# victorca25/traiNNer

Measured on AMD Instinct MI355X. Metric: HR images/sec (G+D step), ESRGAN x4 128->512, higher is better.
Workload: dtype f32 (bf16x3)

## Files before the change

include/trainner_hip.h:

```cpp
#ifndef TRAINNER_HIP_H
#define TRAINNER_HIP_H

#include <stdint.h>

#ifdef __cplusplus
extern "C" {
#endif

#define TNR_OK 0
#define TNR_EINVAL (-1)
#define TNR_ELAUNCH (-2)

enum { TNR_ACT_NONE = 0, TNR_ACT_LRELU = 1, TNR_ACT_RELU = 2 };

enum {
    TNR_CONV_3x3 = 0,
    TNR_CONV_3x3_UP2 = 1,
    TNR_CONV_4x4_S2 = 2,
    TNR_DGRAD_4x4_S2 = 3,
    TNR_CONV_1x1 = 4,
    TNR_CONV_3x3_C4 = 5,
    TNR_CONV_7x7_C4 = 6
};

enum {
    TNR_PACK_FWD = 0,
    TNR_PACK_DGRAD_3x3 = 1,
    TNR_PACK_FWD_S2D = 2,
    TNR_PACK_DGRAD_S2 = 3,
    TNR_PACK_COL_FWD = 4,
    TNR_PACK_COL_DGRAD3 = 5,
    TNR_PACK_C4_FWD = 6,
    TNR_PACK_C4_DGRAD3 = 7,
    TNR_PACK_UP2_DGRAD_S2 = 8,
    TNR_PACK_UP2_FWD_S2D = 9
};

#define TNR_MMA_F32 0
#define TNR_MMA_BF16 1
#define TNR_MMA_BF16X3 2

typedef struct tnr_view {
    float *ptr;
    int32_t ctot;
    int32_t coff;
} tnr_view;

typedef struct tnr_conv_desc {
    tnr_view x;
    int32_t N, H, W;
    int32_t Cin;
    const float *wp;
    int32_t KinP, KoutP;
    tnr_view y;
    int32_t Ho, Wo, Cout;
    int32_t mode;
    const float *bias;
    int32_t act;
    float slope;
    float alpha;
    tnr_view r1; int32_t r1_ch; float beta1;
    tnr_view r2; float alpha2;
    tnr_view m;  int32_t m_lo, m_hi; float m_slope;
    float *ws; int64_t ws_bytes;
    int32_t mma;
    int32_t pad_mode;
    float noise_sigma; int32_t noise_pos; uint32_t noise_key0, noise_key1, noise_pix0;
    const void *wq; int64_t wq_bytes;
    int32_t wq_form;
    int32_t shuffle;
} tnr_conv_desc;

typedef struct tnr_wgrad_desc {
    tnr_view x; int32_t N, H, W; int32_t Cin;
    tnr_view g; int32_t Ho, Wo; int32_t Cout;
    int32_t mode;
    float *dw; int32_t cin_total, cin_begin;
    float *db;
    float alpha, beta;
    float *ws; int64_t ws_bytes;
    int32_t mma;
    int32_t pad_mode;
    float *dw2; int32_t cout_split, cin_total2;
    float *db2;
} tnr_wgrad_desc;

typedef struct tnr_pack_item {
    const float *w;
    float *wp;
    int32_t Cout, Cin, kh, kw;
    int32_t kind;
    int32_t KoutP, KinP;
    int64_t n_out;
} tnr_pack_item;

typedef struct tnr_dense_pack_item {
    const float *w[5];
    float *wp;
    int32_t nf, gc;
    int32_t t;
    int32_t KoutP, KinP;
    float scale5;
    int64_t n_out;
} tnr_dense_pack_item;

const char *tnr_last_error(void);
#define TNR_ABI_VERSION 3
int tnr_version(void);

int tnr_pack_dims(int32_t Cout, int32_t Cin, int32_t kh, int32_t kw, int32_t kind,
                  int32_t *KoutP, int32_t *KinP, int64_t *n_out);
int tnr_pack_weights(const tnr_pack_item *items_dev, int32_t n, int64_t max_out, void *stream);
int tnr_upconv_fold_table(int32_t out[144]);
int tnr_upconv_wgrad_unfold(const float *dws, float *dw3, int32_t Cout, int32_t Cin, float alpha, float beta, void *stream);
int tnr_pack_dense_dims(int32_t nf, int32_t gc, int32_t t, int32_t *KoutP, int32_t *KinP, int64_t *n_out);
int tnr_pack_dense_dgrad(const tnr_dense_pack_item *items_dev, int32_t n, int64_t max_out, void *stream);
int tnr_conv_forward(const tnr_conv_desc *d, void *stream);
int tnr_gauss_mult(tnr_view dst, tnr_view src, int64_t pixels, int32_t C, float sigma, uint32_t key0, uint32_t key1, uint32_t pix0,
                   void *stream);
int64_t tnr_conv_workspace_bytes(const tnr_conv_desc *d);
int64_t tnr_conv_wq_bytes(const tnr_conv_desc *d);
int tnr_conv_wq_pack(const tnr_conv_desc *d, void *image, int64_t image_bytes, void *stream);
int64_t tnr_conv_wino_bytes(const tnr_conv_desc *d);
int tnr_conv_wino_pack(const tnr_conv_desc *d, void *image, int64_t image_bytes, void *stream);
int tnr_im2col(tnr_view x, int32_t N, int32_t H, int32_t W, int32_t C, int32_t k, int32_t stride, int32_t pad,
               int32_t Ho, int32_t Wo, float *out, void *stream);
#define TNR_CHAIN_MAX 6
int64_t tnr_conv_chain_workspace_bytes(const tnr_conv_desc *stage0);
int tnr_conv_chain(const tnr_conv_desc *stages, const int32_t *fresh_from, int32_t n, uint32_t *ws, int64_t ws_bytes,
                   uint32_t epoch, void *stream);
int64_t tnr_conv_sweep_image_bytes(const tnr_conv_desc *stages, int32_t n);
int tnr_conv_sweep_pack(const tnr_conv_desc *stages, int32_t n, void *image, int64_t image_bytes, void *stream);
typedef struct tnr_sweep_pack_item { int32_t units; int32_t reserved; uint64_t opaque[15]; } tnr_sweep_pack_item;
int tnr_conv_sweep_pack_item(const tnr_conv_desc *stages, int32_t n, void *image, int64_t image_bytes, tnr_sweep_pack_item *item);
int tnr_conv_sweep_pack_batch(const tnr_sweep_pack_item *items_dev, int32_t n, int32_t max_units, void *stream);
int tnr_conv_sweep(const tnr_conv_desc *stages, int32_t n, const void *image, uint32_t *ws, int64_t ws_bytes, uint32_t epoch,
                   void *stream);
int64_t tnr_conv_thin_pack_floats(int32_t reduce_channels);
int tnr_conv_thin_pack(const float *w_oihw, float *wp, int32_t Cout, int32_t Cin, int32_t dgrad, void *stream);
int tnr_conv_thin(tnr_view x, int32_t N, int32_t H, int32_t W, int32_t Cin, const float *wp, tnr_view y, int32_t Cout,
                  const float *bias, float alpha, void *stream);
int64_t tnr_conv_thin7_pack_floats(int32_t reduce_channels);
int tnr_conv_thin7_pack(const float *w_oihw, float *wp, int32_t Cout, int32_t Cin, int32_t dgrad, void *stream);
int tnr_conv_thin7(tnr_view x, int32_t N, int32_t H, int32_t W, int32_t Cin, const float *wp, tnr_view y, int32_t Ho, int32_t Wo,
                   int32_t Cout, int32_t pad, int32_t reflect, const float *bias, float alpha, void *stream);
int64_t tnr_wgrad_workspace_bytes(const tnr_wgrad_desc *d);
int64_t tnr_wgrad_thin_workspace_bytes(int32_t N, int32_t H, int32_t Cbig);
int tnr_wgrad_thin(tnr_view big, tnr_view small, int32_t N, int32_t H, int32_t W, int32_t Cbig, int32_t Csmall, int32_t flip,
                   float *dw, float *db, float alpha, float beta, float *ws, int64_t ws_bytes, void *stream);
int64_t tnr_wgrad_thin7_workspace_bytes(int32_t N, int32_t Hbig_grid, int32_t Cbig);
int tnr_wgrad_thin7(tnr_view big, int32_t N, int32_t H, int32_t W, int32_t rpad, tnr_view small, int32_t Hs, int32_t Ws, int32_t off,
                    int32_t Cbig, int32_t Csmall, int32_t flip, float *dw, float *db, float alpha, float beta, float *ws, int64_t ws_bytes,
                    void *stream);
int tnr_conv_wgrad(const tnr_wgrad_desc *d, void *stream);
#define TNR_WGRAD_GROUP_MAX 12
int tnr_conv_wgrad_group(const tnr_wgrad_desc *descs, int32_t n, void *stream);
int tnr_wgrad_tile_class(const tnr_wgrad_desc *d, int32_t group_jobs, int32_t x3_occ, int32_t out[12]);

int tnr_gconv_fwd(tnr_view x, int32_t N, int32_t H, int32_t W, int32_t Cin, const float *w, const float *bias, tnr_view y, int32_t Ho,
                  int32_t Wo, int32_t Cout, int32_t k, int32_t stride, int32_t pad, int32_t reflect, int32_t act, float slope, void *stream);
int tnr_gconv_dgrad(tnr_view g, int32_t N, int32_t H, int32_t W, int32_t Cin, const float *w, tnr_view gx, int32_t Ho, int32_t Wo,
                    int32_t Cout, int32_t k, int32_t stride, int32_t pad, int32_t reflect, void *stream);
int64_t tnr_gconv_wgrad_workspace_bytes(int32_t Cout, int32_t Cin, int32_t k);
int tnr_gconv_wgrad(tnr_view x, int32_t N, int32_t H, int32_t W, int32_t Cin, tnr_view g, int32_t Ho, int32_t Wo, int32_t Cout, int32_t k,
                    int32_t stride, int32_t pad, int32_t reflect, float *dw, float *db, float alpha, float beta, double *ws,
                    int64_t ws_bytes, void *stream);
int tnr_bias_grad(tnr_view g, int64_t pixels, int32_t C, float *db, float alpha, float beta, double *ws, int64_t ws_bytes, void *stream);
int tnr_pad2d(tnr_view x, tnr_view y, int32_t N, int32_t H, int32_t W, int32_t C, int32_t pad, int32_t mode, void *stream);
int tnr_unpad2d(tnr_view xp, tnr_view y, int32_t N, int32_t H, int32_t W, int32_t C, int32_t pad, int32_t mode, void *stream);
int tnr_window2d(tnr_view src, int32_t Hs, int32_t Ws, tnr_view dst, int32_t N, int32_t Hd, int32_t Wd, int32_t C, int32_t oy,
                 int32_t ox, int32_t acc, void *stream);
int tnr_tanh_fwd(const float *x, float *y, int64_t n, void *stream);
int tnr_tanh_bwd(const float *g, const float *y, float *gx, int64_t n, void *stream);
int tnr_gan_loss(const float *pred, int64_t n, int32_t type, float target, float *out, float *grad, void *stream);
int tnr_dp_unique_id(void *id128);
int tnr_dp_init(const void *id128, int32_t rank, int32_t world, void **comm);
int tnr_dp_allreduce_bucket(void *comm, float *buf, int64_t count, int32_t average, void *stream);
int tnr_dp_broadcast(void *comm, float *buf, int64_t count, int32_t root, void *stream);
int tnr_dp_comm_count(void *comm, int32_t *nranks);
int tnr_dp_finalize(void *comm);
int tnr_filter2d(const float *src, float *dst, const float *kernels21, int32_t N, int32_t C, int32_t H, int32_t W, void *stream);
int tnr_resize(const float *src, float *dst, int32_t NC, int32_t H, int32_t W, int32_t Ho, int32_t Wo, int32_t mode, void *stream);
int tnr_noise_gaussian(float *img, int32_t N, int32_t C, int32_t H, int32_t W, const float *sigma255, const int32_t *grey,
                       uint64_t seed, int32_t clip, void *stream);
int tnr_noise_poisson(float *img, int32_t N, int32_t C, int32_t H, int32_t W, const float *vals, const float *scale,
                      const int32_t *grey, uint64_t seed, int32_t clip, void *stream);
int64_t tnr_jpeg_workspace_bytes(int32_t N, int32_t H, int32_t W);
int tnr_jpeg_sim(float *img, int32_t N, int32_t H, int32_t W, const int32_t *quality, float *ws, int64_t ws_bytes, void *stream);
int tnr_feed_u8_to_tensor(const uint8_t *src, int32_t N, int32_t H, int32_t W, int32_t C, const int32_t *flags, int32_t any_rot,
                          float *dst, int32_t bgr2rgb, float data_range, int32_t normalize, void *stream);
int tnr_tensor2np_u8(const float *src, int32_t N, int32_t C, int32_t H, int32_t W, uint8_t *dst, int32_t rgb2bgr,
                     int32_t denormalize, void *stream);
int64_t tnr_metrics_workspace_bytes(int32_t N);
int tnr_psnr_ssim_u8(const uint8_t *a, const uint8_t *b, int32_t N, int32_t H, int32_t W, int32_t C, int32_t crop,
                     int32_t want_ssim, double *out, double *ws, int64_t ws_bytes, void *stream);
int tnr_lpips_stem_dims(int32_t H, int32_t W, int32_t crop, int32_t *Ho, int32_t *Wo);
int tnr_lpips_stem(const void *a, const void *b, int32_t src_kind, int32_t N, int32_t H, int32_t W, int32_t C, int32_t crop,
                   int32_t normalize, const float *shift, const float *scale, const float *w, const float *bias, tnr_view y,
                   void *stream);
int tnr_maxpool3s2_ceil_dims(int32_t H, int32_t W, int32_t *Ho, int32_t *Wo);
int tnr_maxpool3s2_ceil_fwd(tnr_view x, tnr_view y, int32_t N, int32_t H, int32_t W, int32_t C, void *stream);
int64_t tnr_lpips_workspace_bytes(int32_t N, int32_t L);
int tnr_lpips_head(tnr_view f0, tnr_view f1, int32_t N, int32_t H, int32_t W, int32_t C, const float *w, int32_t layer, int32_t L,
                   double *ws, int64_t ws_bytes, void *stream);
int tnr_lpips_finalize(int32_t N, int32_t L, const double *ws, int64_t ws_bytes, double *out, double *per_layer, void *stream);
int tnr_bilinear2x_fwd(tnr_view x, tnr_view y, int32_t N, int32_t H, int32_t W, int32_t C, void *stream);
int tnr_bilinear2x_bwd(tnr_view gy, tnr_view gx, tnr_view gz, tnr_view mask, float mslope, int32_t N, int32_t H, int32_t W,
                       int32_t C, void *stream);
int tnr_add2(tnr_view dst, tnr_view a, tnr_view b, int64_t pixels, int32_t C, void *stream);
int tnr_mask_copy(tnr_view dst, tnr_view src, tnr_view y, int64_t pixels, int32_t C, float mslope, void *stream);
int tnr_nchw_to_nhwc(const float *src, int32_t N, int32_t C, int32_t H, int32_t W, tnr_view dst,
                     int32_t Cpad, const float *scale, const float *shift, void *stream);
int tnr_nhwc_to_nchw(tnr_view src, int32_t N, int32_t C, int32_t H, int32_t W, float *dst,
                     const float *scale, int32_t accumulate, void *stream);
int tnr_upsample2x_bwd(tnr_view gup, tnr_view gx, int32_t N, int32_t H, int32_t W, int32_t C,
                       tnr_view mask, float mslope, void *stream);
int tnr_depth_to_space(tnr_view x, tnr_view y, int32_t N, int32_t H, int32_t W, int32_t Cout, void *stream);
int tnr_space_to_depth_bwd(tnr_view gy, tnr_view gx, int32_t N, int32_t H, int32_t W, int32_t Cout,
                           tnr_view mask, float mslope, void *stream);
int tnr_maxpool2_fwd(tnr_view x, tnr_view y, int32_t N, int32_t H, int32_t W, int32_t C, void *stream);
int tnr_maxpool2_bwd(tnr_view gy, tnr_view x, tnr_view gx, int32_t N, int32_t H, int32_t W, int32_t C,
                     void *stream);
int tnr_axpby(tnr_view dst, tnr_view src, int64_t pixels, int32_t C, float a, float b, void *stream);
int tnr_mask_mul(tnr_view g, tnr_view y, int64_t pixels, int32_t C, float mslope, void *stream);
int tnr_fill(float *p, int64_t n, float v, void *stream);

int64_t tnr_bn_workspace_bytes(int32_t C);
int tnr_bn_train_fwd(tnr_view z, tnr_view y, int64_t pixels, int32_t C, const float *gamma,
                     const float *beta, float *running_mean, float *running_var, int64_t *num_batches,
                     float momentum, float eps, float *save_mean, float *save_invstd, int32_t act,
                     float slope, void *ws, void *stream);
int tnr_bn_train_fwd_stats(tnr_view z, tnr_view y, int64_t pixels, int32_t C, const float *gamma, const float *beta,
                           float *running_mean, float *running_var, int64_t *num_batches, float momentum, float eps,
                           float *save_mean, float *save_invstd, double *stat64, int32_t act, float slope, void *ws, void *stream);
int tnr_bn_replay_running(float *running_mean, float *running_var, int64_t *num_batches, const double *stat64, int32_t C,
                          float momentum, void *stream);
int tnr_bn_train_bwd(tnr_view gy, tnr_view y, tnr_view z, tnr_view gz, int64_t pixels, int32_t C,
                     const float *gamma, const float *save_mean, const float *save_invstd, float mslope,
                     float *dgamma, float *dbeta, float acc_beta, void *ws, void *stream);
int tnr_bn_train_bwd_z(tnr_view gy, tnr_view z, tnr_view gz, int64_t pixels, int32_t C, const float *gamma, const float *beta,
                       const float *save_mean, const float *save_invstd, float mslope, float *dgamma, float *dbeta,
                       float acc_beta, void *ws, void *stream);
int64_t tnr_instnorm_workspace_bytes(int32_t N, int32_t C);
int tnr_instnorm_fwd(tnr_view z, tnr_view y, int32_t N, int64_t pixels_per_image, int32_t C, float eps, float *save_mean,
                     float *save_invstd, int32_t act, float slope, void *ws, void *stream);
int tnr_instnorm_bwd(tnr_view gy, tnr_view y, tnr_view z, tnr_view gz, int32_t N, int64_t pixels_per_image, int32_t C,
                     const float *save_mean, const float *save_invstd, float mslope, void *ws, void *stream);

int tnr_linear_fwd(const float *x, const float *w, const float *b, float *y, int32_t N, int32_t In,
                   int32_t Out, int32_t act, float slope, void *stream);
int tnr_linear_bwd(const float *x, const float *w, const float *gy, const float *yact, float mslope,
                   float *gx, float *dw, float *db, int32_t N, int32_t In, int32_t Out, float acc_beta,
                   float *gpre_ws, void *stream);

int64_t tnr_reduce_workspace_bytes(void);
int tnr_l1_mean_fwd(const float *a, const float *b, int64_t n, float scale, float *loss, void *ws,
                    void *stream);
int tnr_l1_mean_bwd(const float *a, const float *b, int64_t n, float scale, const float *gscale,
                    float *ga, int32_t accumulate, void *stream);
int tnr_ragan_phase_a(const float *pf, const float *pr, int32_t n, float *sums, void *ws, void *stream);
int tnr_ragan_phase_b(const float *pf, const float *pr, int32_t n, int32_t stage, float *sums, void *ws, void *stream);
int tnr_ragan_phase_c(const float *pf, const float *pr, int32_t n, int32_t stage, float weight,
                      const float *sums, float *loss_out, float *gf, float *gr, void *stream);
int tnr_scale_by(float *dst, const float *src, int64_t n, const float *gscale, void *stream);

int64_t tnr_ssim_workspace_bytes(int32_t N, int32_t C, int32_t H, int32_t W, int32_t shave, int32_t K);
int tnr_ssim_fwd(const float *x, const float *y, int32_t N, int32_t C, int32_t H, int32_t W, int32_t layout, int32_t shave,
                 const float *taps, int32_t K, float C1, float C2, double *sums, void *ws, int64_t ws_bytes, void *stream);
int tnr_ssim_bwd(const float *x, const float *y, int32_t N, int32_t C, int32_t H, int32_t W, int32_t layout, int32_t shave,
                 const float *taps, int32_t K, float C1, float C2, const float *coef, const float *gscale, float *gx,
                 int32_t accumulate, void *stream);
int tnr_avgpool2_pad_dims(int32_t H, int32_t W, int32_t shave, int32_t *Ho, int32_t *Wo);
int tnr_avgpool2_pad_fwd(const float *x, const float *y, int32_t N, int32_t C, int32_t H, int32_t W, int32_t layout, int32_t shave,
                         float *xo, float *yo, void *stream);
int tnr_avgpool2_pad_bwd(const float *gcoarse, float *gfine, int32_t N, int32_t C, int32_t H, int32_t W, int32_t layout,
                         int32_t shave, void *stream);
int tnr_msssim_combine(const double *sums, int32_t levels, int32_t N, const int64_t *counts, const float *weights, int32_t mode,
                       float *value, float *coef, void *stream);

enum { TNR_CRIT_L1 = 0, TNR_CRIT_L2 = 1, TNR_CRIT_CB = 2, TNR_CRIT_ELASTIC = 3, TNR_CRIT_CLIPL1 = 4 };
int64_t tnr_imgloss_workspace_bytes(int32_t N, int32_t C, int32_t H, int32_t W);
int tnr_filter_loss_fwd(const float *x, const float *y, int32_t N, int32_t C, int32_t H, int32_t W, int32_t layout, const float *taps,
                        int32_t K, int32_t crit, double scale, float *loss, float *dmap, void *ws, int64_t ws_bytes, void *stream);
int tnr_filter_loss_bwd(const float *dmap, int32_t N, int32_t C, int32_t H, int32_t W, int32_t layout, const float *taps, int32_t K,
                        double scale, const float *gscale, float *gx, int32_t accumulate, void *stream);
int tnr_fd_loss_fwd(const float *x, const float *y, int32_t N, int32_t C, int32_t H, int32_t W, int32_t layout, int32_t dirs,
                    int32_t crit, double scale, float *loss, void *ws, int64_t ws_bytes, void *stream);
int tnr_fd_loss_bwd(const float *x, const float *y, int32_t N, int32_t C, int32_t H, int32_t W, int32_t layout, int32_t dirs,
                    int32_t crit, double scale, const float *gscale, float *gx, int32_t accumulate, void *stream);
int tnr_pointwise_loss_fwd(const float *a, const float *b, int64_t n, int32_t crit, double scale, float *loss, void *ws, void *stream);
int tnr_pointwise_loss_bwd(const float *a, const float *b, int64_t n, int32_t crit, double scale, const float *gscale, float *ga,
                           int32_t accumulate, void *stream);

int tnr_overflow_loss_fwd(const float *x, int64_t n, double scale, float *loss, void *ws, void *stream);
int tnr_overflow_loss_bwd(const float *x, int64_t n, double scale, const float *gscale, float *gx, int32_t accumulate, void *stream);

enum { TNR_CRIT_L1COS = 5 };
int64_t tnr_pooled_workspace_bytes(void);
int tnr_pooled_forward_blocks(int32_t pool_blocks, int32_t ms_blocks);
int tnr_pool_loss_fwd(const float *x, const float *y, int32_t N, int32_t C, int32_t H, int32_t W, int32_t layout, int32_t k, int32_t uv,
                      int32_t crit, float *loss, void *ws, int64_t ws_bytes, void *stream);
int tnr_pool_loss_bwd(const float *x, const float *y, int32_t N, int32_t C, int32_t H, int32_t W, int32_t layout, int32_t k, int32_t uv,
                      int32_t crit, const float *gscale, float *gx, int32_t accumulate, void *stream);
int tnr_multiscale_loss_fwd(const float *x, const float *y, int32_t N, int32_t C, int32_t H, int32_t W, int32_t layout, int32_t crit,
                            float *loss, void *ws, int64_t ws_bytes, void *stream);
int tnr_multiscale_loss_bwd(const float *x, const float *y, int32_t N, int32_t C, int32_t H, int32_t W, int32_t layout, int32_t crit,
                            const float *gscale, float *gx, int32_t accumulate, void *stream);

enum { TNR_SPL_RGB = 1, TNR_SPL_YUV = 2, TNR_SPL_DIMG = 4, TNR_SPL_DYUV = 8 };
int64_t tnr_spl_workspace_bytes(int32_t N, int32_t C, int32_t H, int32_t W, int32_t mask);
int64_t tnr_spl_coef_bytes(int32_t N, int32_t C, int32_t H, int32_t W, int32_t mask);
int tnr_spl_loss_fwd(const float *x, const float *y, int32_t N, int32_t C, int32_t H, int32_t W, int32_t layout, int32_t mask,
                     int32_t denorm, float *loss, float *coef, void *ws, int64_t ws_bytes, void *stream);
int tnr_spl_loss_bwd(const float *x, const float *y, int32_t N, int32_t C, int32_t H, int32_t W, int32_t layout, int32_t mask,
                     int32_t denorm, const float *coef, const float *gscale, float *gx, int32_t accumulate, void *stream);

int tnr_freqsep_low(const float *x, int32_t N, int32_t C, int32_t H, int32_t W, int32_t layout, const float *taps9, const float *gscale,
                    float *out, int32_t accumulate, void *stream);
int tnr_freqsep_high_fwd(const float *x, int32_t N, int32_t C, int32_t H, int32_t W, int32_t layout, const float *taps9, float *out,
                         void *stream);
int tnr_freqsep_high_bwd(const float *g, const float *o, int32_t N, int32_t C, int32_t H, int32_t W, int32_t layout, const float *taps9,
                         const float *gscale, float *gx, int32_t accumulate, void *stream);

int64_t tnr_diffaug_workspace_bytes(int32_t N);
int tnr_diffaug_mean(const float *src, int32_t N, int32_t C, int32_t H, int32_t W, int32_t layout, const void *params,
                     const int32_t *geo, int32_t backward, void *ws, int64_t ws_bytes, void *stream);
int tnr_diffaug_fwd(const float *x, int32_t N, int32_t C, int32_t H, int32_t W, int32_t layout, const void *params, const int32_t *geo,
                    const void *ws, float *out, void *stream);
int tnr_diffaug_bwd(const float *g_out, int32_t N, int32_t C, int32_t H, int32_t W, int32_t layout, const void *params,
                    const int32_t *geo, const void *ws, float *gx, void *stream);

int tnr_batchaug_mix(const float *x, const float *x2, const int32_t *r, const float *col, int32_t N, int32_t C, int32_t H, int32_t W,
                     int32_t layout, const int32_t *prm, float a, float b, float *out, void *stream);
int tnr_batchaug_mask(const float *x, const uint8_t *mask, int32_t N, int32_t C, int32_t H, int32_t W, int32_t layout, int32_t s,
                      float *out, void *stream);

int64_t tnr_gram_workspace_bytes(int32_t N, int32_t H, int32_t W, int32_t C);
int tnr_gram_fwd(tnr_view x, int32_t N, int32_t H, int32_t W, int32_t C, float scale, int32_t mma, float *G, float *ws, int64_t ws_bytes,
                 void *stream);
int tnr_gram_bwd(tnr_view x, const float *S, int32_t N, int32_t H, int32_t W, int32_t C, float scale, int32_t mma, tnr_view dx,
                 int32_t accumulate, void *stream);

int64_t tnr_cx_sums_workspace_bytes(int32_t N, int32_t P, int32_t C);
int tnr_cx_sums(tnr_view y, int32_t N, int32_t H, int32_t W, int32_t C, const int32_t *idx, int32_t P, float *sums, void *ws, int64_t ws_bytes,
                void *stream);
int tnr_cx_prepare(tnr_view x, int32_t N, int32_t H, int32_t W, int32_t C, const int32_t *idx, int32_t P, const float *sums, float *xh, float *nrm,
                   void *stream);
int64_t tnr_cx_matrix_bytes(int32_t N, int32_t P);
int tnr_cx_distance(const float *xh, const float *yh, int32_t N, int32_t P, int32_t C, int32_t mma, float *D, void *stream);
int tnr_cx_rows(float *D, int32_t N, int32_t P, float b, float h, float *rowmin, int32_t *argmin, float *rowE, void *colpack, void *stream);
int tnr_cx_finalize(const void *colpack, int32_t N, int32_t P, float *colmax, int32_t *argmax, float *CS, float *gcoef, float *loss, void *stream);
int tnr_cx_grad_rows(float *D, const float *xh, const float *yh, int32_t N, int32_t P, int32_t C, float h, const float *rowmin,
                     const int32_t *argmin, const float *rowE, const int32_t *argmax, const float *gcoef, float *dwin, void *stream);
int tnr_cx_grad_gemm(const float *G, const float *yh, int32_t N, int32_t P, int32_t C, int32_t mma, float *dxh, void *stream);
int tnr_cx_norm_bwd(const float *dxh, const float *xh, const float *nrm, int32_t N, int32_t H, int32_t W, int32_t C, int32_t P, const int32_t *inv,
                    tnr_view dx, void *stream);

int tnr_sumsq(const float *g, int64_t n, double *out, void *ws, void *stream);
int tnr_clip_by_norm(float *g, int64_t n, const double *sumsq, float max_norm, void *stream);
int tnr_adam_step(float *p, const float *g, float *m, float *v, int64_t n, float step_size, double b1,
                  double b2, float bc2_sqrt, float eps, float weight_decay, void *stream);
int tnr_adam_step_guarded(float *p, const float *g, float *m, float *v, int64_t n, float step_size, double b1,
                          double b2, float bc2_sqrt, float eps, float weight_decay, const uint32_t *fault, void *stream);
int64_t tnr_optim_workspace_bytes(int32_t nseg, int64_t nrows);
int tnr_sgd_step_guarded(float *p, const float *g, float *buf, const int64_t *chunks, int32_t nchunks, float lr, float momentum,
                         float weight_decay, const uint32_t *fault, void *stream);
int tnr_rmsprop_step_guarded(float *p, const float *g, float *square_avg, const int64_t *chunks, int32_t nchunks, float lr,
                             double alpha, float eps, float weight_decay, const uint32_t *fault, void *stream);
int tnr_madgrad_step_guarded(float *p, const float *g, float *grad_sum_sq, float *s, const float *x0, const int64_t *chunks,
                             int32_t nchunks, float lamb, float eps, float decay, float decay_mul, int32_t adamw, double momentum,
                             const uint32_t *fault, void *stream);
int tnr_adamp_step_guarded(float *p, const float *g, float *m, float *v, const int64_t *chunks, int32_t nchunks, const int64_t *segs,
                           int32_t nseg, const int32_t *rowseg, int64_t nrows, void *ws, int64_t ws_bytes, float step_size, double b1,
                           double b2, float bc2_sqrt, float eps, int32_t nesterov, double delta, float weight_decay, float decay_1,
                           float decay_r, const uint32_t *fault, void *stream);
// ... 15 lines not shown
```

trainner_amd/csrc/conv_epilogue.h:

```cpp
#pragma once
#include "conv_body.h"

namespace {

template <int MODE, int TW, int NT, int MT, bool COH, int DEPTH = 1, bool NOISE = true, int BIAS_STEP = 1, class PixFn>
__device__ __forceinline__ void conv_epilogue_dpp_map(const ConvK a, f32x16 (&acc)[MT][NT], const int cb, const int n, const int ty0,
                                                      const int tx0, const int par, const int li, const int half,
                                                      const __amdgpu_buffer_rsrc_t y_rs, PixFn &&pixfn) {
    constexpr bool DG2 = (MODE == TNR_DGRAD_4x4_S2);
    constexpr int NC = NT * 32;
    const int py = par >> 1, px = par & 1;
    TNR_STAMP(2);
#ifdef TNR_PRIO_EPI
    __builtin_amdgcn_s_setprio(TNR_PRIO_EPI);
#endif
    const int qa = li >> 2, qb = li & 3;
    const bool b0 = (qb & 1) != 0, b1 = (qb & 2) != 0;
    auto quad_transpose = [&](float &v0, float &v1, float &v2, float &v3) {
        auto xchg = [&](float &x, float &y, bool sel, int which) {
            const float send = sel ? x : y;
            const int r_ = which == 1 ? __builtin_amdgcn_mov_dpp(__builtin_bit_cast(int, send), 0xB1, 0xF, 0xF, true)
                                      : __builtin_amdgcn_mov_dpp(__builtin_bit_cast(int, send), 0x4E, 0xF, 0xF, true);
            const float recv = __builtin_bit_cast(float, r_);
            x = sel ? recv : x;
            y = sel ? y : recv;
        };
        xchg(v0, v1, b0, 1);
        xchg(v2, v3, b0, 1);
        xchg(v0, v2, b1, 2);
        xchg(v1, v3, b1, 2);
    };
    TNR_STAMP(5);
    TNR_STAMP(6);
    TNR_STAMP(7);
#ifdef TNR_ABL_NOMASK
    const bool has_r1 = a.r1 != nullptr, has_r2 = a.r2 != nullptr, has_m = false;
#else
    const bool has_r1 = a.r1 != nullptr, has_r2 = a.r2 != nullptr, has_m = a.m != nullptr;
#endif
    const bool has_noise = NOISE && a.noise_pos != 0;
    const bool all_full = (a.Cout & 3) == 0;
    const float ns = a.act == TNR_ACT_LRELU ? a.slope : (a.act == TNR_ACT_RELU ? 0.f : 1.f);
    int co_n[NT];
    bool co_ok[NT];
    f32x4 bv[NT];
    float b1f[NT], msf[NT];
    bool use_r1[NT], use_m[NT];
#pragma unroll
    for (int nn = 0; nn < NT; ++nn) {
        const int co = cb * NC + nn * 32 + qa * 4;
        co_n[nn] = co;
        co_ok[nn] = co < a.Cout;
        bv[nn] = f32x4{0.f, 0.f, 0.f, 0.f};
        if (a.bias != nullptr && co_ok[nn]) {
            if constexpr (BIAS_STEP != 1) {
#pragma unroll
                for (int k = 0; k < 4; ++k)
                    if (co + k < a.Cout) bv[nn][k] = a.bias[(co + k) * BIAS_STEP];
            } else if (co + 4 <= a.Cout) {
                bv[nn] = *reinterpret_cast<const f32x4 *>(a.bias + co);
            } else {
#pragma unroll
                for (int k = 0; k < 4; ++k)
                    if (co + k < a.Cout) bv[nn][k] = a.bias[co + k];
            }
        }
        use_r1[nn] = has_r1 && co < a.r1_ch;
        use_m[nn] = has_m && co >= a.m_lo && co < a.m_hi;
        b1f[nn] = use_r1[nn] ? a.beta1 : 0.f;
        msf[nn] = use_m[nn] ? a.m_slope : 1.f;
    }
    constexpr int UNITS = MT * 4;
    constexpr int AHEAD = DEPTH < UNITS ? DEPTH : UNITS, SETS = AHEAD + 1 < UNITS ? AHEAD + 1 : UNITS;
    bool ok[SETS];
    size_t pixi[SETS];
    f32x4 q1[SETS][NT], q2[SETS][NT], qm[SETS][NT];
    auto prep = [&](int u, int set) {
        const int mi = u >> 2, q = u & 3;
        int rr, cc;
        pixfn(mi, 8 * q + 4 * half + qb, rr, cc);
        const int sy = ty0 + rr, sx = tx0 + cc;
        ok[set] = sy < a.th_space && sx < a.tw_space;
        const int oy = DG2 ? 2 * sy + py : sy;
        const int ox = DG2 ? 2 * sx + px : sx;
        const size_t pix = ((size_t)n * a.Ho + oy) * a.Wo + ox;
        pixi[set] = pix;
        const f32x4 zero = {0.f, 0.f, 0.f, 0.f}, one = {1.f, 1.f, 1.f, 1.f};
#pragma unroll
        for (int nn = 0; nn < NT; ++nn) {
            const bool okc = ok[set] && co_ok[nn];
            if (has_r1) {
                q1[set][nn] = zero;
                if (okc && use_r1[nn]) q1[set][nn] = *reinterpret_cast<const f32x4 *>(a.r1 + pix * a.r1_ct + a.r1_co + co_n[nn]);
            }
            if (has_r2) {
                q2[set][nn] = zero;
                if (okc) q2[set][nn] = *reinterpret_cast<const f32x4 *>(a.r2 + pix * a.r2_ct + a.r2_co + co_n[nn]);
            }
            if (has_m) {
                qm[set][nn] = one;
                if (okc && use_m[nn]) qm[set][nn] = *reinterpret_cast<const f32x4 *>(a.m + pix * a.m_ct + a.m_co + co_n[nn]);
            }
        }
    };
    auto finish = [&](int u, int set) {
        const int mi = u >> 2, q = u & 3;
#pragma unroll
        for (int nn = 0; nn < NT; ++nn) {
            float v0 = acc[mi][nn][4 * q + 0], v1 = acc[mi][nn][4 * q + 1], v2 = acc[mi][nn][4 * q + 2], v3 = acc[mi][nn][4 * q + 3];
            quad_transpose(v0, v1, v2, v3);
            f32x4 v = f32x4{v0, v1, v2, v3} + bv[nn];
#pragma unroll
            for (int e = 0; e < 4; ++e) v[e] = __builtin_fmaf(ns, __builtin_fminf(v[e], 0.f), __builtin_fmaxf(v[e], 0.f)) * a.alpha;
            if (has_r1) v += b1f[nn] * q1[set][nn];
            if (has_noise) {
                const f32x4 nm = tnr_gauss_mult4(((unsigned)pixi[set] + a.noise_pix0) * (unsigned)(a.Cout >> 2) + (unsigned)(co_n[nn] >> 2),
                                                 a.noise_k0, a.noise_k1, a.noise_sigma);
                if (a.noise_pos == 1) v *= nm;
                if (has_r2) v = v * a.alpha2 + q2[set][nn];
                if (a.noise_pos != 1) v *= nm;
            } else if (has_r2) {
                v = v * a.alpha2 + q2[set][nn];
            }
            if (has_m) {
#pragma unroll
                for (int e = 0; e < 4; ++e) v[e] *= (qm[set][nn][e] > 0.f ? 1.f : msf[nn]);
            }
            if (!(ok[set] && co_ok[nn])) continue;
            const int co = co_n[nn];
#ifdef TNR_ABL_NOEPISTORE
            if (v[0] == 1.2345e30f) a.y[0] = v[1] + v[2] + v[3];
            continue;
#endif
            if (COH) {
                __builtin_amdgcn_raw_buffer_store_b128(__builtin_bit_cast(tnr_u32x4, v), y_rs,
                                                       (int)((unsigned)(pixi[set] * a.y_ct + a.y_co + co) * 4u), 0, TNR_COH_STORE_AUX);
            } else {
                float *yp = a.y + pixi[set] * a.y_ct + a.y_co + co;
                if (all_full) {
                    *reinterpret_cast<f32x4 *>(yp) = v;
                } else {
#pragma unroll
                    for (int e = 0; e < 4; ++e)
                        if (co + e < a.Cout) yp[e] = v[e];
                }
            }
        }
    };
#pragma unroll
    for (int u = 0; u < AHEAD; ++u) prep(u, u % SETS);
#pragma unroll
    for (int u = 0; u < UNITS; ++u) {
        if (u + AHEAD < UNITS) prep(u + AHEAD, (u + AHEAD) % SETS);
        finish(u, u % SETS);
    }
}

template <int MODE, int TW, int NT, int MT, bool COH, int DEPTH = 1, bool NOISE = true, int BIAS_STEP = 1>
__device__ __forceinline__ void conv_epilogue_dpp(const ConvK a, f32x16 (&acc)[MT][NT], const int cb, const int n, const int ty0,
                                                  const int tx0, const int par, const int wave, const int li, const int half,
                                                  const __amdgpu_buffer_rsrc_t y_rs) {
    conv_epilogue_dpp_map<MODE, TW, NT, MT, COH, DEPTH, NOISE, BIAS_STEP>(a, acc, cb, n, ty0, tx0, par, li, half, y_rs,
                                                                [&](int mi, int row, int &rr, int &cc) __attribute__((always_inline)) {
                                                                    const int p = (wave * MT + mi) * 32 + row;
                                                                    rr = p / TW;
                                                                    cc = p - rr * TW;
                                                                });
}

}
```

trainner_amd/csrc/conv_wino.hip:

```cpp
#include <stddef.h>
#include <stdlib.h>
#include <type_traits>
#include <utility>
#include "conv_body.h"
#include "conv_epilogue.h"

namespace {

constexpr int WN_T = 16;
constexpr int WN_PT = WN_T / 2;
constexpr int WN_NP = WN_PT * WN_PT;
constexpr int WN_RAW_W = WN_T + 2;
constexpr int WN_RAW_PIX = WN_RAW_W * WN_RAW_W;
constexpr int WN_RAW_STRIDE = 24;
constexpr int WN_RAW_FLOATS = WN_RAW_PIX * WN_RAW_STRIDE;
constexpr int WN_ROW = TNR_X3_ROW;
constexpr int WN_VH_ROWS = 8 * WN_NP;
constexpr int WN_VH_FLOATS = WN_VH_ROWS * WN_ROW;
constexpr size_t WN_LDS_BYTES = (size_t)(2 * WN_VH_FLOATS + 2 * WN_RAW_FLOATS) * sizeof(float);
constexpr int WN_UNIT_FLOATS = 32 * WN_ROW;
constexpr int WN_STAGE_ITEMS = WN_RAW_PIX * 4;
constexpr int WN_STAGE_IT = (WN_STAGE_ITEMS / 2 + 255) / 256;
static_assert(WN_LDS_BYTES <= 160 * 1024, "one Winograd workgroup per CU");
static_assert(8 * 4 * 16 * 64 * sizeof(float) <= WN_LDS_BYTES, "the inverse transform's exchange fits the LDS");
static_assert(WN_STAGE_IT * 256 * 2 >= WN_STAGE_ITEMS, "staging plan covers the patch");

#ifndef WN_PRIO
#define WN_PRIO 3
#endif
#ifdef WN_TIMELINE
__device__ unsigned long long wn_tl[2][16];
#define WN_T(v) const unsigned long long v = __builtin_amdgcn_s_memtime()
#define WN_ADD(i, d) do { if (lane == 0 && (wave & 3) == 0) tl[i] += (d); } while (0)
#else
#define WN_T(v) do { } while (0)
#define WN_ADD(i, d) do { } while (0)
#endif

struct WinoK {
    ConvK a;
    const float *wq;
    int wq_bytes;
    int nck;
    int tiles_x, tiles_y, ncb, tiles;
};

struct WinoPackK {
    const float *wp;
    int KinP, KoutP, nck, ncb, units;
    float *out;
};

__global__ void __launch_bounds__(256) wino_pack_kernel(const WinoPackK a) {
    const int g = blockIdx.x * 256 + threadIdx.x;
    const int unit = g >> 6, r = (g >> 1) & 31, oh = g & 1;
    if (unit >= a.units) return;
    const int j = unit & 3;
    int rest = unit >> 2;
    const int ck = rest % a.nck;
    rest /= a.nck;
    const int i = rest & 3, nt = (rest >> 2) & 1, cb = rest >> 3;
    const int co = cb * 64 + nt * 32 + r;
    const double G[4][3] = {{1.0, 0.0, 0.0}, {0.5, 0.5, 0.5}, {0.5, -0.5, 0.5}, {0.0, 0.0, 1.0}};
    f32x4 q[2];
#pragma unroll
    for (int e = 0; e < 8; ++e) {
        const int ch = 16 * ck + 8 * oh + e;
        double u = 0.0;
#pragma unroll
        for (int ky = 0; ky < 3; ++ky)
#pragma unroll
            for (int kx = 0; kx < 3; ++kx)
                u += G[i][ky] * G[j][kx] * (double)a.wp[((size_t)(ky * 3 + kx) * a.KoutP + co) * a.KinP + ch];
        q[e >> 2][e & 3] = (float)u;
    }
    tnr_bf16x8 pl[3];
    tnr_split_bf16x3(q[0], q[1], pl);
    float *dst = a.out + (size_t)unit * WN_UNIT_FLOATS + (oh * 32 + r) * 4;
#pragma unroll
    for (int k = 0; k < 3; ++k) *reinterpret_cast<tnr_bf16x8 *>(dst + k * 256) = pl[k];
}

template <int B, class F, int... I>
__device__ __forceinline__ void wn_static_for_seq(F &f, std::integer_sequence<int, I...>) {
    (f(std::integral_constant<int, B + I>{}), ...);
}
template <int B, int E, class F>
__device__ __forceinline__ void wn_static_for(F &&f) {
    wn_static_for_seq<B>(f, std::make_integer_sequence<int, (E > B ? E - B : 0)>{});
}

__global__ void __launch_bounds__(512, 2) conv3x3_wino_kernel(const WinoK c) {
    extern __shared__ __attribute__((aligned(16))) float smem[];
    float *s_v = smem;
    float *s_raw = smem + 2 * WN_VH_FLOATS;
    const int tid = threadIdx.x;
    const int wave = __builtin_amdgcn_readfirstlane(tid >> 6), lane = tid & 63, li = lane & 31, half = lane >> 5;
    const int wil = wave & 1, wn = (wave >> 1) & 1, wh = wave >> 2;
    const int wi = 2 * wh + wil;
    const int tt = tid & 255;
    const ConvK &a = c.a;
    const __amdgpu_buffer_rsrc_t x_rs =
        __builtin_amdgcn_make_buffer_rsrc(const_cast<float *>(a.x), 0, (int)((unsigned)a.N * a.H * a.W * a.x_ct * 4u), 0x00020000);
    const __amdgpu_buffer_rsrc_t w_rs = __builtin_amdgcn_make_buffer_rsrc(const_cast<float *>(c.wq), 0, c.wq_bytes, 0x00020000);
    const __amdgpu_buffer_rsrc_t y_rs =
        __builtin_amdgcn_make_buffer_rsrc(a.y, 0, (int)((unsigned)a.N * a.Ho * a.Wo * a.y_ct * 4u), 0x00020000);
    float *s_vh = s_v + wh * WN_VH_FLOATS;

    const int tp = tt >> 2, tq = tt & 3;
    const int tpy = tp >> 3, tpx = tp & 7;
    const int raw_off = ((2 * tpy + wh) * WN_RAW_W + 2 * tpx) * WN_RAW_STRIDE + 4 * tq;
    static_assert(TNR_X3_SWZ < 4, "the swizzle bit must not depend on the transform position or the M-tile");
    const int v_dst0 = tp * WN_ROW + 4 * ((tq >> 1) ^ ((tp >> TNR_X3_SWZ) & 1)) + 2 * (tq & 1);
    const int a_src0 = (wil * 4 * WN_NP + li) * WN_ROW + 4 * (half ^ ((li >> TNR_X3_SWZ) & 1));
    constexpr int XL_STRIDE = WN_NP * WN_ROW;

#ifdef WN_TIMELINE
    unsigned long long tl[16] = {0, 0, 0, 0, 0, 0, 0, 0, 0, 0, 0, 0, 0, 0, 0, 0};
    const unsigned long long tl_begin = __builtin_amdgcn_s_memtime();
#endif
    for (int tile = blockIdx.x; tile < c.tiles; tile += gridDim.x) {
        const int cb = tile % c.ncb;
        int rest = tile / c.ncb;
        const int tx = rest % c.tiles_x;
        rest /= c.tiles_x;
        const int ty = rest % c.tiles_y, n = rest / c.tiles_y;
        const int ty0 = ty * WN_T, tx0 = tx * WN_T;
        int in_off[WN_STAGE_IT], r_dst[WN_STAGE_IT];
#pragma unroll
        for (int it = 0; it < WN_STAGE_IT; ++it) {
            const int il = tt + it * 256;
            const int i = wh * (WN_STAGE_ITEMS / 2) + il, pix = i >> 2, q = i & 3;
            const int pr = pix / WN_RAW_W, pc = pix - pr * WN_RAW_W;
            int Y = ty0 + pr - 1, X = tx0 + pc - 1;
            if (a.reflect) {
                Y = Y == -1 ? 1 : (Y == a.H ? a.H - 2 : Y);
                X = X == -1 ? 1 : (X == a.W ? a.W - 2 : X);
            }
            const bool mine = il < WN_STAGE_ITEMS / 2;
            const bool in = mine & (Y >= 0) & (Y < a.H) & (X >= 0) & (X < a.W);
            in_off[it] = in ? (((n * a.H + Y) * a.W + X) * a.x_ct + a.x_co + q * 4) : -1;
            r_dst[it] = mine ? pix * WN_RAW_STRIDE + 4 * q : -1;
        }
        f32x4 rin[WN_STAGE_IT];
        auto raw_load = [&](int ch, bool valid) __attribute__((always_inline)) {
#pragma unroll
            for (int it = 0; it < WN_STAGE_IT; ++it) {
                const unsigned bo = (valid && in_off[it] >= 0) ? (unsigned)(in_off[it] + ch) * 4u : 0xfffffff0u;
                rin[it] = __builtin_bit_cast(f32x4, __builtin_amdgcn_raw_buffer_load_b128(x_rs, (int)bo, 0, 0));
            }
        };
        auto raw_store = [&](int buf) __attribute__((always_inline)) {
#pragma unroll
            for (int it = 0; it < WN_STAGE_IT; ++it)
                if (r_dst[it] >= 0) *reinterpret_cast<f32x4 *>(s_raw + buf * WN_RAW_FLOATS + r_dst[it]) = rin[it];
        };

        f32x16 acc[4][2];
#pragma unroll
        for (int j = 0; j < 4; ++j)
#pragma unroll
            for (int m = 0; m < 2; ++m)
#pragma unroll
                for (int r = 0; r < 16; ++r) acc[j][m][r] = 0.f;

        tnr_bf16x8 fbr[4][3];
        const int bq0 = (((cb * 2 + wn) * 4 + wi) * c.nck) * 4;
        auto b_fetch = [&](int ck, auto j0c) __attribute__((always_inline)) {
            constexpr int J0 = decltype(j0c)::value;
            const int u0 = bq0 + ck * 4;
#pragma unroll
            for (int j = J0; j < J0 + 2; ++j)
#pragma unroll
                for (int sp = 0; sp < 3; ++sp)
                    fbr[j][sp] = __builtin_bit_cast(tnr_bf16x8, __builtin_amdgcn_raw_buffer_load_b128(w_rs, lane * 16, ((u0 + j) * 3 + sp) * 1024, 0));
        };

        auto transform_h = [&](int rb, auto hc) __attribute__((always_inline)) {
            constexpr int H = decltype(hc)::value;
            const float *src = s_raw + rb * WN_RAW_FLOATS + raw_off;
            f32x4 ea[4], eb[4];
            f32x4 r[4][3];
#pragma unroll
            for (int q = 0; q < 4; ++q)
#pragma unroll
                for (int p = 0; p < 3; ++p) r[q][p] = *reinterpret_cast<const f32x4 *>(src + (p * WN_RAW_W + q) * WN_RAW_STRIDE);
            __builtin_amdgcn_sched_barrier(0);
#ifdef WN_TIMELINE
            asm volatile("s_waitcnt lgkmcnt(0)" ::: "memory");
            { WN_T(ts); WN_ADD(9, ts); }
#endif
#pragma unroll
            for (int q = 0; q < 4; ++q) {
                ea[q] = H == 0 ? r[q][0] - r[q][2] : r[q][1] - r[q][0];
                eb[q] = H == 0 ? r[q][1] + r[q][2] : r[q][0] - r[q][2];
            }
            auto colstep = [&](const f32x4 (&e)[4], int j) __attribute__((always_inline)) {
// ... 31 lines not shown
                    l[j] = __builtin_bit_cast(tnr_bf16x4, tnr_f32x2{__builtin_bit_cast(float, __builtin_convertvector(a0, tnr_bf16x2)),
                                                                   __builtin_bit_cast(float, __builtin_convertvector(a1, tnr_bf16x2))});
                }
#pragma unroll
                for (int j = 0; j < 4; ++j) store3(xl0 + j, h[j], m[j], l[j]);
#else
#pragma unroll
                for (int j = 0; j < 4; j += 2) {
                    const f32x4 va = colstep(e, j), vb = colstep(e, j + 1);
                    tnr_bf16x4 ha, hb, ma, mb;
                    f32x4 ra, rb, qa, qb;
                    tnr_pk_level(va, ha, ra);
                    tnr_pk_level(vb, hb, rb);
                    tnr_pk_level(ra, ma, qa);
                    tnr_pk_level(rb, mb, qb);
                    const tnr_f32x2 a0 = {qa[0], qa[1]}, a1 = {qa[2], qa[3]}, b0 = {qb[0], qb[1]}, b1 = {qb[2], qb[3]};
                    const tnr_bf16x4 la = __builtin_bit_cast(tnr_bf16x4, tnr_f32x2{__builtin_bit_cast(float, __builtin_convertvector(a0, tnr_bf16x2)),
                                                                                 __builtin_bit_cast(float, __builtin_convertvector(a1, tnr_bf16x2))});
                    const tnr_bf16x4 lb = __builtin_bit_cast(tnr_bf16x4, tnr_f32x2{__builtin_bit_cast(float, __builtin_convertvector(b0, tnr_bf16x2)),
                                                                                 __builtin_bit_cast(float, __builtin_convertvector(b1, tnr_bf16x2))});
                    store3(xl0 + j, ha, ma, la);
                    store3(xl0 + j + 1, hb, mb, lb);
                }
#endif
            };
#ifdef WN_TIMELINE
            __builtin_amdgcn_sched_barrier(0);
            { WN_T(ts); WN_ADD(10, ts); }
#endif
            emit(ea, 0);
#ifdef WN_TIMELINE
            __builtin_amdgcn_sched_barrier(0);
            { WN_T(ts); WN_ADD(11, ts); }
#endif
            emit(eb, 4);
#ifdef WN_TIMELINE
            asm volatile("s_waitcnt lgkmcnt(0)" ::: "memory");
            { WN_T(ts); WN_ADD(12, ts); }
#endif
        };
        auto transform = [&](int rb) __attribute__((always_inline)) {
#ifdef WN_TPRIO
            __builtin_amdgcn_s_setprio(WN_TPRIO);
#endif
            if (wh == 0) transform_h(rb, std::integral_constant<int, 0>{});
            else transform_h(rb, std::integral_constant<int, 1>{});
#ifdef WN_TPRIO
            __builtin_amdgcn_s_setprio(0);
#endif
        };

        auto multiply = [&]() __attribute__((always_inline)) {
            constexpr int TA[6] = {0, 2, 1, 0, 1, 0}, TB[6] = {2, 0, 1, 1, 0, 0};
            tnr_bf16x8 fa[2][3];
#ifndef WN_NOPRIO
            __builtin_amdgcn_s_setprio(WN_PRIO);
#endif
#pragma unroll
            for (int sp = 0; sp < 3; ++sp) fa[0][sp] = *reinterpret_cast<const tnr_bf16x8 *>(s_vh + a_src0 + 8 * sp);
            wn_static_for<0, 8>([&](auto uc) __attribute__((always_inline)) {
                constexpr int u = decltype(uc)::value, j = u >> 1, m = u & 1;
#ifndef WN_X_NOFA
                if constexpr (u + 1 < 8) {
                    constexpr int j1 = (u + 1) >> 1, m1 = (u + 1) & 1;
#pragma unroll
                    for (int sp = 0; sp < 3; ++sp)
                        fa[(u + 1) & 1][sp] = *reinterpret_cast<const tnr_bf16x8 *>(s_vh + a_src0 + j1 * XL_STRIDE + m1 * 32 * WN_ROW + 8 * sp);
                }
#else
                if constexpr (u == 0) {
#pragma unroll
                    for (int sp = 0; sp < 3; ++sp) fa[1][sp] = fa[0][sp];
                }
#endif
                __builtin_amdgcn_sched_barrier(0);
#pragma unroll
                for (int p = 0; p < 6; ++p) {
                    acc[j][m] = __builtin_amdgcn_mfma_f32_32x32x16_bf16(fa[u & 1][TA[p]], fbr[j][TB[p]], acc[j][m], 0, 0, 0);
#ifdef WN_MFMA_NOPS
#pragma unroll
                    for (int k = 0; k < WN_MFMA_NOPS; ++k) asm volatile("s_nop 7");
#endif
                }
                __builtin_amdgcn_sched_barrier(0);
            });
#ifndef WN_NOPRIO
            __builtin_amdgcn_s_setprio(0);
#endif
        };

        __syncthreads();
        raw_load(0, true);
        raw_store(0);
        raw_load(16, c.nck > 1);
        if (c.nck > 1) raw_store(1);
        __syncthreads();
        WN_T(t_loop0);
        if (wh == 1) __syncthreads();
#pragma unroll 1
        for (int ck = 0; ck < c.nck; ++ck) {
            WN_T(t0);
#ifndef WN_X_NORAW
            if (ck >= 1 && ck + 1 < c.nck) raw_store((ck + 1) & 1);
#endif
#if !defined(WN_X_NOB) && defined(WN_B_EARLY)
            b_fetch(ck, std::integral_constant<int, 0>{});
#elif defined(WN_X_NOB)
            if (ck == 0) { b_fetch(0, std::integral_constant<int, 0>{}); b_fetch(0, std::integral_constant<int, 2>{}); }
#endif
            { WN_T(ts); WN_ADD(8, ts); WN_ADD(13, t0); }
#ifndef WN_X_NOT
            transform(ck & 1);
#endif
#if !defined(WN_X_NOB) && !defined(WN_B_EARLY)
            b_fetch(ck, std::integral_constant<int, 0>{});
#endif
            WN_T(t1);
            __syncthreads();
            WN_T(t2);
#ifndef WN_X_NOB
            b_fetch(ck, std::integral_constant<int, 2>{});
#endif
#ifndef WN_X_NORAW
            raw_load(16 * (ck + 2), ck + 2 < c.nck);
#endif
#ifndef WN_X_NOM
            multiply();
#endif
            WN_T(t3);
            __syncthreads();
            WN_T(t4);
            WN_ADD(0, t1 - t0); WN_ADD(1, t2 - t1); WN_ADD(2, t3 - t2); WN_ADD(3, t4 - t3); WN_ADD(7, 1ull);
        }
        if (wh == 0) __syncthreads();
        WN_T(t_loop1);
        WN_ADD(4, t_loop1 - t_loop0);

#ifdef WN_X_NOEPI
        if (a.alpha == 1.2345e30f)
#endif
        {
        {
            float *xch = smem + wave * (4 * 16 * 64);
#pragma unroll
            for (int l = 0; l < 2; ++l)
#pragma unroll
                for (int m = 0; m < 2; ++m) {
                    const f32x16 rr = l == 0 ? (acc[0][m] + acc[1][m]) + acc[2][m] : (acc[1][m] - acc[2][m]) - acc[3][m];
#pragma unroll
                    for (int r = 0; r < 16; ++r) xch[((l * 2 + m) * 16 + r) * 64 + lane] = rr[r];
                }
        }
        __syncthreads();
        f32x16 keep[2][1];
        {
            const int k = wil, m = wh;
            auto slot = [&](int ip, int l) __attribute__((always_inline)) {
                return smem + (((ip >> 1) * 4 + wn * 2 + (ip & 1)) * 4 + l * 2 + m) * (16 * 64) + lane;
            };
#pragma unroll
            for (int l = 0; l < 2; ++l) {
                const float *p0 = slot(k, l), *p1 = slot(k + 1, l), *p2 = slot(k + 2, l);
#pragma unroll
                for (int r = 0; r < 16; ++r) {
                    const float x0 = p0[r * 64], x1 = p1[r * 64], x2 = p2[r * 64];
                    keep[l][0][r] = k == 0 ? (x0 + x1) + x2 : (x0 - x1) - x2;
                }
            }
        }
        conv_epilogue_dpp_map<TNR_CONV_3x3, WN_T, 1, 2, false, 1>(a, keep, cb * 2 + wn, n, ty0, tx0, 0, li, half, y_rs,
                                                                  [&](int mi, int row, int &rr, int &cc) __attribute__((always_inline)) {
                                                                      const int p = 32 * wh + row;
                                                                      rr = 2 * (p >> 3) + wil;
                                                                      cc = 2 * (p & 7) + mi;
                                                                  });
        }
    }
#ifdef WN_TIMELINE
    if (lane == 0 && (wave & 3) == 0) {
        tl[5] = __builtin_amdgcn_s_memtime() - tl_begin;
        for (int i = 0; i < 16; ++i) atomicAdd(&wn_tl[wh][i], tl[i]);
    }
#endif
}

constexpr int W16_STAGE_IT = (WN_STAGE_ITEMS / 2 + 511) / 512;

__global__ void __launch_bounds__(1024, 4) conv3x3_wino16_kernel(const WinoK c) {
    extern __shared__ __attribute__((aligned(16))) float smem[];
    float *s_v = smem;
    float *s_raw = smem + 2 * WN_VH_FLOATS;
    const int tid = threadIdx.x;
    const int wave = __builtin_amdgcn_readfirstlane(tid >> 6), lane = tid & 63, li = lane & 31, half = lane >> 5;
    const int wh = (wave >> 2) & 1, role = (wave & 3) | ((wave >> 3) << 2);
    const int wil = role & 1, wn = (role >> 1) & 1, wjp = role >> 2;
    const int wi = 2 * wh + wil;
    const int tt = role * 64 + lane;
    const ConvK &a = c.a;
    const __amdgpu_buffer_rsrc_t x_rs =
        __builtin_amdgcn_make_buffer_rsrc(const_cast<float *>(a.x), 0, (int)((unsigned)a.N * a.H * a.W * a.x_ct * 4u), 0x00020000);
    const __amdgpu_buffer_rsrc_t w_rs = __builtin_amdgcn_make_buffer_rsrc(const_cast<float *>(c.wq), 0, c.wq_bytes, 0x00020000);
    const __amdgpu_buffer_rsrc_t y_rs =
        __builtin_amdgcn_make_buffer_rsrc(a.y, 0, (int)((unsigned)a.N * a.Ho * a.Wo * a.y_ct * 4u), 0x00020000);
    float *s_vh = s_v + wh * WN_VH_FLOATS;

    const int tp = (tt >> 2) & 63, tq = tt & 3, rs = tt >> 8;
    const int tpy = tp >> 3, tpx = tp & 7;
    const int it_ = 2 * wh + rs;
    const int pa = it_ == 0 ? 0 : (it_ == 2 ? 2 : 1), pb = it_ == 0 ? 2 : (it_ == 1 ? 2 : (it_ == 2 ? 1 : 3));
    const bool plus = it_ == 1;
    const int raw_a = ((2 * tpy + pa) * WN_RAW_W + 2 * tpx) * WN_RAW_STRIDE + 4 * tq;
    const int raw_b = ((2 * tpy + pb) * WN_RAW_W + 2 * tpx) * WN_RAW_STRIDE + 4 * tq;
    static_assert(TNR_X3_SWZ < 4, "the swizzle bit must not depend on the transform position or the M-tile");
    const int v_dst0 = (rs * 4 * WN_NP + tp) * WN_ROW + 4 * ((tq >> 1) ^ ((tp >> TNR_X3_SWZ) & 1)) + 2 * (tq & 1);
    const int a_src0 = ((wil * 4 + 2 * wjp) * WN_NP + li) * WN_ROW + 4 * (half ^ ((li >> TNR_X3_SWZ) & 1));
    constexpr int XL_STRIDE = WN_NP * WN_ROW;

    for (int tile = blockIdx.x; tile < c.tiles; tile += gridDim.x) {
        const int cb = tile % c.ncb;
        int rest = tile / c.ncb;
        const int tx = rest % c.tiles_x;
        rest /= c.tiles_x;
        const int ty = rest % c.tiles_y, n = rest / c.tiles_y;
        const int ty0 = ty * WN_T, tx0 = tx * WN_T;
        int in_off[W16_STAGE_IT], r_dst[W16_STAGE_IT];
#pragma unroll
        for (int it = 0; it < W16_STAGE_IT; ++it) {
            const int il = tt + it * 512;
            const int i = wh * (WN_STAGE_ITEMS / 2) + il, pix = i >> 2, q = i & 3;
            const int pr = pix / WN_RAW_W, pc = pix - pr * WN_RAW_W;
            int Y = ty0 + pr - 1, X = tx0 + pc - 1;
            if (a.reflect) {
                Y = Y == -1 ? 1 : (Y == a.H ? a.H - 2 : Y);
                X = X == -1 ? 1 : (X == a.W ? a.W - 2 : X);
            }
            const bool mine = il < WN_STAGE_ITEMS / 2;
            const bool in = mine & (Y >= 0) & (Y < a.H) & (X >= 0) & (X < a.W);
            in_off[it] = in ? (((n * a.H + Y) * a.W + X) * a.x_ct + a.x_co + q * 4) : -1;
            r_dst[it] = mine ? pix * WN_RAW_STRIDE + 4 * q : -1;
        }
        f32x4 rin[W16_STAGE_IT];
        auto raw_load = [&](int ch, bool valid) __attribute__((always_inline)) {
#pragma unroll
            for (int it = 0; it < W16_STAGE_IT; ++it) {
                const unsigned bo = (valid && in_off[it] >= 0) ? (unsigned)(in_off[it] + ch) * 4u : 0xfffffff0u;
                rin[it] = __builtin_bit_cast(f32x4, __builtin_amdgcn_raw_buffer_load_b128(x_rs, (int)bo, 0, 0));
            }
        };
        auto raw_store = [&](int buf) __attribute__((always_inline)) {
#pragma unroll
            for (int it = 0; it < W16_STAGE_IT; ++it)
                if (r_dst[it] >= 0) *reinterpret_cast<f32x4 *>(s_raw + buf * WN_RAW_FLOATS + r_dst[it]) = rin[it];
        };

        f32x16 acc[2][2];
#pragma unroll
        for (int jj = 0; jj < 2; ++jj)
#pragma unroll
            for (int m = 0; m < 2; ++m)
#pragma unroll
                for (int r = 0; r < 16; ++r) acc[jj][m][r] = 0.f;

        tnr_bf16x8 fbr[2][3];
        const int bq0 = (((cb * 2 + wn) * 4 + wi) * c.nck) * 4 + 2 * wjp;
        auto b_fetch = [&](int ck) __attribute__((always_inline)) {
            const int u0 = bq0 + ck * 4;
#pragma unroll
            for (int jj = 0; jj < 2; ++jj)
#pragma unroll
                for (int sp = 0; sp < 3; ++sp)
                    fbr[jj][sp] = __builtin_bit_cast(tnr_bf16x8, __builtin_amdgcn_raw_buffer_load_b128(w_rs, lane * 16, ((u0 + jj) * 3 + sp) * 1024, 0));
        };
        auto transform = [&](int rb) __attribute__((always_inline)) {
            const float *sa_ = s_raw + rb * WN_RAW_FLOATS + raw_a, *sb_ = s_raw + rb * WN_RAW_FLOATS + raw_b;
            f32x4 e[4];
#pragma unroll
            for (int q = 0; q < 4; ++q) {
                const f32x4 da = *reinterpret_cast<const f32x4 *>(sa_ + q * WN_RAW_STRIDE), db = *reinterpret_cast<const f32x4 *>(sb_ + q * WN_RAW_STRIDE);
                e[q] = plus ? da + db : da - db;
            }
            auto store3 = [&](int j, const tnr_bf16x4 &h_, const tnr_bf16x4 &m_, const tnr_bf16x4 &l_) __attribute__((always_inline)) {
                float *d = s_vh + v_dst0 + j * XL_STRIDE;
                *reinterpret_cast<tnr_f32x2 *>(d) = __builtin_bit_cast(tnr_f32x2, h_);
                *reinterpret_cast<tnr_f32x2 *>(d + 8) = __builtin_bit_cast(tnr_f32x2, m_);
                *reinterpret_cast<tnr_f32x2 *>(d + 16) = __builtin_bit_cast(tnr_f32x2, l_);
            };
#pragma unroll
            for (int j = 0; j < 4; ++j) {
                const f32x4 v = j == 0 ? e[0] - e[2] : (j == 1 ? e[1] + e[2] : (j == 2 ? e[2] - e[1] : e[1] - e[3]));
                tnr_bf16x4 hh, mm;
                f32x4 r1, r2;
                tnr_pk_level(v, hh, r1);
                tnr_pk_level(r1, mm, r2);
                const tnr_f32x2 a0 = {r2[0], r2[1]}, a1 = {r2[2], r2[3]};
                const tnr_bf16x4 ll = __builtin_bit_cast(tnr_bf16x4, tnr_f32x2{__builtin_bit_cast(float, __builtin_convertvector(a0, tnr_bf16x2)),
                                                                             __builtin_bit_cast(float, __builtin_convertvector(a1, tnr_bf16x2))});
                store3(j, hh, mm, ll);
            }
        };
        auto multiply = [&]() __attribute__((always_inline)) {
            constexpr int TA[6] = {0, 2, 1, 0, 1, 0}, TB[6] = {2, 0, 1, 1, 0, 0};
            tnr_bf16x8 fa[2][3];
#pragma unroll
            for (int sp = 0; sp < 3; ++sp) fa[0][sp] = *reinterpret_cast<const tnr_bf16x8 *>(s_vh + a_src0 + 8 * sp);
            wn_static_for<0, 4>([&](auto uc) __attribute__((always_inline)) {
                constexpr int u = decltype(uc)::value, jj = u >> 1, m = u & 1;
                if constexpr (u + 1 < 4) {
                    constexpr int j1 = (u + 1) >> 1, m1 = (u + 1) & 1;
#pragma unroll
                    for (int sp = 0; sp < 3; ++sp)
                        fa[(u + 1) & 1][sp] = *reinterpret_cast<const tnr_bf16x8 *>(s_vh + a_src0 + j1 * XL_STRIDE + m1 * 32 * WN_ROW + 8 * sp);
                }
                __builtin_amdgcn_sched_barrier(0);
#pragma unroll
                for (int p = 0; p < 6; ++p)
                    acc[jj][m] = __builtin_amdgcn_mfma_f32_32x32x16_bf16(fa[u & 1][TA[p]], fbr[jj][TB[p]], acc[jj][m], 0, 0, 0);
                __builtin_amdgcn_sched_barrier(0);
            });
        };

        __syncthreads();
        raw_load(0, true);
        raw_store(0);
        raw_load(16, c.nck > 1);
        if (c.nck > 1) raw_store(1);
        __syncthreads();
        if (wh == 1) __syncthreads();
#pragma unroll 1
        for (int ck = 0; ck < c.nck; ++ck) {
            if (ck >= 1 && ck + 1 < c.nck) raw_store((ck + 1) & 1);
            transform(ck & 1);
            b_fetch(ck);
            __syncthreads();
            raw_load(16 * (ck + 2), ck + 2 < c.nck);
            multiply();
            __syncthreads();
        }
        if (wh == 0) __syncthreads();

        f32x16 pr_[2][2];
#pragma unroll
        for (int m = 0; m < 2; ++m) {
            if (wjp == 0) {
                pr_[0][m] = acc[0][m] + acc[1][m];
                pr_[1][m] = acc[1][m];
            } else {
                pr_[0][m] = acc[0][m];
                pr_[1][m] = -acc[0][m] - acc[1][m];
            }
        }
        float *xa = smem + (((wave & 3) | (wh << 2)) * 4) * (16 * 64);
        if (wjp == 1) {
#pragma unroll
            for (int l = 0; l < 2; ++l)
#pragma unroll
                for (int m = 0; m < 2; ++m)
#pragma unroll
                    for (int r = 0; r < 16; ++r) xa[((l * 2 + m) * 16 + r) * 64 + lane] = pr_[l][m][r];
        }
        __syncthreads();
        if (wjp == 0) {
#pragma unroll
            for (int l = 0; l < 2; ++l)
#pragma unroll
                for (int m = 0; m < 2; ++m)
#pragma unroll
                    for (int r = 0; r < 16; ++r) pr_[l][m][r] = l == 0 ? pr_[l][m][r] + xa[((l * 2 + m) * 16 + r) * 64 + lane]
                                                                       : pr_[l][m][r] + xa[((l * 2 + m) * 16 + r) * 64 + lane];
        }
        __syncthreads();
        float *xb = smem + ((wh * 4 + wn * 2 + wil) * 4) * (16 * 64);
        if (wjp == 0) {
#pragma unroll
            for (int l = 0; l < 2; ++l)
#pragma unroll
                for (int m = 0; m < 2; ++m)
#pragma unroll
                    for (int r = 0; r < 16; ++r) xb[((l * 2 + m) * 16 + r) * 64 + lane] = pr_[l][m][r];
        }
        __syncthreads();
        f32x16 keep[1][1];
        {
            const int k = wil, m = wh, l = wjp;
            auto slot = [&](int ip) __attribute__((always_inline)) {
                return smem + (((ip >> 1) * 4 + wn * 2 + (ip & 1)) * 4 + l * 2 + m) * (16 * 64) + lane;
            };
            const float *p0 = slot(k), *p1 = slot(k + 1), *p2 = slot(k + 2);
#pragma unroll
            for (int r = 0; r < 16; ++r) {
                const float x0 = p0[r * 64], x1 = p1[r * 64], x2 = p2[r * 64];
                keep[0][0][r] = k == 0 ? (x0 + x1) + x2 : (x0 - x1) - x2;
            }
        }
        conv_epilogue_dpp_map<TNR_CONV_3x3, WN_T, 1, 1, false, 1>(a, keep, cb * 2 + wn, n, ty0, tx0, 0, li, half, y_rs,
                                                                  [&](int, int row, int &rr, int &cc) __attribute__((always_inline)) {
                                                                      const int p = 32 * wh + row;
                                                                      rr = 2 * (p >> 3) + wil;
                                                                      cc = 2 * (p & 7) + wjp;
                                                                  });
    }
}

bool wino_ok(const tnr_conv_desc *d) {
    return d->mode == TNR_CONV_3x3 && d->mma == TNR_MMA_BF16X3 && (d->pad_mode == 0 || (d->pad_mode == 1 && d->H >= 2 && d->W >= 2)) &&
           (d->Cout % 64) == 0 && d->KoutP == d->Cout && d->Cin == d->KinP && (d->Cin % 16) == 0 && d->Cin >= 32 && d->Ho == d->H &&
           d->Wo == d->W && d->W >= 8 && d->H >= 8 && buffers_addressable(*d) &&
           (int64_t)(d->Cout / 64) * (d->Cin / 16) * 32 * WN_UNIT_FLOATS * (int64_t)sizeof(float) < (1LL << 31);
}

}

#ifdef WN_TIMELINE
extern "C" int tnr_debug_wino_timeline(unsigned long long *out16, int reset) {
    if (out16 != nullptr && hipMemcpyFromSymbol(out16, HIP_SYMBOL(wn_tl), sizeof(wn_tl)) != hipSuccess) return TNR_ELAUNCH;
    if (reset) {
        unsigned long long z[32] = {0};
        if (hipMemcpyToSymbol(HIP_SYMBOL(wn_tl), z, sizeof(z)) != hipSuccess) return TNR_ELAUNCH;
    }
    return TNR_OK;
}
#endif

extern "C" int64_t tnr_conv_wino_bytes(const tnr_conv_desc *d) {
    if (d == nullptr || !wino_ok(d)) return 0;
    return (int64_t)(d->Cout / 64) * (d->Cin / 16) * 32 * WN_UNIT_FLOATS * (int64_t)sizeof(float);
}

extern "C" int tnr_conv_wino_pack(const tnr_conv_desc *d, void *image, int64_t image_bytes, void *stream) {
    TNR_REQUIRE(d != nullptr && image != nullptr && d->wp != nullptr && wino_ok(d), "conv_wino_pack: the launch cannot run in the Winograd form");
    WinoPackK a;
    a.wp = d->wp; a.KinP = d->KinP; a.KoutP = d->KoutP; a.nck = d->Cin / 16; a.ncb = d->Cout / 64;
    a.units = a.ncb * a.nck * 32;
    TNR_REQUIRE((int64_t)a.units * WN_UNIT_FLOATS * (int64_t)sizeof(float) <= image_bytes, "conv_wino_pack: image buffer too small");
    a.out = static_cast<float *>(image);
    hipLaunchKernelGGL(wino_pack_kernel, dim3((unsigned)tnr_cdiv(a.units * 64, 256)), dim3(256), 0, (hipStream_t)stream, a);
    return tnr_check_launch("conv_wino_pack");
}

int tnr_launch_conv3x3_wino(const tnr_conv_desc *d, void *stream) {
    if (!wino_ok(d) || d->wq == nullptr || d->wq_bytes < tnr_conv_wino_bytes(d) || d->noise_pos < 0 || d->noise_pos > 2) return 1;
    static int cus = 0;
    if (const int rc = tnr_kernel_setup(&cus, "conv3x3_wino", {{conv3x3_wino_kernel, WN_LDS_BYTES}, {conv3x3_wino16_kernel, WN_LDS_BYTES}})) return rc;
    WinoK c;
    if (!stream_k_from_desc(c, *d, tnr_conv_wino_bytes(d), WN_T, WN_T, 1)) return 1;
    const int grid = c.tiles < cus ? c.tiles : cus;
    static const bool w16 = [] { const char *e = getenv("TNR_WINO_WAVES"); return e != nullptr && atoi(e) == 16; }();
    if (w16) {
        hipLaunchKernelGGL(conv3x3_wino16_kernel, dim3((unsigned)grid), dim3(1024), WN_LDS_BYTES, (hipStream_t)stream, c);
        return tnr_check_launch("conv3x3_wino16");
    }
    hipLaunchKernelGGL(conv3x3_wino_kernel, dim3((unsigned)grid), dim3(512), WN_LDS_BYTES, (hipStream_t)stream, c);
    return tnr_check_launch("conv3x3_wino");
}
```

trainner_amd/csrc/elementwise.hip:

```cpp
#include "common.h"
#include "gauss_noise.h"

namespace {

constexpr int EW_BLOCK = 256;
inline unsigned ew_grid(int64_t n) {
    int64_t b = tnr_cdiv64(n, EW_BLOCK);
    if (b > 256 * 8) b = 256 * 8;
    if (b < 1) b = 1;
    return (unsigned)b;
}

__global__ void nchw_to_nhwc_kernel(const float *src, int N, int C, int H, int W, float *dst, int ct, int co, int Cpad,
                                    const float *scale, const float *shift) {
    const int64_t HW = (int64_t)H * W;
    const int groups = Cpad / 4;
    const int64_t total = (int64_t)N * HW * groups;
    for (int64_t e = (int64_t)blockIdx.x * blockDim.x + threadIdx.x; e < total; e += (int64_t)gridDim.x * blockDim.x) {
        const int64_t pix = e % ((int64_t)N * HW);
        const int gidx = (int)(e / ((int64_t)N * HW));
        const int64_t n = pix / HW, hw = pix - n * HW;
        f32x4 v = {0.f, 0.f, 0.f, 0.f};
#pragma unroll
        for (int k = 0; k < 4; ++k) {
// ... 23 lines not shown
        dst[e] = v;
    }
}

__global__ void upsample2x_bwd_kernel(const float *gup, int u_ct, int u_co, float *gx, int x_ct, int x_co, int N, int H,
                                      int W, int C, const float *mask, int m_ct, int m_co, float mslope) {
    const int c4n = C / 4;
    const int64_t total = (int64_t)N * H * W * c4n;
    for (int64_t e = (int64_t)blockIdx.x * blockDim.x + threadIdx.x; e < total; e += (int64_t)gridDim.x * blockDim.x) {
        const int c4 = (int)(e % c4n);
        const int64_t pix = e / c4n;
        const int x = (int)(pix % W);
        const int64_t q = pix / W;
        const int y = (int)(q % H);
        const int64_t n = q / H;
        f32x4 s = {0.f, 0.f, 0.f, 0.f};
#pragma unroll
        for (int dy = 0; dy < 2; ++dy)
#pragma unroll
            for (int dx = 0; dx < 2; ++dx) {
                const int64_t up = (n * 2 * H + 2 * y + dy) * (2 * W) + 2 * x + dx;
                s += *reinterpret_cast<const f32x4 *>(gup + up * u_ct + u_co + c4 * 4);
            }
        if (mask) {
            const f32x4 mv = *reinterpret_cast<const f32x4 *>(mask + pix * m_ct + m_co + c4 * 4);
#pragma unroll
            for (int k = 0; k < 4; ++k) s[k] *= (mv[k] > 0.f ? 1.f : mslope);
        }
        *reinterpret_cast<f32x4 *>(gx + pix * x_ct + x_co + c4 * 4) = s;
    }
}

__global__ void depth_to_space_kernel(const float *x, int x_ct, int x_co, float *y, int y_ct, int y_co, int N, int H,
                                      int W, int Cout) {
    const int64_t total = (int64_t)N * H * W * Cout;
    for (int64_t e = (int64_t)blockIdx.x * blockDim.x + threadIdx.x; e < total; e += (int64_t)gridDim.x * blockDim.x) {
        const int c = (int)(e % Cout);
        const int64_t pix = e / Cout;
        const int w = (int)(pix % W);
        const int64_t q = pix / W;
        const int h = (int)(q % H);
        const int64_t n = q / H;
        const f32x4 v = *reinterpret_cast<const f32x4 *>(x + pix * x_ct + x_co + c * 4);
#pragma unroll
        for (int k = 0; k < 4; ++k) {
            const int64_t op = (n * 2 * H + 2 * h + (k >> 1)) * (2 * W) + 2 * w + (k & 1);
            y[op * y_ct + y_co + c] = v[k];
        }
    }
}

__global__ void space_to_depth_bwd_kernel(const float *gy, int g_ct, int g_co, float *gx, int x_ct, int x_co, int N, int H,
                                          int W, int Cout, const float *mask, int m_ct, int m_co, float mslope) {
    const int64_t total = (int64_t)N * H * W * Cout;
    for (int64_t e = (int64_t)blockIdx.x * blockDim.x + threadIdx.x; e < total; e += (int64_t)gridDim.x * blockDim.x) {
        const int c = (int)(e % Cout);
        const int64_t pix = e / Cout;
        const int w = (int)(pix % W);
        const int64_t q = pix / W;
        const int h = (int)(q % H);
        const int64_t n = q / H;
        f32x4 v;
#pragma unroll
        for (int k = 0; k < 4; ++k) {
            const int64_t op = (n * 2 * H + 2 * h + (k >> 1)) * (2 * W) + 2 * w + (k & 1);
            float g = gy[op * g_ct + g_co + c];
            if (mask) g *= (mask[op * m_ct + m_co + c] > 0.f ? 1.f : mslope);
            v[k] = g;
        }
        *reinterpret_cast<f32x4 *>(gx + pix * x_ct + x_co + c * 4) = v;
    }
}

__global__ void im2col_kernel(const float *x, int x_ct, int x_co, int N, int H, int W, int C, int k, int stride, int pad, int Ho,
                              int Wo, float *out) {
    const int c4n = C / 4, kk = k * k;
    const int64_t total = (int64_t)N * Ho * Wo * kk * c4n;
    for (int64_t e = (int64_t)blockIdx.x * blockDim.x + threadIdx.x; e < total; e += (int64_t)gridDim.x * blockDim.x) {
        const int c4 = (int)(e % c4n);
        int64_t q = e / c4n;
        const int t = (int)(q % kk);
        const int64_t pix = q / kk;
        const int ox = (int)(pix % Wo);
        q = pix / Wo;
        const int oy = (int)(q % Ho);
        const int64_t n = q / Ho;
        const int Y = oy * stride - pad + t / k, X = ox * stride - pad + t % k;
        f32x4 v = {0.f, 0.f, 0.f, 0.f};
        if (Y >= 0 && Y < H && X >= 0 && X < W) v = *reinterpret_cast<const f32x4 *>(x + ((n * H + Y) * W + X) * x_ct + x_co + c4 * 4);
        *reinterpret_cast<f32x4 *>(out + (pix * kk + t) * C + c4 * 4) = v;
    }
}

__global__ void maxpool2_fwd_kernel(const float *x, int x_ct, int x_co, float *y, int y_ct, int y_co, int N, int H, int W,
                                    int C) {
    const int Ho = H / 2, Wo = W / 2, c4n = C / 4;
    const int64_t total = (int64_t)N * Ho * Wo * c4n;
    for (int64_t e = (int64_t)blockIdx.x * blockDim.x + threadIdx.x; e < total; e += (int64_t)gridDim.x * blockDim.x) {
        const int c4 = (int)(e % c4n);
        const int64_t pix = e / c4n;
        const int ox = (int)(pix % Wo);
        const int64_t q = pix / Wo;
        const int oy = (int)(q % Ho);
        const int64_t n = q / Ho;
        f32x4 best;
#pragma unroll
        for (int k = 0; k < 4; ++k) {
            const int64_t ip = (n * H + 2 * oy + (k >> 1)) * W + 2 * ox + (k & 1);
            const f32x4 v = *reinterpret_cast<const f32x4 *>(x + ip * x_ct + x_co + c4 * 4);
            if (k == 0) best = v;
            else
#pragma unroll
                for (int j = 0; j < 4; ++j) best[j] = v[j] > best[j] ? v[j] : best[j];
        }
        *reinterpret_cast<f32x4 *>(y + pix * y_ct + y_co + c4 * 4) = best;
    }
}

__global__ void maxpool2_bwd_kernel(const float *gy, int g_ct, int g_co, const float *x, int x_ct, int x_co, float *gx,
                                    int gx_ct, int gx_co, int N, int H, int W, int C) {
    const int Ho = H / 2, Wo = W / 2, c4n = C / 4;
    const int64_t total = (int64_t)N * Ho * Wo * c4n;
    for (int64_t e = (int64_t)blockIdx.x * blockDim.x + threadIdx.x; e < total; e += (int64_t)gridDim.x * blockDim.x) {
        const int c4 = (int)(e % c4n);
        const int64_t pix = e / c4n;
        const int ox = (int)(pix % Wo);
        const int64_t q = pix / Wo;
        const int oy = (int)(q % Ho);
        const int64_t n = q / Ho;
        const f32x4 g = *reinterpret_cast<const f32x4 *>(gy + pix * g_ct + g_co + c4 * 4);
        f32x4 v[4];
        int64_t ip[4];
#pragma unroll
        for (int k = 0; k < 4; ++k) {
            ip[k] = (n * H + 2 * oy + (k >> 1)) * W + 2 * ox + (k & 1);
            v[k] = *reinterpret_cast<const f32x4 *>(x + ip[k] * x_ct + x_co + c4 * 4);
        }
        f32x4 o[4];
#pragma unroll
        for (int j = 0; j < 4; ++j) {
            int arg = 0;
            float best = v[0][j];
#pragma unroll
            for (int k = 1; k < 4; ++k)
                if (v[k][j] > best) {
                    best = v[k][j];
                    arg = k;
                }
#pragma unroll
            for (int k = 0; k < 4; ++k) o[k][j] = (k == arg && best > 0.f) ? g[j] : 0.f;
        }
#pragma unroll
        for (int k = 0; k < 4; ++k) *reinterpret_cast<f32x4 *>(gx + ip[k] * gx_ct + gx_co + c4 * 4) = o[k];
    }
}

__global__ void axpby_kernel(float *dst, int d_ct, int d_co, const float *src, int s_ct, int s_co, int64_t pixels, int C,
                             float a, float b) {
    const int c4n = C / 4;
    const int64_t total = pixels * c4n;
    for (int64_t e = (int64_t)blockIdx.x * blockDim.x + threadIdx.x; e < total; e += (int64_t)gridDim.x * blockDim.x) {
        const int c4 = (int)(e % c4n);
        const int64_t pix = e / c4n;
        f32x4 s = *reinterpret_cast<const f32x4 *>(src + pix * s_ct + s_co + c4 * 4);
        float *dp = dst + pix * d_ct + d_co + c4 * 4;
        f32x4 d = {0.f, 0.f, 0.f, 0.f};
        if (b != 0.f) d = *reinterpret_cast<const f32x4 *>(dp);
        *reinterpret_cast<f32x4 *>(dp) = a * s + b * d;
    }
}

__global__ void gauss_mult_kernel(float *dst, int d_ct, int d_co, const float *src, int s_ct, int s_co, int64_t pixels, int C, float sigma,
                                  unsigned k0, unsigned k1, unsigned pix0) {
    const int c4n = C / 4;
    const int64_t total = pixels * c4n;
    for (int64_t e = (int64_t)blockIdx.x * blockDim.x + threadIdx.x; e < total; e += (int64_t)gridDim.x * blockDim.x) {
        const int c4 = (int)(e % c4n);
        const int64_t pix = e / c4n;
        f32x4 v = {1.f, 1.f, 1.f, 1.f};
        if (src != nullptr) v = *reinterpret_cast<const f32x4 *>(src + pix * s_ct + s_co + c4 * 4);
        v *= tnr_gauss_mult4(((unsigned)pix + pix0) * (unsigned)c4n + (unsigned)c4, k0, k1, sigma);
        *reinterpret_cast<f32x4 *>(dst + pix * d_ct + d_co + c4 * 4) = v;
    }
}

__global__ void mask_mul_kernel(float *g, int g_ct, int g_co, const float *y, int y_ct, int y_co, int64_t pixels, int C,
                                float mslope) {
    const int c4n = C / 4;
    const int64_t total = pixels * c4n;
    for (int64_t e = (int64_t)blockIdx.x * blockDim.x + threadIdx.x; e < total; e += (int64_t)gridDim.x * blockDim.x) {
        const int c4 = (int)(e % c4n);
        const int64_t pix = e / c4n;
        float *gp = g + pix * g_ct + g_co + c4 * 4;
        f32x4 gv = *reinterpret_cast<const f32x4 *>(gp);
        const f32x4 yv = *reinterpret_cast<const f32x4 *>(y + pix * y_ct + y_co + c4 * 4);
#pragma unroll
        for (int k = 0; k < 4; ++k) gv[k] *= (yv[k] > 0.f ? 1.f : mslope);
        *reinterpret_cast<f32x4 *>(gp) = gv;
    }
}

__device__ __forceinline__ void bil_taps(int o, int n, int &i0, int &i1, float &w0, float &w1) {
    const int i = o >> 1;
    if (o & 1) {
        i0 = i;
        i1 = i + 1 < n ? i + 1 : n - 1;
        w0 = 0.75f;
        w1 = 0.25f;
    } else {
        i0 = i > 0 ? i - 1 : 0;
        i1 = i;
        w0 = 0.25f;
        w1 = 0.75f;
    }
}

__global__ void bilinear2x_fwd_kernel(const float *x, int x_ct, int x_co, float *y, int y_ct, int y_co, int N, int H, int W, int C) {
    const int c4n = C / 4;
    const int H2 = 2 * H, W2 = 2 * W;
    const int64_t total = (int64_t)N * H2 * W2 * c4n;
    for (int64_t e = (int64_t)blockIdx.x * blockDim.x + threadIdx.x; e < total; e += (int64_t)gridDim.x * blockDim.x) {
        const int c4 = (int)(e % c4n);
        const int64_t pix = e / c4n;
        const int ox = (int)(pix % W2);
        const int64_t q = pix / W2;
        const int oy = (int)(q % H2);
        const int64_t n = q / H2;
        int y0, y1, x0, x1;
        float wy0, wy1, wx0, wx1;
        bil_taps(oy, H, y0, y1, wy0, wy1);
        bil_taps(ox, W, x0, x1, wx0, wx1);
        const float *b = x + x_co + c4 * 4;
        const f32x4 v00 = *reinterpret_cast<const f32x4 *>(b + ((n * H + y0) * W + x0) * x_ct);
        const f32x4 v01 = *reinterpret_cast<const f32x4 *>(b + ((n * H + y0) * W + x1) * x_ct);
        const f32x4 v10 = *reinterpret_cast<const f32x4 *>(b + ((n * H + y1) * W + x0) * x_ct);
        const f32x4 v11 = *reinterpret_cast<const f32x4 *>(b + ((n * H + y1) * W + x1) * x_ct);
        const f32x4 r = wy0 * (wx0 * v00 + wx1 * v01) + wy1 * (wx0 * v10 + wx1 * v11);
        *reinterpret_cast<f32x4 *>(y + pix * y_ct + y_co + c4 * 4) = r;
    }
}

__device__ __forceinline__ void bil_adj(int i, int n, int o[4], float w[4]) {
    o[0] = 2 * i - 1; o[1] = 2 * i; o[2] = 2 * i + 1; o[3] = 2 * i + 2;
    w[0] = 0.25f; w[1] = 0.75f; w[2] = 0.75f; w[3] = 0.25f;
    if (i == 0) { o[0] = 0; }
    if (i == n - 1) { o[3] = 2 * n - 1; }
}

__global__ void bilinear2x_bwd_kernel(const float *gy, int g_ct, int g_co, float *gx, int x_ct, int x_co, float *gz, int z_ct,
                                      int z_co, const float *mask, int m_ct, int m_co, float mslope, int N, int H, int W, int C) {
    const int c4n = C / 4;
    const int W2 = 2 * W;
    const int64_t total = (int64_t)N * H * W * c4n;
    for (int64_t e = (int64_t)blockIdx.x * blockDim.x + threadIdx.x; e < total; e += (int64_t)gridDim.x * blockDim.x) {
        const int c4 = (int)(e % c4n);
        const int64_t pix = e / c4n;
        const int x = (int)(pix % W);
        const int64_t q = pix / W;
        const int y = (int)(q % H);
        const int64_t n = q / H;
        int oy[4], ox[4];
        float wy[4], wx[4];
        bil_adj(y, H, oy, wy);
        bil_adj(x, W, ox, wx);
        f32x4 s = {0.f, 0.f, 0.f, 0.f};
#pragma unroll
        for (int a = 0; a < 4; ++a) {
            f32x4 r = {0.f, 0.f, 0.f, 0.f};
#pragma unroll
            for (int b = 0; b < 4; ++b)
                r += wx[b] * *reinterpret_cast<const f32x4 *>(gy + ((n * 2 * H + oy[a]) * W2 + ox[b]) * g_ct + g_co + c4 * 4);
            s += wy[a] * r;
        }
        if (gx) *reinterpret_cast<f32x4 *>(gx + pix * x_ct + x_co + c4 * 4) = s;
        if (gz) {
            const f32x4 mv = *reinterpret_cast<const f32x4 *>(mask + pix * m_ct + m_co + c4 * 4);
#pragma unroll
            for (int k = 0; k < 4; ++k) s[k] *= (mv[k] > 0.f ? 1.f : mslope);
            *reinterpret_cast<f32x4 *>(gz + pix * z_ct + z_co + c4 * 4) = s;
        }
    }
}

__global__ void add2_kernel(float *dst, int d_ct, int d_co, const float *a, int a_ct, int a_co, const float *b, int b_ct, int b_co,
                            int64_t pixels, int C) {
    const int c4n = C / 4;
    const int64_t total = pixels * c4n;
    for (int64_t e = (int64_t)blockIdx.x * blockDim.x + threadIdx.x; e < total; e += (int64_t)gridDim.x * blockDim.x) {
        const int c4 = (int)(e % c4n);
        const int64_t pix = e / c4n;
        const f32x4 av = *reinterpret_cast<const f32x4 *>(a + pix * a_ct + a_co + c4 * 4);
        const f32x4 bv = *reinterpret_cast<const f32x4 *>(b + pix * b_ct + b_co + c4 * 4);
        *reinterpret_cast<f32x4 *>(dst + pix * d_ct + d_co + c4 * 4) = av + bv;
    }
}

__global__ void mask_copy_kernel(float *dst, int d_ct, int d_co, const float *src, int s_ct, int s_co, const float *y, int y_ct,
                                 int y_co, int64_t pixels, int C, float mslope) {
    const int c4n = C / 4;
    const int64_t total = pixels * c4n;
    for (int64_t e = (int64_t)blockIdx.x * blockDim.x + threadIdx.x; e < total; e += (int64_t)gridDim.x * blockDim.x) {
        const int c4 = (int)(e % c4n);
        const int64_t pix = e / c4n;
        f32x4 gv = *reinterpret_cast<const f32x4 *>(src + pix * s_ct + s_co + c4 * 4);
        const f32x4 yv = *reinterpret_cast<const f32x4 *>(y + pix * y_ct + y_co + c4 * 4);
#pragma unroll
        for (int k = 0; k < 4; ++k) gv[k] *= (yv[k] > 0.f ? 1.f : mslope);
        *reinterpret_cast<f32x4 *>(dst + pix * d_ct + d_co + c4 * 4) = gv;
    }
}

__global__ void fill_kernel(float *p, int64_t n, float v) {
    for (int64_t e = (int64_t)blockIdx.x * blockDim.x + threadIdx.x; e < n; e += (int64_t)gridDim.x * blockDim.x) p[e] = v;
}

__global__ void upconv_wgrad_unfold_kernel(const float *dws, float *dw3, int Cout, int Cin, float alpha, float beta) {
    const int total = Cout * Cin;
    for (int e = blockIdx.x * blockDim.x + threadIdx.x; e < total; e += gridDim.x * blockDim.x) {
        const int co = e / Cin, ci = e - co * Cin;
        float dF[16];
        const f32x4 *src = reinterpret_cast<const f32x4 *>(dws + ((size_t)ci * Cout + co) * 16);
#pragma unroll
        for (int q = 0; q < 4; ++q) {
            const f32x4 v = src[q];
#pragma unroll
            for (int k = 0; k < 4; ++k) dF[4 * q + k] = v[k];
        }
        float *dst = dw3 + (size_t)e * 9;
#pragma unroll
        for (int t = 0; t < 9; ++t) {
            const float prev = (beta != 0.f) ? beta * dst[t] : 0.f;
            dst[t] = prev + alpha * tnr_upfold_grad(dF, t / 3, t % 3);
        }
    }
}

inline bool view_ok(const tnr_view &v) { return v.ptr != nullptr && (v.ctot % 4) == 0 && (v.coff % 4) == 0; }

}

extern "C" int tnr_nchw_to_nhwc(const float *src, int32_t N, int32_t C, int32_t H, int32_t W, tnr_view dst, int32_t Cpad,
                                const float *scale, const float *shift, void *stream) {
    TNR_REQUIRE(src && view_ok(dst) && (Cpad % 4) == 0 && Cpad >= C, "nchw_to_nhwc: bad arguments");
    TNR_REQUIRE((scale == nullptr) == (shift == nullptr), "nchw_to_nhwc: scale and shift go together");
    const int64_t total = (int64_t)N * H * W * (Cpad / 4);
    hipLaunchKernelGGL(nchw_to_nhwc_kernel, dim3(ew_grid(total)), dim3(EW_BLOCK), 0, (hipStream_t)stream, src, N, C, H, W,
                       dst.ptr, dst.ctot, dst.coff, Cpad, scale, shift);
    return tnr_check_launch("nchw_to_nhwc");
}

extern "C" int tnr_nhwc_to_nchw(tnr_view src, int32_t N, int32_t C, int32_t H, int32_t W, float *dst, const float *scale,
                                int32_t accumulate, void *stream) {
    TNR_REQUIRE(dst && view_ok(src), "nhwc_to_nchw: bad arguments");
    const int64_t total = (int64_t)N * C * H * W;
    hipLaunchKernelGGL(nhwc_to_nchw_kernel, dim3(ew_grid(total)), dim3(EW_BLOCK), 0, (hipStream_t)stream, src.ptr, src.ctot,
                       src.coff, N, C, H, W, dst, scale, accumulate);
    return tnr_check_launch("nhwc_to_nchw");
}

extern "C" int tnr_upsample2x_bwd(tnr_view gup, tnr_view gx, int32_t N, int32_t H, int32_t W, int32_t C, tnr_view mask,
                                  float mslope, void *stream) {
    TNR_REQUIRE(view_ok(gup) && view_ok(gx) && (C % 4) == 0, "upsample2x_bwd: bad arguments");
    const int64_t total = (int64_t)N * H * W * (C / 4);
    hipLaunchKernelGGL(upsample2x_bwd_kernel, dim3(ew_grid(total)), dim3(EW_BLOCK), 0, (hipStream_t)stream, gup.ptr, gup.ctot,
                       gup.coff, gx.ptr, gx.ctot, gx.coff, N, H, W, C, mask.ptr, mask.ctot, mask.coff, mslope);
    return tnr_check_launch("upsample2x_bwd");
}

extern "C" int tnr_upconv_wgrad_unfold(const float *dws, float *dw3, int32_t Cout, int32_t Cin, float alpha, float beta, void *stream) {
    TNR_REQUIRE(dws != nullptr && dw3 != nullptr && Cout > 0 && Cin > 0 && (int64_t)Cout * Cin < (1LL << 26),
                "upconv_wgrad_unfold: bad arguments (%d -> %d channels)", Cin, Cout);
    TNR_REQUIRE((reinterpret_cast<uintptr_t>(dws) & 15) == 0, "upconv_wgrad_unfold: the folded gradient must be 16-byte aligned");
    hipLaunchKernelGGL(upconv_wgrad_unfold_kernel, dim3(ew_grid((int64_t)Cout * Cin)), dim3(EW_BLOCK), 0, (hipStream_t)stream, dws, dw3,
                       Cout, Cin, alpha, beta);
    return tnr_check_launch("upconv_wgrad_unfold");
}

extern "C" int tnr_depth_to_space(tnr_view x, tnr_view y, int32_t N, int32_t H, int32_t W, int32_t Cout, void *stream) {
    TNR_REQUIRE(view_ok(x) && view_ok(y), "depth_to_space: bad arguments");
    const int64_t total = (int64_t)N * H * W * Cout;
    hipLaunchKernelGGL(depth_to_space_kernel, dim3(ew_grid(total)), dim3(EW_BLOCK), 0, (hipStream_t)stream, x.ptr, x.ctot,
                       x.coff, y.ptr, y.ctot, y.coff, N, H, W, Cout);
    return tnr_check_launch("depth_to_space");
}

extern "C" int tnr_space_to_depth_bwd(tnr_view gy, tnr_view gx, int32_t N, int32_t H, int32_t W, int32_t Cout, tnr_view mask,
                                      float mslope, void *stream) {
    TNR_REQUIRE(view_ok(gy) && view_ok(gx), "space_to_depth_bwd: bad arguments");
    const int64_t total = (int64_t)N * H * W * Cout;
    hipLaunchKernelGGL(space_to_depth_bwd_kernel, dim3(ew_grid(total)), dim3(EW_BLOCK), 0, (hipStream_t)stream, gy.ptr, gy.ctot,
                       gy.coff, gx.ptr, gx.ctot, gx.coff, N, H, W, Cout, mask.ptr, mask.ctot, mask.coff, mslope);
    return tnr_check_launch("space_to_depth_bwd");
}

extern "C" int tnr_maxpool2_fwd(tnr_view x, tnr_view y, int32_t N, int32_t H, int32_t W, int32_t C, void *stream) {
    TNR_REQUIRE(view_ok(x) && view_ok(y) && (C % 4) == 0 && (H % 2) == 0 && (W % 2) == 0, "maxpool2_fwd: bad arguments");
    const int64_t total = (int64_t)N * (H / 2) * (W / 2) * (C / 4);
    hipLaunchKernelGGL(maxpool2_fwd_kernel, dim3(ew_grid(total)), dim3(EW_BLOCK), 0, (hipStream_t)stream, x.ptr, x.ctot, x.coff,
                       y.ptr, y.ctot, y.coff, N, H, W, C);
    return tnr_check_launch("maxpool2_fwd");
}

extern "C" int tnr_maxpool2_bwd(tnr_view gy, tnr_view x, tnr_view gx, int32_t N, int32_t H, int32_t W, int32_t C,
                                void *stream) {
    TNR_REQUIRE(view_ok(gy) && view_ok(x) && view_ok(gx) && (C % 4) == 0 && (H % 2) == 0 && (W % 2) == 0, "maxpool2_bwd: bad arguments");
    const int64_t total = (int64_t)N * (H / 2) * (W / 2) * (C / 4);
    hipLaunchKernelGGL(maxpool2_bwd_kernel, dim3(ew_grid(total)), dim3(EW_BLOCK), 0, (hipStream_t)stream, gy.ptr, gy.ctot,
                       gy.coff, x.ptr, x.ctot, x.coff, gx.ptr, gx.ctot, gx.coff, N, H, W, C);
    return tnr_check_launch("maxpool2_bwd");
}

extern "C" int tnr_im2col(tnr_view x, int32_t N, int32_t H, int32_t W, int32_t C, int32_t k, int32_t stride, int32_t pad,
                          int32_t Ho, int32_t Wo, float *out, void *stream) {
    TNR_REQUIRE(view_ok(x) && out != nullptr && (C % 4) == 0 && k >= 1 && stride >= 1 && pad >= 0, "im2col: bad arguments");
    TNR_REQUIRE(Ho == (H + 2 * pad - k) / stride + 1 && Wo == (W + 2 * pad - k) / stride + 1, "im2col: output size mismatch");
    const int64_t total = (int64_t)N * Ho * Wo * k * k * (C / 4);
    hipLaunchKernelGGL(im2col_kernel, dim3(ew_grid(total)), dim3(EW_BLOCK), 0, (hipStream_t)stream, x.ptr, x.ctot, x.coff, N, H, W,
                       C, k, stride, pad, Ho, Wo, out);
    return tnr_check_launch("im2col");
}

extern "C" int tnr_axpby(tnr_view dst, tnr_view src, int64_t pixels, int32_t C, float a, float b, void *stream) {
    TNR_REQUIRE(view_ok(dst) && view_ok(src) && (C % 4) == 0, "axpby: bad arguments");
    hipLaunchKernelGGL(axpby_kernel, dim3(ew_grid(pixels * (C / 4))), dim3(EW_BLOCK), 0, (hipStream_t)stream, dst.ptr, dst.ctot,
                       dst.coff, src.ptr, src.ctot, src.coff, pixels, C, a, b);
    return tnr_check_launch("axpby");
}

extern "C" int tnr_gauss_mult(tnr_view dst, tnr_view src, int64_t pixels, int32_t C, float sigma, uint32_t key0, uint32_t key1,
                              uint32_t pix0, void *stream) {
    TNR_REQUIRE(view_ok(dst) && (src.ptr == nullptr || view_ok(src)) && (C % 4) == 0 && pixels >= 0, "gauss_mult: bad arguments");
    if (pixels == 0) return TNR_OK;
    hipLaunchKernelGGL(gauss_mult_kernel, dim3(ew_grid(pixels * (C / 4))), dim3(EW_BLOCK), 0, (hipStream_t)stream, dst.ptr, dst.ctot,
                       dst.coff, src.ptr, src.ctot, src.coff, pixels, C, sigma, key0, key1, pix0);
    return tnr_check_launch("gauss_mult");
}

extern "C" int tnr_mask_mul(tnr_view g, tnr_view y, int64_t pixels, int32_t C, float mslope, void *stream) {
    TNR_REQUIRE(view_ok(g) && view_ok(y) && (C % 4) == 0, "mask_mul: bad arguments");
    hipLaunchKernelGGL(mask_mul_kernel, dim3(ew_grid(pixels * (C / 4))), dim3(EW_BLOCK), 0, (hipStream_t)stream, g.ptr, g.ctot,
                       g.coff, y.ptr, y.ctot, y.coff, pixels, C, mslope);
    return tnr_check_launch("mask_mul");
}

extern "C" int tnr_bilinear2x_fwd(tnr_view x, tnr_view y, int32_t N, int32_t H, int32_t W, int32_t C, void *stream) {
    TNR_REQUIRE(view_ok(x) && view_ok(y) && (C % 4) == 0 && H >= 1 && W >= 1, "bilinear2x_fwd: bad arguments");
    const int64_t total = (int64_t)N * 4 * H * W * (C / 4);
    hipLaunchKernelGGL(bilinear2x_fwd_kernel, dim3(ew_grid(total)), dim3(EW_BLOCK), 0, (hipStream_t)stream, x.ptr, x.ctot, x.coff,
                       y.ptr, y.ctot, y.coff, N, H, W, C);
    return tnr_check_launch("bilinear2x_fwd");
}

extern "C" int tnr_bilinear2x_bwd(tnr_view gy, tnr_view gx, tnr_view gz, tnr_view mask, float mslope, int32_t N, int32_t H,
                                  int32_t W, int32_t C, void *stream) {
    TNR_REQUIRE(view_ok(gy) && (gx.ptr == nullptr || view_ok(gx)) && (gz.ptr == nullptr || (view_ok(gz) && view_ok(mask))) &&
                    (gx.ptr != nullptr || gz.ptr != nullptr) && (C % 4) == 0,
                "bilinear2x_bwd: bad arguments");
    const int64_t total = (int64_t)N * H * W * (C / 4);
    hipLaunchKernelGGL(bilinear2x_bwd_kernel, dim3(ew_grid(total)), dim3(EW_BLOCK), 0, (hipStream_t)stream, gy.ptr, gy.ctot, gy.coff,
                       gx.ptr, gx.ctot, gx.coff, gz.ptr, gz.ctot, gz.coff, mask.ptr, mask.ctot, mask.coff, mslope, N, H, W, C);
    return tnr_check_launch("bilinear2x_bwd");
}

extern "C" int tnr_add2(tnr_view dst, tnr_view a, tnr_view b, int64_t pixels, int32_t C, void *stream) {
    TNR_REQUIRE(view_ok(dst) && view_ok(a) && view_ok(b) && (C % 4) == 0, "add2: bad arguments");
    hipLaunchKernelGGL(add2_kernel, dim3(ew_grid(pixels * (C / 4))), dim3(EW_BLOCK), 0, (hipStream_t)stream, dst.ptr, dst.ctot,
                       dst.coff, a.ptr, a.ctot, a.coff, b.ptr, b.ctot, b.coff, pixels, C);
    return tnr_check_launch("add2");
}

extern "C" int tnr_mask_copy(tnr_view dst, tnr_view src, tnr_view y, int64_t pixels, int32_t C, float mslope, void *stream) {
    TNR_REQUIRE(view_ok(dst) && view_ok(src) && view_ok(y) && (C % 4) == 0, "mask_copy: bad arguments");
    hipLaunchKernelGGL(mask_copy_kernel, dim3(ew_grid(pixels * (C / 4))), dim3(EW_BLOCK), 0, (hipStream_t)stream, dst.ptr, dst.ctot,
                       dst.coff, src.ptr, src.ctot, src.coff, y.ptr, y.ctot, y.coff, pixels, C, mslope);
    return tnr_check_launch("mask_copy");
}

extern "C" int tnr_fill(float *p, int64_t n, float v, void *stream) {
    TNR_REQUIRE(p != nullptr && n >= 0, "fill: bad arguments");
    if (n == 0) return TNR_OK;
    hipLaunchKernelGGL(fill_kernel, dim3(ew_grid(n)), dim3(EW_BLOCK), 0, (hipStream_t)stream, p, n, v);
    return tnr_check_launch("fill");
}
```

trainner_amd/engine.py:

```python
import torch

from . import hip, ops
from .flat import FlatParams


class ConvOp:

    def __init__(self, mod, packer, need_dgrad=True, ups=False):
        self.mod, self.packer = mod, packer
        k, s = mod.kernel_size, mod.stride
        if k == 3 and s == 1:
            self.mode_f = ops.CONV_3x3_UP2 if ups else ops.CONV_3x3
            self.mode_d = ops.CONV_3x3
            pf, pd = ops.PACK_FWD, ops.PACK_DGRAD_3x3
        elif k == 4 and s == 2 and not ups:
            self.mode_f, self.mode_d = ops.CONV_4x4_S2, ops.DGRAD_4x4_S2
            pf, pd = ops.PACK_FWD_S2D, ops.PACK_DGRAD_S2
        else:
            raise NotImplementedError("conv k=%d s=%d is not on the SR hot path" % (k, s))
        self.i_f = packer.add(mod.weight, pf)
        self.i_d = packer.add(mod.weight, pd) if need_dgrad else None
        self.ups = ups
        self.i_uf = packer.add(mod.weight, ops.PACK_UP2_DGRAD_S2) if ups else None
        self.i_ud = packer.add(mod.weight, ops.PACK_UP2_FWD_S2D) if (ups and need_dgrad) else None
        deep = mod.in_channels * k * k >= 2048 and not ups
        i_fc = packer.add(mod.weight, ops.PACK_COL_FWD) if deep else None
        i_dc = packer.add(mod.weight, ops.PACK_COL_DGRAD3) if (deep and need_dgrad and k == 3) else None
        img = k == 3 and s == 1 and not ups
        self.thin = img
        i_f4 = packer.add(mod.weight, ops.PACK_C4_FWD) if (img and mod.in_channels <= 4) else None
        i_d4 = packer.add(mod.weight, ops.PACK_C4_DGRAD3) if (img and need_dgrad and mod.out_channels <= 4) else None
        cin, cout = mod.in_channels, mod.out_channels
        self.dirs = {False: (self.mode_f, ops.ConvLayer(k, s, cin, cout, False, ups, direct=self.i_f, c4=i_f4, col=i_fc)),
                     True: (self.mode_d, ops.ConvLayer(k, s, cin, cout, True, ups, direct=self.i_d, c4=i_d4, col=i_dc))}

    def _run(self, dgrad, x, y, epi):
        mode, layer = self.dirs[dgrad]
        wp = self.packer.get(layer.direct)
        form = ops.conv_plan(x, wp, y, mode, epi, layer=layer)[0]
        if form == "thin":
            ops.conv_thin(x, self.mod.weight, y, bias=None if dgrad else self.mod.bias, alpha=epi.get("alpha", 1.0), dgrad=dgrad)
        elif form == "c4":
            ops.conv(x if x.C == 4 else ops.View(x.buf), self.packer.get(layer.c4), y, mode=ops.CONV_3x3_C4, **epi)
        elif form == "im2col":
            ops.conv_small(x, self.packer.get(layer.col), y, layer.k, layer.stride, **epi)
        else:
            ops.conv(x, wp, y, mode=mode, **epi)

    def fwd(self, x, y, **epi):
        epi["bias"] = self.mod.bias
        self._run(False, x, y, epi)

    def fwd_up2(self, x, y, **epi):
        if "fwd" not in ops.upconv_plan(x)[0]:
            return self.fwd(x, y, **epi)
        ops.conv(x, self.packer.get(self.i_uf), y, mode=ops.DGRAD_4x4_S2, family=ops.UPFOLD_FAMILY, bias=self.mod.bias, **epi)

    def fwd_shuffle2(self, x, y, **epi):
        return ops.conv_shuffle2(x, self.packer.get(self.i_f), y, layer=self.dirs[False][1], bias=self.mod.bias, **epi)

    def dgrad(self, g, gx, **epi):
        self._run(True, g, gx, epi)

    def dgrad_up2(self, g, gx, mask=None, m_slope=0.2):
        if "dgrad" in ops.upconv_plan(gx)[0]:
            epi = dict(mask=mask, m_slope=m_slope) if mask is not None else {}
            ops.conv(g, self.packer.get(self.i_ud), gx, mode=ops.CONV_4x4_S2, family=ops.UPFOLD_FAMILY, **epi)
            return
        gup = ops.View(ops.new_act(g.N, g.H, g.W, gx.C, g.buf.device))
        self.dgrad(g, gup)
        ops.upsample2x_bwd(gup, gx, mask=mask, mslope=m_slope)

    def _wgrad_up2_folded(self, x, g, alpha, with_bias):
        w, b = self.mod.weight, self.mod.bias
        cout, cin = w.shape[0], w.shape[1]
        n = cin * cout * 16
        dws = ops.WS.get("upfold_dw@%x" % hip.stream(), n * 4, x.buf.device).view(torch.float32)[:n].view(cin, cout, 4, 4)
        ops.wgrad_group([dict(x=g, g=x, dw=dws, db=None, alpha=1.0, beta=0.0)], mode=ops.CONV_4x4_S2, family=ops.UPFOLD_FAMILY)
        ops.upconv_wgrad_unfold(dws, w.grad, alpha=alpha, beta=1.0)
        if with_bias and b is not None:
            ops.bias_grad(g, b.grad, alpha=alpha, beta=1.0)

    def fwd_stage(self, x, y, fresh_from=None, **epi):
        return dict(x=x, wp=self.packer.get(self.i_f), y=y, mode=self.mode_f, bias=self.mod.bias, fresh_from=fresh_from, **epi)

    def wgrad_item(self, x, g, alpha=1.0, cin_begin=0, with_bias=True, reflect=False):
        w = self.mod.weight
        db = self.mod.bias.grad if (with_bias and self.mod.bias is not None and cin_begin == 0) else None
        return dict(x=x, g=g, dw=w.grad, db=db, cin_begin=cin_begin, alpha=alpha, beta=1.0, reflect=reflect)

    def wgrad(self, x, g, alpha=1.0, cin_begin=0, with_bias=True, reflect=False):
        if self.ups and cin_begin == 0 and not reflect and "wgrad" in ops.upconv_plan(x)[0]:
            self._wgrad_up2_folded(x, g, alpha, with_bias)
            return
        if reflect:
            ops.wgrad_group([self.wgrad_item(x, g, alpha, cin_begin, with_bias, reflect=True)], mode=self.mode_f)
            return
        if self.thin and ops.IMAGE_C4 and cin_begin == 0 and x.N == g.N and (x.H, x.W) == (g.H, g.W):
            m = self.mod
            db = m.bias.grad if (with_bias and m.bias is not None) else None
            if m.in_channels <= 3 and x.ctot == 4 and x.coff == 0 and g.C in (16, 32, 64):
                ops.wgrad_thin(g, ops.View(x.buf), m.weight.grad, db, flip=False, alpha=alpha)
                return
            if m.out_channels <= 3 and g.ctot == 4 and g.coff == 0 and x.C in (16, 32, 64):
                ops.wgrad_thin(x, ops.View(g.buf), m.weight.grad, db, flip=True, alpha=alpha)
                return
        ops.wgrad_group([self.wgrad_item(x, g, alpha, cin_begin, with_bias)], mode=self.mode_f)


class _NetFn(torch.autograd.Function):

    @staticmethod
    def forward(ctx, net, x, *params):
        need_param_grad = any(ctx.needs_input_grad[2:])
        need_graph = ctx.needs_input_grad[1] or need_param_grad
        memo = net._memo_lookup(x) if (net.memoize and net.training) else None
        if memo is not None and memo[1] is not None:
            out, saved = memo
            net.replay_forward_side_effects(saved)
            out = out.detach()
        else:
            out, saved = net.engine_forward(x, save=need_graph or (net.memoize and net.training))
            if net.memoize and net.training:
                net._memo_store(x, out, saved)
        ctx.net, ctx.saved, ctx.need_param_grad = net, (saved if need_graph else None), need_param_grad
        return out

    @staticmethod
    def backward(ctx, gout):
        saved = ctx.saved
        if saved is None:
            raise RuntimeError("HIP engine: backward through a forward that saved no activations")
        ctx.saved = None
        sched = getattr(ctx.net, "_bucket_schedule", None)
        if sched is not None and ctx.need_param_grad:
            sched.begin_pass()
        gx = ctx.net.engine_backward(saved, gout, need_input_grad=ctx.needs_input_grad[1],
                                     need_param_grad=ctx.need_param_grad)
        return (None, gx) + (None,) * (len(ctx.needs_input_grad) - 2)


class HipNet(torch.nn.Module):

    memoize = False

    def _memo_key(self, x):
        fp = self.flat_params()
        return (fp.version, fp.flat._version), (x.data_ptr(), tuple(x.shape), tuple(x.stride()), x._version)

    def _memo_lookup(self, x):
        ver, key = self._memo_key(x)
        if self._memo_ver != ver:
            self._memo, self._memo_ver = {}, ver
        hit = self._memo.get(key)
        return None if hit is None else (hit[1], hit[2])

    def _memo_store(self, x, out, saved):
        ver, key = self._memo_key(x)
        if self._memo_ver != ver:
            self._memo, self._memo_ver = {}, ver
        self._memo[key] = (x.detach(), out, saved)

    def memo_clear(self):
        self._memo = {}

    def replay_forward_side_effects(self, saved):
        """Hook: what a repeated training-mode forward would change besides its outputs (BatchNorm running statistics)."""

    def _init_engine(self):
        self._memo, self._memo_ver = {}, None
        self._flat = FlatParams(self)
        self._packer = None
        self._dense_packer = None
        self._packer_owner = None
        self._packed_version = None
        self._ops = None
        self.register_load_state_dict_post_hook(lambda module, incompatible: module._flat.touch())

    def flat_params(self):
        return self._flat.ensure()

    def _refresh_derived(self):
        """Hook: tensors derived from the parameters that the packer reads (zero-extended taps, ...) are rebuilt here,
        right before the weights are re-packed."""

    def _prepare(self, x):
        hip.require_device(x)
        if x.dtype != torch.float32:
            raise hip.HipEngineError("the HIP engine computes in fp32; got %s" % x.dtype)
        fp = self.flat_params()
        if fp.flat.device != x.device:
            raise hip.HipEngineError("network is on %s but input on %s" % (fp.flat.device, x.device))
        if self._packer is None or self._packer.device != x.device or self._packer_owner is not fp.flat:
            self._packer = ops.WeightPacker(x.device)
            self._dense_packer = ops.DensePacker(x.device)
            self._packer_owner = fp.flat
            self._packed_version = None
            self._build_ops(self._packer)
        key = (fp.version, fp.flat._version)
        if self._packed_version != key:
            self._refresh_derived()
            self._packer.run()
            self._dense_packer.run()
            self._packed_version = key

    def forward(self, x, **kw):
        x = x.contiguous()
        self._prepare(x)
        params = list(self.parameters())
        return _NetFn.apply(self, x, *params)
```

trainner_amd/hip.py:

```python
import ctypes as C
import os

import torch

from . import build as _build

c_f = C.c_float
c_i = C.c_int32
c_l = C.c_int64
c_p = C.c_void_p

ACT_NONE, ACT_LRELU, ACT_RELU = 0, 1, 2
MMA_F32, MMA_BF16, MMA_BF16X3 = 0, 1, 2
CONV_3x3, CONV_3x3_UP2, CONV_4x4_S2, DGRAD_4x4_S2, CONV_1x1, CONV_3x3_C4, CONV_7x7_C4 = 0, 1, 2, 3, 4, 5, 6
PACK_FWD, PACK_DGRAD_3x3, PACK_FWD_S2D, PACK_DGRAD_S2, PACK_COL_FWD, PACK_COL_DGRAD3 = 0, 1, 2, 3, 4, 5
PACK_C4_FWD, PACK_C4_DGRAD3 = 6, 7
PACK_UP2_DGRAD_S2, PACK_UP2_FWD_S2D = 8, 9
PACK_DENSE_DGRAD = 16


class CView(C.Structure):
    _fields_ = [("ptr", c_p), ("ctot", c_i), ("coff", c_i)]


class ConvDesc(C.Structure):
    _fields_ = [
        ("x", CView), ("N", c_i), ("H", c_i), ("W", c_i), ("Cin", c_i),
        ("wp", c_p), ("KinP", c_i), ("KoutP", c_i),
        ("y", CView), ("Ho", c_i), ("Wo", c_i), ("Cout", c_i),
        ("mode", c_i), ("bias", c_p), ("act", c_i), ("slope", c_f), ("alpha", c_f),
        ("r1", CView), ("r1_ch", c_i), ("beta1", c_f),
        ("r2", CView), ("alpha2", c_f),
        ("m", CView), ("m_lo", c_i), ("m_hi", c_i), ("m_slope", c_f),
        ("ws", c_p), ("ws_bytes", c_l), ("mma", c_i), ("pad_mode", c_i),
        ("noise_sigma", c_f), ("noise_pos", c_i), ("noise_key0", C.c_uint32), ("noise_key1", C.c_uint32), ("noise_pix0", C.c_uint32),
        ("wq", c_p), ("wq_bytes", c_l), ("wq_form", c_i), ("shuffle", c_i),
    ]


class WgradDesc(C.Structure):
    _fields_ = [
        ("x", CView), ("N", c_i), ("H", c_i), ("W", c_i), ("Cin", c_i),
        ("g", CView), ("Ho", c_i), ("Wo", c_i), ("Cout", c_i),
        ("mode", c_i),
        ("dw", c_p), ("cin_total", c_i), ("cin_begin", c_i),
        ("db", c_p), ("alpha", c_f), ("beta", c_f),
        ("ws", c_p), ("ws_bytes", c_l), ("mma", c_i), ("pad_mode", c_i),
        ("dw2", c_p), ("cout_split", c_i), ("cin_total2", c_i), ("db2", c_p),
    ]


class SweepPackItem(C.Structure):
    _fields_ = [("units", c_i), ("reserved", c_i), ("opaque", C.c_uint64 * 15)]


class PackItem(C.Structure):
    _fields_ = [("w", c_p), ("wp", c_p), ("Cout", c_i), ("Cin", c_i), ("kh", c_i), ("kw", c_i),
                ("kind", c_i), ("KoutP", c_i), ("KinP", c_i), ("n_out", c_l)]


class DensePackItem(C.Structure):
    _fields_ = [("w", c_p * 5), ("wp", c_p), ("nf", c_i), ("gc", c_i), ("t", c_i), ("KoutP", c_i), ("KinP", c_i),
                ("scale5", c_f), ("n_out", c_l)]


_SIGS = {
    "tnr_last_error": (C.c_char_p, []),
    "tnr_version": (c_i, []),
    "tnr_pack_dims": (c_i, [c_i, c_i, c_i, c_i, c_i, C.POINTER(c_i), C.POINTER(c_i), C.POINTER(c_l)]),
    "tnr_pack_weights": (c_i, [c_p, c_i, c_l, c_p]),
    "tnr_upconv_fold_table": (c_i, [C.POINTER(c_i * 144)]),
    "tnr_upconv_wgrad_unfold": (c_i, [c_p, c_p, c_i, c_i, c_f, c_f, c_p]),
    "tnr_pack_dense_dims": (c_i, [c_i, c_i, c_i, C.POINTER(c_i), C.POINTER(c_i), C.POINTER(c_l)]),
    "tnr_pack_dense_dgrad": (c_i, [c_p, c_i, c_l, c_p]),
    "tnr_conv_forward": (c_i, [C.POINTER(ConvDesc), c_p]),
    "tnr_conv_workspace_bytes": (c_l, [C.POINTER(ConvDesc)]),
    "tnr_conv_wq_bytes": (c_l, [C.POINTER(ConvDesc)]),
    "tnr_conv_wq_pack": (c_i, [C.POINTER(ConvDesc), c_p, c_l, c_p]),
    "tnr_conv_wino_bytes": (c_l, [C.POINTER(ConvDesc)]),
    "tnr_conv_wino_pack": (c_i, [C.POINTER(ConvDesc), c_p, c_l, c_p]),
    "tnr_gauss_mult": (c_i, [CView, CView, c_l, c_i, c_f, C.c_uint32, C.c_uint32, C.c_uint32, c_p]),
    "tnr_im2col": (c_i, [CView, c_i, c_i, c_i, c_i, c_i, c_i, c_i, c_i, c_i, c_p, c_p]),
    "tnr_conv_chain_workspace_bytes": (c_l, [C.POINTER(ConvDesc)]),
    "tnr_conv_chain": (c_i, [C.POINTER(ConvDesc), C.POINTER(C.c_int32), c_i, c_p, c_l, C.c_uint32, c_p]),
    "tnr_conv_sweep_image_bytes": (c_l, [C.POINTER(ConvDesc), c_i]),
    "tnr_conv_sweep_pack_item": (c_i, [C.POINTER(ConvDesc), c_i, c_p, c_l, C.POINTER(SweepPackItem)]),
    "tnr_conv_sweep_pack_batch": (c_i, [c_p, c_i, c_i, c_p]),
    "tnr_conv_sweep_pack": (c_i, [C.POINTER(ConvDesc), c_i, c_p, c_l, c_p]),
    "tnr_conv_sweep": (c_i, [C.POINTER(ConvDesc), c_i, c_p, c_p, c_l, C.c_uint32, c_p]),
    "tnr_conv_thin_pack_floats": (c_l, [c_i]),
    "tnr_conv_thin_pack": (c_i, [c_p, c_p, c_i, c_i, c_i, c_p]),
    "tnr_conv_thin": (c_i, [CView, c_i, c_i, c_i, c_i, c_p, CView, c_i, c_p, c_f, c_p]),
    "tnr_wgrad_workspace_bytes": (c_l, [C.POINTER(WgradDesc)]),
    "tnr_conv_thin7_pack_floats": (c_l, [c_i]),
    "tnr_conv_thin7_pack": (c_i, [c_p, c_p, c_i, c_i, c_i, c_p]),
    "tnr_conv_thin7": (c_i, [CView, c_i, c_i, c_i, c_i, c_p, CView, c_i, c_i, c_i, c_i, c_i, c_p, c_f, c_p]),
    "tnr_wgrad_thin7_workspace_bytes": (c_l, [c_i, c_i, c_i]),
    "tnr_wgrad_thin7": (c_i, [CView, c_i, c_i, c_i, c_i, CView, c_i, c_i, c_i, c_i, c_i, c_i, c_p, c_p, c_f, c_f, c_p, c_l, c_p]),
    "tnr_wgrad_thin_workspace_bytes": (c_l, [c_i, c_i, c_i]),
    "tnr_wgrad_thin": (c_i, [CView, CView, c_i, c_i, c_i, c_i, c_i, c_i, c_p, c_p, c_f, c_f, c_p, c_l, c_p]),
    "tnr_conv_wgrad": (c_i, [C.POINTER(WgradDesc), c_p]),
    "tnr_conv_wgrad_group": (c_i, [C.POINTER(WgradDesc), c_i, c_p]),
    "tnr_wgrad_tile_class": (c_i, [C.POINTER(WgradDesc), c_i, c_i, C.POINTER(c_i * 12)]),
    "tnr_nchw_to_nhwc": (c_i, [c_p, c_i, c_i, c_i, c_i, CView, c_i, c_p, c_p, c_p]),
    "tnr_nhwc_to_nchw": (c_i, [CView, c_i, c_i, c_i, c_i, c_p, c_p, c_i, c_p]),
    "tnr_upsample2x_bwd": (c_i, [CView, CView, c_i, c_i, c_i, c_i, CView, c_f, c_p]),
    "tnr_depth_to_space": (c_i, [CView, CView, c_i, c_i, c_i, c_i, c_p]),
    "tnr_space_to_depth_bwd": (c_i, [CView, CView, c_i, c_i, c_i, c_i, CView, c_f, c_p]),
    "tnr_maxpool2_fwd": (c_i, [CView, CView, c_i, c_i, c_i, c_i, c_p]),
    "tnr_maxpool2_bwd": (c_i, [CView, CView, CView, c_i, c_i, c_i, c_i, c_p]),
    "tnr_gconv_fwd": (c_i, [CView, c_i, c_i, c_i, c_i, c_p, c_p, CView, c_i, c_i, c_i, c_i, c_i, c_i, c_i, c_i, c_f, c_p]),
    "tnr_gconv_dgrad": (c_i, [CView, c_i, c_i, c_i, c_i, c_p, CView, c_i, c_i, c_i, c_i, c_i, c_i, c_i, c_p]),
    "tnr_gconv_wgrad_workspace_bytes": (c_l, [c_i, c_i, c_i]),
    "tnr_gconv_wgrad": (c_i, [CView, c_i, c_i, c_i, c_i, CView, c_i, c_i, c_i, c_i, c_i, c_i, c_i, c_p, c_p, c_f, c_f, c_p, c_l, c_p]),
    "tnr_bias_grad": (c_i, [CView, c_l, c_i, c_p, c_f, c_f, c_p, c_l, c_p]),
    "tnr_pad2d": (c_i, [CView, CView, c_i, c_i, c_i, c_i, c_i, c_i, c_p]),
    "tnr_unpad2d": (c_i, [CView, CView, c_i, c_i, c_i, c_i, c_i, c_i, c_p]),
    "tnr_window2d": (c_i, [CView, c_i, c_i, CView, c_i, c_i, c_i, c_i, c_i, c_i, c_i, c_p]),
    "tnr_tanh_fwd": (c_i, [c_p, c_p, c_l, c_p]),
    "tnr_tanh_bwd": (c_i, [c_p, c_p, c_p, c_l, c_p]),
    "tnr_gan_loss": (c_i, [c_p, c_l, c_i, c_f, c_p, c_p, c_p]),
    "tnr_dp_unique_id": (c_i, [c_p]),
    "tnr_dp_init": (c_i, [c_p, c_i, c_i, C.POINTER(c_p)]),
    "tnr_dp_allreduce_bucket": (c_i, [c_p, c_p, c_l, c_i, c_p]),
    "tnr_dp_broadcast": (c_i, [c_p, c_p, c_l, c_i, c_p]),
    "tnr_dp_comm_count": (c_i, [c_p, C.POINTER(c_i)]),
    "tnr_dp_finalize": (c_i, [c_p]),
    "tnr_filter2d": (c_i, [c_p, c_p, c_p, c_i, c_i, c_i, c_i, c_p]),
    "tnr_resize": (c_i, [c_p, c_p, c_i, c_i, c_i, c_i, c_i, c_i, c_p]),
    "tnr_noise_gaussian": (c_i, [c_p, c_i, c_i, c_i, c_i, c_p, c_p, C.c_uint64, c_i, c_p]),
    "tnr_noise_poisson": (c_i, [c_p, c_i, c_i, c_i, c_i, c_p, c_p, c_p, C.c_uint64, c_i, c_p]),
    "tnr_jpeg_workspace_bytes": (c_l, [c_i, c_i, c_i]),
    "tnr_jpeg_sim": (c_i, [c_p, c_i, c_i, c_i, c_p, c_p, c_l, c_p]),
    "tnr_feed_u8_to_tensor": (c_i, [c_p, c_i, c_i, c_i, c_i, c_p, c_i, c_p, c_i, c_f, c_i, c_p]),
    "tnr_tensor2np_u8": (c_i, [c_p, c_i, c_i, c_i, c_i, c_p, c_i, c_i, c_p]),
    "tnr_metrics_workspace_bytes": (c_l, [c_i]),
    "tnr_psnr_ssim_u8": (c_i, [c_p, c_p, c_i, c_i, c_i, c_i, c_i, c_i, c_p, c_p, c_l, c_p]),
    "tnr_lpips_stem_dims": (c_i, [c_i, c_i, c_i, C.POINTER(c_i), C.POINTER(c_i)]),
    "tnr_lpips_stem": (c_i, [c_p, c_p, c_i, c_i, c_i, c_i, c_i, c_i, c_i, c_p, c_p, c_p, c_p, CView, c_p]),
    "tnr_maxpool3s2_ceil_dims": (c_i, [c_i, c_i, C.POINTER(c_i), C.POINTER(c_i)]),
    "tnr_maxpool3s2_ceil_fwd": (c_i, [CView, CView, c_i, c_i, c_i, c_i, c_p]),
    "tnr_lpips_workspace_bytes": (c_l, [c_i, c_i]),
    "tnr_lpips_head": (c_i, [CView, CView, c_i, c_i, c_i, c_i, c_p, c_i, c_i, c_p, c_l, c_p]),
    "tnr_lpips_finalize": (c_i, [c_i, c_i, c_p, c_l, c_p, c_p, c_p]),
    "tnr_bilinear2x_fwd": (c_i, [CView, CView, c_i, c_i, c_i, c_i, c_p]),
    "tnr_bilinear2x_bwd": (c_i, [CView, CView, CView, CView, c_f, c_i, c_i, c_i, c_i, c_p]),
    "tnr_add2": (c_i, [CView, CView, CView, c_l, c_i, c_p]),
    "tnr_mask_copy": (c_i, [CView, CView, CView, c_l, c_i, c_f, c_p]),
    "tnr_axpby": (c_i, [CView, CView, c_l, c_i, c_f, c_f, c_p]),
    "tnr_mask_mul": (c_i, [CView, CView, c_l, c_i, c_f, c_p]),
    "tnr_fill": (c_i, [c_p, c_l, c_f, c_p]),
    "tnr_bn_workspace_bytes": (c_l, [c_i]),
    "tnr_bn_train_fwd": (c_i, [CView, CView, c_l, c_i, c_p, c_p, c_p, c_p, c_p, c_f, c_f, c_p, c_p, c_i, c_f, c_p, c_p]),
    "tnr_bn_train_fwd_stats": (c_i, [CView, CView, c_l, c_i, c_p, c_p, c_p, c_p, c_p, c_f, c_f, c_p, c_p, c_p, c_i, c_f, c_p, c_p]),
    "tnr_bn_replay_running": (c_i, [c_p, c_p, c_p, c_p, c_i, c_f, c_p]),
    "tnr_bn_train_bwd": (c_i, [CView, CView, CView, CView, c_l, c_i, c_p, c_p, c_p, c_f, c_p, c_p, c_f, c_p, c_p]),
    "tnr_bn_train_bwd_z": (c_i, [CView, CView, CView, c_l, c_i, c_p, c_p, c_p, c_p, c_f, c_p, c_p, c_f, c_p, c_p]),
    "tnr_instnorm_workspace_bytes": (c_l, [c_i, c_i]),
    "tnr_instnorm_fwd": (c_i, [CView, CView, c_i, c_l, c_i, c_f, c_p, c_p, c_i, c_f, c_p, c_p]),
    "tnr_instnorm_bwd": (c_i, [CView, CView, CView, CView, c_i, c_l, c_i, c_p, c_p, c_f, c_p, c_p]),
    "tnr_linear_fwd": (c_i, [c_p, c_p, c_p, c_p, c_i, c_i, c_i, c_i, c_f, c_p]),
    "tnr_linear_bwd": (c_i, [c_p, c_p, c_p, c_p, c_f, c_p, c_p, c_p, c_i, c_i, c_i, c_f, c_p, c_p]),
    "tnr_reduce_workspace_bytes": (c_l, []),
    "tnr_l1_mean_fwd": (c_i, [c_p, c_p, c_l, c_f, c_p, c_p, c_p]),
    "tnr_l1_mean_bwd": (c_i, [c_p, c_p, c_l, c_f, c_p, c_p, c_i, c_p]),
    "tnr_ragan_phase_a": (c_i, [c_p, c_p, c_i, c_p, c_p, c_p]),
    "tnr_ragan_phase_b": (c_i, [c_p, c_p, c_i, c_i, c_p, c_p, c_p]),
    "tnr_ragan_phase_c": (c_i, [c_p, c_p, c_i, c_i, c_f, c_p, c_p, c_p, c_p, c_p]),
    "tnr_scale_by": (c_i, [c_p, c_p, c_l, c_p, c_p]),
    "tnr_ssim_workspace_bytes": (c_l, [c_i, c_i, c_i, c_i, c_i, c_i]),
    "tnr_ssim_fwd": (c_i, [c_p, c_p, c_i, c_i, c_i, c_i, c_i, c_i, C.POINTER(c_f), c_i, c_f, c_f, c_p, c_p, c_l, c_p]),
    "tnr_ssim_bwd": (c_i, [c_p, c_p, c_i, c_i, c_i, c_i, c_i, c_i, C.POINTER(c_f), c_i, c_f, c_f, c_p, c_p, c_p, c_i, c_p]),
    "tnr_avgpool2_pad_dims": (c_i, [c_i, c_i, c_i, C.POINTER(c_i), C.POINTER(c_i)]),
    "tnr_avgpool2_pad_fwd": (c_i, [c_p, c_p, c_i, c_i, c_i, c_i, c_i, c_i, c_p, c_p, c_p]),
    "tnr_avgpool2_pad_bwd": (c_i, [c_p, c_p, c_i, c_i, c_i, c_i, c_i, c_i, c_p]),
    "tnr_msssim_combine": (c_i, [c_p, c_i, c_i, C.POINTER(c_l), C.POINTER(c_f), c_i, c_p, c_p, c_p]),
    "tnr_imgloss_workspace_bytes": (c_l, [c_i, c_i, c_i, c_i]),
    "tnr_filter_loss_fwd": (c_i, [c_p, c_p, c_i, c_i, c_i, c_i, c_i, C.POINTER(c_f), c_i, c_i, C.c_double, c_p, c_p, c_p, c_l, c_p]),
    "tnr_filter_loss_bwd": (c_i, [c_p, c_i, c_i, c_i, c_i, c_i, C.POINTER(c_f), c_i, C.c_double, c_p, c_p, c_i, c_p]),
    "tnr_fd_loss_fwd": (c_i, [c_p, c_p, c_i, c_i, c_i, c_i, c_i, c_i, c_i, C.c_double, c_p, c_p, c_l, c_p]),
    "tnr_fd_loss_bwd": (c_i, [c_p, c_p, c_i, c_i, c_i, c_i, c_i, c_i, c_i, C.c_double, c_p, c_p, c_i, c_p]),
    "tnr_pointwise_loss_fwd": (c_i, [c_p, c_p, c_l, c_i, C.c_double, c_p, c_p, c_p]),
    "tnr_pointwise_loss_bwd": (c_i, [c_p, c_p, c_l, c_i, C.c_double, c_p, c_p, c_i, c_p]),
    "tnr_overflow_loss_fwd": (c_i, [c_p, c_l, C.c_double, c_p, c_p, c_p]),
    "tnr_overflow_loss_bwd": (c_i, [c_p, c_l, C.c_double, c_p, c_p, c_i, c_p]),
    "tnr_pooled_workspace_bytes": (c_l, []),
    "tnr_pooled_forward_blocks": (c_i, [c_i, c_i]),
    "tnr_pool_loss_fwd": (c_i, [c_p, c_p, c_i, c_i, c_i, c_i, c_i, c_i, c_i, c_i, c_p, c_p, c_l, c_p]),
    "tnr_pool_loss_bwd": (c_i, [c_p, c_p, c_i, c_i, c_i, c_i, c_i, c_i, c_i, c_i, c_p, c_p, c_i, c_p]),
    "tnr_multiscale_loss_fwd": (c_i, [c_p, c_p, c_i, c_i, c_i, c_i, c_i, c_i, c_p, c_p, c_l, c_p]),
    "tnr_multiscale_loss_bwd": (c_i, [c_p, c_p, c_i, c_i, c_i, c_i, c_i, c_i, c_p, c_p, c_i, c_p]),
    "tnr_spl_workspace_bytes": (c_l, [c_i, c_i, c_i, c_i, c_i]),
    "tnr_spl_coef_bytes": (c_l, [c_i, c_i, c_i, c_i, c_i]),
    "tnr_spl_loss_fwd": (c_i, [c_p, c_p, c_i, c_i, c_i, c_i, c_i, c_i, c_i, c_p, c_p, c_p, c_l, c_p]),
    "tnr_spl_loss_bwd": (c_i, [c_p, c_p, c_i, c_i, c_i, c_i, c_i, c_i, c_i, c_p, c_p, c_p, c_i, c_p]),
    "tnr_freqsep_low": (c_i, [c_p, c_i, c_i, c_i, c_i, c_i, C.POINTER(c_f), c_p, c_p, c_i, c_p]),
    "tnr_freqsep_high_fwd": (c_i, [c_p, c_i, c_i, c_i, c_i, c_i, C.POINTER(c_f), c_p, c_p]),
    "tnr_freqsep_high_bwd": (c_i, [c_p, c_p, c_i, c_i, c_i, c_i, c_i, C.POINTER(c_f), c_p, c_p, c_i, c_p]),
    "tnr_diffaug_workspace_bytes": (c_l, [c_i]),
    "tnr_diffaug_mean": (c_i, [c_p, c_i, c_i, c_i, c_i, c_i, c_p, C.POINTER(c_i), c_i, c_p, c_l, c_p]),
    "tnr_diffaug_fwd": (c_i, [c_p, c_i, c_i, c_i, c_i, c_i, c_p, C.POINTER(c_i), c_p, c_p, c_p]),
    "tnr_diffaug_bwd": (c_i, [c_p, c_i, c_i, c_i, c_i, c_i, c_p, C.POINTER(c_i), c_p, c_p, c_p]),
    "tnr_batchaug_mix": (c_i, [c_p, c_p, c_p, c_p, c_i, c_i, c_i, c_i, c_i, C.POINTER(c_i), c_f, c_f, c_p, c_p]),
    "tnr_batchaug_mask": (c_i, [c_p, c_p, c_i, c_i, c_i, c_i, c_i, c_i, c_p, c_p]),
    "tnr_gram_workspace_bytes": (c_l, [c_i, c_i, c_i, c_i]),
    "tnr_gram_fwd": (c_i, [CView, c_i, c_i, c_i, c_i, c_f, c_i, c_p, c_p, c_l, c_p]),
    "tnr_gram_bwd": (c_i, [CView, c_p, c_i, c_i, c_i, c_i, c_f, c_i, CView, c_i, c_p]),
    "tnr_cx_sums_workspace_bytes": (c_l, [c_i, c_i, c_i]),
    "tnr_cx_sums": (c_i, [CView, c_i, c_i, c_i, c_i, c_p, c_i, c_p, c_p, c_l, c_p]),
    "tnr_cx_prepare": (c_i, [CView, c_i, c_i, c_i, c_i, c_p, c_i, c_p, c_p, c_p, c_p]),
    "tnr_cx_matrix_bytes": (c_l, [c_i, c_i]),
    "tnr_cx_distance": (c_i, [c_p, c_p, c_i, c_i, c_i, c_i, c_p, c_p]),
    "tnr_cx_rows": (c_i, [c_p, c_i, c_i, c_f, c_f, c_p, c_p, c_p, c_p, c_p]),
    "tnr_cx_finalize": (c_i, [c_p, c_i, c_i, c_p, c_p, c_p, c_p, c_p, c_p]),
    "tnr_cx_grad_rows": (c_i, [c_p, c_p, c_p, c_i, c_i, c_i, c_f, c_p, c_p, c_p, c_p, c_p, c_p, c_p]),
    "tnr_cx_grad_gemm": (c_i, [c_p, c_p, c_i, c_i, c_i, c_i, c_p, c_p]),
    "tnr_cx_norm_bwd": (c_i, [c_p, c_p, c_p, c_i, c_i, c_i, c_i, c_i, c_p, CView, c_p]),
    "tnr_sumsq": (c_i, [c_p, c_l, c_p, c_p, c_p]),
    "tnr_clip_by_norm": (c_i, [c_p, c_l, c_p, c_f, c_p]),
    "tnr_adam_step": (c_i, [c_p, c_p, c_p, c_p, c_l, c_f, C.c_double, C.c_double, c_f, c_f, c_f, c_p]),
    "tnr_adam_step_guarded": (c_i, [c_p, c_p, c_p, c_p, c_l, c_f, C.c_double, C.c_double, c_f, c_f, c_f, c_p, c_p]),
    "tnr_optim_workspace_bytes": (c_l, [c_i, c_l]),
    "tnr_sgd_step_guarded": (c_i, [c_p, c_p, c_p, c_p, c_i, c_f, c_f, c_f, c_p, c_p]),
    "tnr_rmsprop_step_guarded": (c_i, [c_p, c_p, c_p, c_p, c_i, c_f, C.c_double, c_f, c_f, c_p, c_p]),
    "tnr_madgrad_step_guarded": (c_i, [c_p, c_p, c_p, c_p, c_p, c_p, c_i, c_f, c_f, c_f, c_f, c_i, C.c_double, c_p, c_p]),
    "tnr_adamp_step_guarded": (c_i, [c_p, c_p, c_p, c_p, c_p, c_i, c_p, c_i, c_p, c_l, c_p, c_l, c_f, C.c_double, C.c_double, c_f, c_f,
                                     c_i, C.c_double, c_f, c_f, c_f, c_p, c_p]),
    "tnr_sgdp_step_guarded": (c_i, [c_p, c_p, c_p, c_p, c_i, c_p, c_i, c_p, c_l, c_p, c_l, c_f, c_f, C.c_double, c_f, c_i, C.c_double,
                                    c_f, c_f, c_f, c_p, c_p]),
    "tnr_ranger_step_guarded": (c_i, [c_p, c_p, c_p, c_p, c_p, c_p, c_i, c_p, c_i, c_p, c_l, c_p, c_l, c_i, C.c_double, C.c_double,
                                      c_f, c_f, c_f, c_i, c_i, c_f, c_p, c_p]),
    "tnr_set_fault_word": (c_i, [c_p]),
}

EXPORTS = tuple(_SIGS)
_lib = None


class HipEngineError(RuntimeError):
    pass


def library_path():
    return os.environ.get("TNR_HIP_LIB") or _build.LIB


ABI_VERSION = 3


def load(build_if_missing=False):
    global _lib
    if _lib is not None:
        return _lib
    path = library_path()
    if not os.path.exists(path):
        if build_if_missing:
            _build.build()
        else:
            raise HipEngineError(
                "libtrainner_hip.so not found at %s -- run `python -m trainner_amd.build` "
                "(the engine has no CPU / eager fallback)" % path)
    lib = C.CDLL(path)
    for name, (res, args) in _SIGS.items():
# ... 38 lines not shown
```

trainner_amd/models/modules/architectures/perceptual.py:

```python
import logging
import os

import torch
import torch.nn as nn

from .... import ops
from ....engine import ConvOp, HipNet
from ....ops import View, new_act
from . import block as B

logger = logging.getLogger("base")

VGG_CFG = {
    "vgg16": [64, 64, "M", 128, 128, "M", 256, 256, 256, "M", 512, 512, 512, "M", 512, 512, 512, "M"],
    "vgg19": [64, 64, "M", 128, 128, "M", 256, 256, 256, 256, "M", 512, 512, 512, 512, "M", 512, 512, 512, 512, "M"],
}


def vgg_layer_names(net):
    names, blk, idx = [], 1, 1
    for v in VGG_CFG[net]:
        if v == "M":
            names.append("pool%d" % blk)
            blk, idx = blk + 1, 1
        else:
            names += ["conv%d_%d" % (blk, idx), "relu%d_%d" % (blk, idx)]
            idx += 1
    return names


TORCHVISION_FILES = {"vgg11": "vgg11-8a719046.pth", "vgg13": "vgg13-19584684.pth", "vgg16": "vgg16-397923af.pth", "vgg19": "vgg19-dcbb9e9d.pth"}


class FeatureExtractor(HipNet):
    def __init__(self, listen_list=None, net="vgg19", use_input_norm=True, z_norm=False, requires_grad=False,
                 remove_pooling=False, pooling_stride=2, change_padding=False, load_path=None, allow_random_init=False):
        super().__init__()
        for opt_name, on in (("remove_pooling", remove_pooling), ("change_padding", change_padding), ("requires_grad", requires_grad),
                             ("z_norm", z_norm)):
            if on:
                raise NotImplementedError("FeatureExtractor option '%s' is not implemented by the HIP engine" % opt_name)
        if net not in VGG_CFG or pooling_stride != 2:
            raise NotImplementedError("FeatureExtractor net=%r / pooling_stride=%r is not implemented by the HIP engine" % (net, pooling_stride))
        listen_list = list(listen_list or ["conv5_4"])
        names = vgg_layer_names(net)
        unknown = [v for v in listen_list if v not in names]
        if unknown:
            raise ValueError("FeatureExtractor(%s): unknown layer name(s) %s" % (net, ", ".join(map(str, unknown))))
        self.listen_list = set(listen_list)
        self.use_input_norm = use_input_norm
        last = max(names.index(v) for v in listen_list)
        self.names = names[:last + 1]
        self.taps = [n for n in self.names if n in self.listen_list]
        self._single = len(self.taps) == 1 and self.taps[0].startswith("conv")
        self.listen = self.taps[0] if self._single else None
        layers, c, chans = nn.ModuleDict(), 3, iter([v for v in VGG_CFG[net] if v != "M"])
        for n in self.names:
            if n.startswith("conv"):
                v = next(chans)
                layers[n] = B.Conv2dHIP(c, v, 3, 1)
                c = v
            else:
                layers[n] = B.Marker(n)
        self.feature_net = layers
        self.out_channels = c
        if use_input_norm:
            self.register_buffer("mean", torch.tensor([[[0.485]], [[0.456]], [[0.406]]]))
            self.register_buffer("std", torch.tensor([[[0.229]], [[0.224]], [[0.225]]]))
        self.weights_source = self._load_pretrained(net, load_path, allow_random_init)
        for p in self.parameters():
            p.requires_grad = False
        self.eval()
        self._init_engine()
        self._norm = None

    def _load_pretrained(self, net, load_path, allow_random_init):
        if load_path and os.path.exists(load_path):
            self.load_torchvision_state(torch.load(load_path, map_location="cpu", weights_only=False))
            return load_path
        why = "pretrained_path %r does not exist" % load_path if load_path else "no perceptual_opt.pretrained_path given"
        try:
            from torchvision.models import vgg as tv_vgg
            self.load_torchvision_state(getattr(tv_vgg, net)(pretrained=True).state_dict())
            return "torchvision:%s" % net
        except Exception as e:
            why += "; torchvision pretrained weights unavailable (%s: %s)" % (type(e).__name__, e)
        cached = os.path.join(torch.hub.get_dir(), "checkpoints", TORCHVISION_FILES.get(net, ""))
        if os.path.isfile(cached):
            self.load_torchvision_state(torch.load(cached, map_location="cpu", weights_only=False))
            return cached
        why += "; no cached %s" % cached
        if not allow_random_init:
            from ....hip import HipEngineError
            raise HipEngineError("FeatureExtractor(%s): %s. A perceptual loss on randomly initialised features is refused; "
                                 "set train.perceptual_opt.pretrained_path to a torchvision %s state_dict, or opt in with "
                                 "train.perceptual_allow_random_init: true (benchmarks / parity tests that load their own "
                                 "weights)" % (net, why, net))
        logger.warning("FeatureExtractor(%s): %s -- weights left at their random init (allow_random_init)", net, why)
        return "random-init"

    def load_torchvision_state(self, sd):
        own = self.state_dict()
        for i, n in enumerate(self.names):
            if n.startswith("conv"):
                own["feature_net.%s.weight" % n].copy_(sd["features.%d.weight" % i])
                own["feature_net.%s.bias" % n].copy_(sd["features.%d.bias" % i])

    def _build_ops(self, packer):
        self._ops = {n: ConvOp(self.feature_net[n], packer) for n in self.names if n.startswith("conv")}

    def _norm_consts(self, dev):
        if self._norm is None or self._norm[0].device != dev:
            if self.use_input_norm:
                mean = [float(v) for v in self.mean.reshape(3).cpu().tolist()]
                std = [float(v) for v in self.std.reshape(3).cpu().tolist()]
                scale = torch.tensor([1.0 / s for s in std], dtype=torch.float32).to(dev)
                shift = torch.tensor([-m / s for m, s in zip(mean, std)], dtype=torch.float32).to(dev)
            else:
                scale = torch.ones(3).to(dev)
                shift = torch.zeros(3).to(dev)
            self._norm = (scale, shift)
        return self._norm

    def engine_forward(self, x, save):
        N, Cc, H, W = x.shape
        if Cc != 3:
            raise ValueError("FeatureExtractor expects RGB input")
        dev = x.device
        scale, shift = self._norm_consts(dev)
        x4 = View(new_act(N, H, W, 4, dev))
        ops.nchw_to_nhwc(x, x4, Cpad=4, scale=scale, shift=shift)
        cur, tape = x4, []
        for n in self.names:
            if n.startswith("conv"):
                y = View(new_act(N, cur.H, cur.W, self.feature_net[n].out_channels, dev))
                if n == self.listen:
                    self._ops[n].fwd(cur, y)
                else:
                    self._ops[n].fwd(cur, y, act=ops.ACT_RELU)
                tape.append((n, cur, y))
                cur = y
            elif n.startswith("pool"):
                y = View(new_act(N, cur.H // 2, cur.W // 2, cur.C, dev))
                ops.maxpool2_fwd(cur, y)
                tape.append((n, cur, y))
                cur = y
        out = cur.buf.permute(0, 3, 1, 2)
        return out, (dict(tape=tape, in_shape=(N, H, W)) if save else None)

    def engine_backward(self, sv, gout, need_input_grad, need_param_grad):
        if not need_input_grad:
            return None
        tape = sv["tape"]
        N, H, W = sv["in_shape"]
        dev = gout.device
        g_nhwc = gout.permute(0, 2, 3, 1)
        if not g_nhwc.is_contiguous():
            g_nhwc = g_nhwc.contiguous()
        g = View(g_nhwc)
        for i in range(len(tape) - 1, -1, -1):
            n, xin, y = tape[i]
            gx = View(new_act(N, xin.H, xin.W, xin.C, dev))
            if n.startswith("pool"):
                ops.maxpool2_bwd(g, xin, gx)
            else:
                prev = tape[i - 1][0] if i > 0 else None
                if prev is not None and prev.startswith("conv"):
                    self._ops[n].dgrad(g, gx, mask=xin, m_slope=0.0)
                else:
                    self._ops[n].dgrad(g, gx)
            g = gx
        scale, _ = self._norm_consts(dev)
        out = torch.empty((N, 3, H, W), dtype=torch.float32, device=dev)
        ops.nhwc_to_nchw(View(g.buf, 0, 3), out, scale=scale)
        return out

    def engine_forward_taps(self, x, save):
        N, Cc, H, W = x.shape
        if Cc != 3:
            raise ValueError("FeatureExtractor expects RGB input")
        dev = x.device
        scale, shift = self._norm_consts(dev)
        x4 = View(new_act(N, H, W, 4, dev))
        ops.nchw_to_nhwc(x, x4, Cpad=4, scale=scale, shift=shift)
        cur, tape, feats = x4, [], {}
        for i, n in enumerate(self.names):
            if n.startswith("conv"):
                y = View(new_act(N, cur.H, cur.W, self.feature_net[n].out_channels, dev))
                if n not in self.listen_list:
                    self._ops[n].fwd(cur, y, act=ops.ACT_RELU)
                else:
                    self._ops[n].fwd(cur, y)
                    feats[n] = y
                    if i + 1 < len(self.names):
                        post = View(new_act(N, y.H, y.W, y.C, dev))
                        ops.mask_copy(post, y, y, mslope=0.0)
                        y = post
                tape.append((n, cur, y))
                cur = y
            elif n.startswith("pool"):
                y = View(new_act(N, cur.H // 2, cur.W // 2, cur.C, dev))
                ops.maxpool2_fwd(cur, y)
                tape.append((n, cur, y))
                cur = y
                if n in self.listen_list:
                    feats[n] = y
            elif n in self.listen_list:
                feats[n] = cur
        outs = tuple(feats[n].buf.permute(0, 3, 1, 2) for n in self.taps)
        return outs, (dict(tape=tape, in_shape=(N, H, W)) if save else None)

    @staticmethod
    def _grad_view(g):
        g_nhwc = g.permute(0, 2, 3, 1)
        return View(g_nhwc if g_nhwc.is_contiguous() else g_nhwc.contiguous())

    def _inject(self, entry, tg, g):
        n, _, y = entry
        dev = y.buf.device

        def add(g, t):
            if g is None:
                return t
            if any(g is v for v in tg.values()):
                s = View(new_act(y.N, y.H, y.W, y.C, dev))
                ops.add2(s, g, t)
                return s
            ops.axpby(g, t, 1.0, 1.0)
            return g

        if n.startswith("pool"):
            return add(g, tg[n]) if tg.get(n) is not None else g
        tr = tg.get("relu" + n[4:])
        if tr is not None:
            m = View(new_act(y.N, y.H, y.W, y.C, dev))
            ops.mask_copy(m, tr, y, mslope=0.0)
            g = m if g is None else add(g, m)
        if tg.get(n) is not None:
            g = add(g, tg[n])
        return g

    def engine_backward_taps(self, sv, gouts):
        tape = sv["tape"]
        N, H, W = sv["in_shape"]
        tg = {n: self._grad_view(g) for n, g in zip(self.taps, gouts) if g is not None}
        dev = tape[0][1].buf.device
        g = self._inject(tape[-1], tg, None)
        for i in range(len(tape) - 1, -1, -1):
            n, xin, y = tape[i]
            if g is not None:
                gx = View(new_act(N, xin.H, xin.W, xin.C, dev))
                if n.startswith("pool"):
                    ops.maxpool2_bwd(g, xin, gx)
                else:
                    prev = tape[i - 1][0] if i > 0 else None
                    if prev is not None and prev.startswith("conv"):
                        self._ops[n].dgrad(g, gx, mask=xin, m_slope=0.0)
                    else:
                        self._ops[n].dgrad(g, gx)
                g = gx
            if i > 0:
                g = self._inject(tape[i - 1], tg, g)
        out = torch.empty((N, 3, H, W), dtype=torch.float32, device=dev)
        if g is None:
            return out.zero_()
        scale, _ = self._norm_consts(dev)
        ops.nhwc_to_nchw(View(g.buf, 0, 3), out, scale=scale)
        return out

    def forward(self, x):
        if self._single:
            return {self.listen: super().forward(x)}
        x = x.contiguous()
        self._prepare(x)
        feats = _TapsFn.apply(self, x, *self.parameters())
        return dict(zip(self.taps, feats))


class _TapsFn(torch.autograd.Function):

    @staticmethod
    def forward(ctx, net, x, *params):
        ctx.set_materialize_grads(False)
        outs, saved = net.engine_forward_taps(x, save=ctx.needs_input_grad[1])
        ctx.net, ctx.saved = net, saved
        return outs

    @staticmethod
    def backward(ctx, *gouts):
        saved, ctx.saved = ctx.saved, None
        if saved is None:
            raise RuntimeError("HIP engine: backward through a forward that saved no activations")
        gx = ctx.net.engine_backward_taps(saved, gouts) if ctx.needs_input_grad[1] else None
        return (None, gx) + (None,) * (len(ctx.needs_input_grad) - 2)
```

trainner_amd/ops.py:

```python
import collections
import ctypes as C
import math
import os

import torch

from . import hip
from .hip import (ACT_LRELU, ACT_NONE, ACT_RELU, CONV_1x1, CONV_3x3, CONV_3x3_C4, CONV_3x3_UP2, CONV_4x4_S2, CONV_7x7_C4, DGRAD_4x4_S2,
                  PACK_C4_DGRAD3, PACK_C4_FWD, PACK_COL_DGRAD3, PACK_COL_FWD, PACK_DENSE_DGRAD, PACK_DGRAD_3x3, PACK_DGRAD_S2, PACK_FWD, PACK_FWD_S2D, PACK_UP2_DGRAD_S2,
                  PACK_UP2_FWD_S2D, CView,
                  ConvDesc,
                  DensePackItem, PackItem, WgradDesc)


def round_up(a, b):
    return (a + b - 1) // b * b


class View:
    __slots__ = ("buf", "coff", "C")

    def __init__(self, buf, coff=0, C=None):
        assert buf.dim() == 4 and buf.dtype == torch.float32 and buf.is_contiguous()
        self.buf, self.coff = buf, coff
# ... 265 lines not shown


def _stream_image(owner, attr, key, need, dev, pack):
    if owner is None:
        cache, gen, key = _ONEOFF_IMAGES[attr], None, (key, hip.stream())
    else:
        cache, gen = owner.__dict__.setdefault(attr, {}), owner.gen
    ent = cache.get(key)
    if owner is None and ent is not None:
        cache[key] = cache.pop(key)
    fresh = ent is None or ent[0].numel() * 4 < need
    if fresh:
        ent = cache[key] = [torch.empty(need // 4, dtype=torch.float32, device=dev), None]
        if owner is None:
            while len(cache) > 64:
                cache.pop(next(iter(cache)))
    if gen is None or ent[1] != gen:
        pack(ent[0].data_ptr(), need)
        ent[1] = gen
    return ent, fresh


def _wq_image(lib, d, wp, dev, tag=None):
    need = lib.tnr_conv_wq_bytes(C.byref(d))
    if need <= 0:
        return None
    key = wp.t.data_ptr() if tag is None else (tag, wp.t.data_ptr())
    return _stream_image(wp.owner, "_wq_images", key, need, dev,
                         lambda img, nb: hip.check(lib.tnr_conv_wq_pack(C.byref(d), img, nb, hip.stream()), "conv_wq_pack"))[0][0]


WINO = os.environ.get("TNR_WINO", "1") != "0"
WINO_MIN_CIN = int(os.environ.get("TNR_WINO_MIN_CIN", "64"))
WINO_MIN_PIXELS = int(os.environ.get("TNR_WINO_MIN_PIXELS", "4096"))


def _wino_image(lib, d, wp, dev):
    need = lib.tnr_conv_wino_bytes(C.byref(d))
    if need <= 0:
        return None
    return _stream_image(wp.owner, "_wq_images", ("wino", wp.t.data_ptr()), need, dev,
                         lambda img, nb: hip.check(lib.tnr_conv_wino_pack(C.byref(d), img, nb, hip.stream()), "conv_wino_pack"))[0][0]
SHUFFLE_FOLD = os.environ.get("TNR_SHUFFLE_FOLD", "1") != "0"
_LIVE = object()
ConvLayer = collections.namedtuple("ConvLayer", "k stride cin cout dgrad ups direct c4 col")
_STREAM_MMA = (hip.MMA_BF16X3, hip.MMA_BF16)
_FUSED = ("r1", "r2", "mask")
_CONV_FAMILY = {CONV_3x3: ("conv_tile_3x3", 9), CONV_3x3_UP2: ("conv_tile_3x3_up2", 9), CONV_4x4_S2: ("conv_tile_4x4s2", 16), DGRAD_4x4_S2: ("conv_tile_dgrad4x4s2", 4),
                CONV_1x1: ("conv_tile_1x1", 1), CONV_3x3_C4: ("conv_tile_3x3_c4", 9), CONV_7x7_C4: ("conv_tile_7x7_c4", 49)}


def conv_plan(x, wp, y, mode=CONV_3x3, epi=None, shuffle=0, layer=None, wino=None, mma=_LIVE, splitk=True, wino_ok=True, stream_ok=True):
    mma = MMA if mma is _LIVE else mma
    epi = epi or {}
    if shuffle:
        no = ((not (SHUFFLE_FOLD and X3_D4 and x.buf.is_cuda) and "switch")
              or (mma not in _STREAM_MMA and "arithmetic")
              or (layer is not None and (layer.k != 3 or layer.stride != 1 or layer.ups or layer.cout != 4 * y.C) and "shape")
              or ((wp.KoutP != 4 * y.C or y.H != 2 * x.H or y.W != 2 * x.W) and "shape")
              or (not stream_ok and "declined"))
        return ("tile", no) if no else ("stream", None)
    why = None
    if layer is not None:
        if layer.k == 3 and layer.stride == 1 and not layer.ups and (layer.cin if layer.dgrad else layer.cout) <= 4 and y.C <= 4:
            why = ((not IMAGE_C4 and "switch")
                   or ((any(epi.get(n) is not None for n in _FUSED) or epi.get("act", ACT_NONE) != ACT_NONE) and "epilogue"))
            if not why:
                return "thin", None
        if layer.c4 is not None and x.ctot == 4 and x.coff == 0:
            if IMAGE_C4:
                return "c4", why
            why = why or "switch"
        if layer.col is not None:
            no = ((not SMALL_GEMM and "switch")
                  or ((y.pixels > 4096 or y.pixels % 8 or x.C % 4) and "shape")
                  or ((any(epi.get(n) is not None for n in _FUSED) or epi.get("reflect")) and "epilogue"))
            if not no:
                return "im2col", why
            why = why or no
    if splitk and wp.KinP >= 512 and y.pixels <= 16384:
        return "tile", "splitk"
    if mode in (CONV_3x3_C4, CONV_7x7_C4):
        return "c4", why
    if mode == CONV_3x3:
        no = ((wino is False and "forbidden")
              or (wino is None and not WINO and "switch")
              or (wino is None and (x.C < WINO_MIN_CIN or y.pixels < WINO_MIN_PIXELS) and "shape")
              or (mma != hip.MMA_BF16X3 and "arithmetic")
              or (y.C % 64 and "shape")
              or (not wino_ok and "declined"))
        if not no:
            return "wino", why or ("forced" if wino else None)
        why = why or no
    if mode in (CONV_3x3, CONV_4x4_S2, DGRAD_4x4_S2):
        no = ((not (X3_D4 and (S2_D4 or mode == CONV_3x3)) and "switch")
              or (mma not in _STREAM_MMA and "arithmetic")
              or (y.C % 64 and "shape")
              or (not stream_ok and "declined"))
        if not no:
            return "stream", why
        why = why or no
    return "tile", why


def _conv_launch(x, wp, y, mode, wino, shuffle, epi, layer=None, family=None):
    d, said = None, {}
    while True:
        form, why = conv_plan(x, wp, y, mode, epi, shuffle, layer, wino, **said)
        if shuffle and form != "stream":
            return None
        if d is None:
            lib, d = hip.load(), ConvDesc()
            _conv_desc(d, x, wp, y, mode, **epi)
            if shuffle:
                d.Ho, d.Wo, d.Cout, d.shuffle, d.m_hi = x.H, x.W, 4 * y.C, shuffle, 0
        if why == "splitk":
            need = lib.tnr_conv_workspace_bytes(C.byref(d))
            if need > 0:
                ws = WS.get("splitk@%x" % hip.stream(), need, x.buf.device)
                d.ws, d.ws_bytes = ws.data_ptr(), ws.numel() * 8
                break
            said["splitk"] = False
        elif form == "wino":
            img = _wino_image(lib, d, wp, x.buf.device)
            if img is not None:
                d.wq, d.wq_bytes, d.wq_form = img.data_ptr(), img.numel() * 4, 1
                break
            assert wino is not True, "this launch cannot run in the Winograd form"
            said["wino_ok"] = False
        elif form == "stream":
            img = _wq_image(lib, d, wp, x.buf.device, tag="shuffle2" if shuffle else None)
            if img is not None:
                d.wq, d.wq_bytes = img.data_ptr(), img.numel() * 4
                break
            said["stream_ok"] = False
        else:
            break
    t0 = PROFILE.begin() if PROFILE is not None else None
    hip.check(lib.tnr_conv_forward(C.byref(d), hip.stream()), "conv_forward")
    if PROFILE is not None:
        fam, taps = _CONV_FAMILY[mode]
        PROFILE.end("conv_wino_3x3" if form == "wino" else (family or fam), 2.0 * d.N * d.Ho * d.Wo * taps * min(x.C, wp.KinP) * d.Cout, t0, (x.C, d.Cout, d.Ho, wp.kind))
    return form


def conv_shuffle2(x, wp, y, layer=None, **epi):
    return _conv_launch(x, wp, y, CONV_3x3, None, 2, epi, layer) is not None


def conv(x, wp, y, mode=CONV_3x3, wino=None, family=None, **epi):
    _conv_launch(x, wp, y, mode, wino, 0, epi, family=family)


UPFOLD_FAMILY = "conv_upfold"
UPFOLD_PASSES = ("fwd", "dgrad", "wgrad")
UPFOLD_TAPS = ((2,), (1, 2), (0, 1), (0,))
_UPFOLD_DEFAULT = ("dgrad", "wgrad")


def upconv_plan(x, mma=_LIVE, switch=_LIVE):
    sw = os.environ.get("TNR_UPCONV_FOLD", "1") if switch is _LIVE else str(switch)
    if sw == "0":
        return (), "switch"
    if (MMA if mma is _LIVE else mma) != hip.MMA_BF16X3:
        return (), "arithmetic"
    if not _on_device(x.buf):
        return (), "device"
    if sw == "1":
        return _UPFOLD_DEFAULT, None
    return tuple(p for p in UPFOLD_PASSES if p in sw.split(",")), None


def upconv_fold_table():
    out = (C.c_int32 * 144)()
    hip.check(hip.load().tnr_upconv_fold_table(C.byref(out)), "upconv_fold_table")
    return torch.tensor(list(out), dtype=torch.float64).view(16, 9)


def upconv_fold_weights(w):
    rows = []
    for ty in range(3):
        rows.append(torch.stack([w[..., ty, t[0]] if len(t) == 1 else w[..., ty, t[0]] + w[..., ty, t[1]] for t in UPFOLD_TAPS], dim=-1))
    return torch.stack([rows[t[0]] if len(t) == 1 else rows[t[0]] + rows[t[1]] for t in UPFOLD_TAPS], dim=-2)


def upconv_unfold_grad(dF):
    def row(ky):
        return torch.stack([dF[..., ky, 2 - tx] + dF[..., ky, 3 - tx] for tx in range(3)], dim=-1)
    return torch.stack([row(2 - ty) + row(3 - ty) for ty in range(3)], dim=-2)


def upconv_wgrad_unfold(dws, dw3, alpha=1.0, beta=1.0):
    Cout, Cin = dw3.shape[0], dw3.shape[1]
    assert tuple(dws.shape) == (Cin, Cout, 4, 4) and dws.is_contiguous() and dw3.is_contiguous()
    hip.check(hip.load().tnr_upconv_wgrad_unfold(dws.data_ptr(), dw3.data_ptr(), Cout, Cin, alpha, beta, hip.stream()), "upconv_wgrad_unfold")


CHAIN_MAX = 6
CONV_CHAIN = os.environ.get("TNR_CONV_CHAIN", "1") != "0"
CONV_SWEEP = os.environ.get("TNR_CONV_SWEEP", "1") != "0"
CHAIN_X3 = os.environ.get("TNR_CHAIN_X3", "1") == "1"
AMP_SWEEP = os.environ.get("TNR_AMP_SWEEP", "1") != "0"
SWEEP_DISPENSED = os.environ.get("TNR_SWEEP_WAVES", "4") != "8"
CHAIN_WITH_COLLECTIVES = os.environ.get("TNR_CHAIN_WITH_COLLECTIVES", "0") == "1"
SWEEP_AUTO = os.environ.get("TNR_SWEEP_AUTO", "1") != "0"
SWEEP_AUTO_STATE = {"choice": None, "sweep_us": None, "layers_us": None}
DENSE_SPLIT = os.environ.get("TNR_DENSE_SPLIT", "1") != "0"
_SWEEP_FORM_DMA = os.environ.get("TNR_SWEEP_FORM", "")[:2] == "dm"
COLLECTIVES_IN_FLIGHT = False
COUNTERS = {"one_launch_next_to_collectives": 0, "per_layer_next_to_collectives": 0}
_cu_counts = {}


def _cus(dev):
    if dev not in _cu_counts:
        _cu_counts[dev] = torch.cuda.get_device_properties(dev).multi_processor_count
    return _cu_counts[dev]


def _on_device(buf):
    return buf.is_cuda


def _crowded(in_flight):
    return in_flight and not CHAIN_WITH_COLLECTIVES


def _chain_mma(mma):
    return hip.MMA_F32 if mma == hip.MMA_BF16X3 and not CHAIN_X3 else mma


def _eligible(stages):
    return all(st.get("mode", CONV_3x3) == CONV_3x3 and st["y"].C % 32 == 0 and st["wp"].KoutP == st["y"].C for st in stages)


def _split_shape(stages):
    x0 = stages[0]["x"]
    if not all(st.get("mode", CONV_3x3) == CONV_3x3 and not st.get("reflect") and st["wp"].KoutP == st["y"].C and st["wp"].KinP == st["x"].C for st in stages) \
            or stages[4]["y"].C != 64 or any(st["y"].C != 32 for st in stages[:4]) or x0.C % 16 or x0.C < 32 or stages[4]["x"].C != x0.C + 128:
        return False
    return x0.H >= 8 and x0.W >= 8 and -(-x0.W // 32) * -(-x0.H // 8) <= _cus(x0.buf.device)


def dense_block_plan(stages, crowded=_LIVE, mma=_LIVE, choice=_LIVE, sweepable=True):
    n = 5 if stages is None else len(stages)
    mma = _chain_mma(MMA if mma is _LIVE else mma)
    x3 = mma == hip.MMA_BF16X3
    if not CONV_CHAIN:
        return "layers", "switch"
    if stages is not None and not _eligible(stages):
        return "layers", "shape"
    on_device = stages is None or _on_device(stages[0]["x"].buf)
    sweep = sweepable and CONV_SWEEP and ((n in (4, 5) and x3) or (n == 5 and mma == hip.MMA_BF16 and AMP_SWEEP))
    if sweep and x3 and on_device and SWEEP_AUTO and (SWEEP_AUTO_STATE["choice"] if choice is _LIVE else choice) == "layers":
        return "layers", "calibrated"
    crowded = _crowded(COLLECTIVES_IN_FLIGHT if crowded is _LIVE else crowded)
    dispensed = sweep and SWEEP_DISPENSED
    if crowded and not dispensed:
        return "layers", "crowded"
    if not sweep:
        return "chain", None
    if DENSE_SPLIT and dispensed and x3 and n == 5 and on_device and not crowded and not _SWEEP_FORM_DMA and stages is not None and _split_shape(stages):
        return "split", None
    return "sweep", None


def dense_split_applies(stages):
    return dense_block_plan(stages)[0] == "split"


def dense_block_form_applies(stages):
    return len(stages) == 5 and dense_block_plan(stages, mma=FP32_MMA, choice="layers") == ("layers", "calibrated")


def dense_blocks_overlap_collectives():
    return not _crowded(True) or dense_block_plan(None, crowded=True, choice=None)[0] != "layers"


def g_buckets_leave_in_backward():
    want = os.environ.get("TNR_DP_OVERLAP_G", "0")
    return want == "1" or (want == "auto" and dense_blocks_overlap_collectives())


SWEEP_PACK_BATCH = os.environ.get("TNR_SWEEP_PACK_BATCH", "0") != "0"


def _repack_sweep_images(owner):
    b = owner.__dict__.get("_sweep_batch")
    if not b or not SWEEP_PACK_BATCH:
        return
    if b["table"] is None:
        raw = b"".join(bytes(it) for it in b["items"])
        b["table"] = torch.frombuffer(bytearray(raw), dtype=torch.uint8).to(b["ents"][0][0].device)
    hip.check(hip.load().tnr_conv_sweep_pack_batch(b["table"].data_ptr(), len(b["items"]), b["max_units"], hip.stream()), "conv_sweep_pack_batch")
    for ent in b["ents"]:
        ent[1] = owner.gen


_chain_epoch = {}


def _sweep_image(lib, descs, n, stages, dev):
    need = lib.tnr_conv_sweep_image_bytes(descs, n)
    if need <= 0:
        return None
    owner = stages[0]["wp"].owner if all(st["wp"].owner is stages[0]["wp"].owner for st in stages) else None
# ... 171 lines not shown
    if PROFILE is not None:
        PROFILE.end("conv_thin", 2.0 * y.pixels * 9 * x.C * y.C, t0, (x.C, y.C, y.H, int(dgrad)))


def conv_thin7(x, w, y, pad=3, reflect=True, bias=None, alpha=1.0, dgrad=False):
    lib = hip.load()
    Cout, Cin = w.shape[0], w.shape[1]
    n = lib.tnr_conv_thin7_pack_floats(Cout if dgrad else Cin)
    wp = WS.get("thin7_w@%x" % hip.stream(), n * 4, x.buf.device)
    hip.check(lib.tnr_conv_thin7_pack(w.data_ptr(), wp.data_ptr(), Cout, Cin, int(dgrad), hip.stream()), "conv_thin7_pack")
    t0 = PROFILE.begin() if PROFILE is not None else None
    hip.check(lib.tnr_conv_thin7(x.c(), x.N, x.H, x.W, x.C, wp.data_ptr(), y.c(), y.H, y.W, y.C, pad, int(reflect), hip.ptr(bias), alpha,
                                 hip.stream()), "conv_thin7")
    if PROFILE is not None:
        PROFILE.end("conv_thin", 2.0 * y.pixels * 49 * x.C * y.C, t0, (x.C, y.C, y.H, 70 + int(dgrad)))


def wgrad_thin7(big, small4, dw, db, flip, rpad=0, off=0, alpha=1.0, beta=1.0):
    lib = hip.load()
    cs = dw.shape[0] if flip else dw.shape[1]
    need = lib.tnr_wgrad_thin7_workspace_bytes(big.N, big.H + 2 * rpad, big.C)
    ws = WS.get("wgrad_thin7@%x" % hip.stream(), need, big.buf.device)
    t0 = PROFILE.begin() if PROFILE is not None else None
    hip.check(lib.tnr_wgrad_thin7(big.c(), big.N, big.H, big.W, rpad, small4.c(), small4.H, small4.W, off, big.C, cs, int(flip),
                                  dw.data_ptr(), hip.ptr(db), alpha, beta, ws.data_ptr(), ws.numel() * 8, hip.stream()), "wgrad_thin7")
    if PROFILE is not None:
        PROFILE.end("wgrad_thin", 2.0 * big.N * (big.H + 2 * rpad) * (big.W + 2 * rpad) * 49 * big.C * cs, t0, (big.C, cs, big.H, 70 + int(flip)))


def conv_small(x, wp_col, y, k, stride, pad=1, **epi):
    M, K = y.pixels, k * k * x.C
    dev = x.buf.device
    col = WS.get("im2col@%x" % hip.stream(), M * K * 4, dev)
    hip.check(hip.load().tnr_im2col(x.c(), x.N, x.H, x.W, x.C, k, stride, pad, y.H, y.W, col.data_ptr(), hip.stream()), "im2col")
    wimg = 32 if M % 32 == 0 else (16 if M % 16 == 0 else 8)
    cimg = col.view(torch.float32)[:M * K].view(1, M // wimg, wimg, K)
    yimg = View(y.buf.view(1, M // wimg, wimg, y.ctot), y.coff, y.C)
    conv(View(cimg), wp_col, yimg, mode=CONV_1x1, **epi)


def conv_col(x, wp_col, y, k, stride=1, pad=1, **epi):
    K = k * k * x.C
    if K % 16 or K != wp_col.KinP:
        raise hip.HipEngineError("conv_col: k*k*C = %d must be a multiple of 16 and match the packed weights (%d)" % (K, wp_col.KinP))
    M = y.pixels
    col = WS.get("im2col@%x" % hip.stream(), M * K * 4, x.buf.device)
    hip.check(hip.load().tnr_im2col(x.c(), x.N, x.H, x.W, x.C, k, stride, pad, y.H, y.W, col.data_ptr(), hip.stream()), "im2col")
    conv(View(col.view(torch.float32)[:M * K].view(y.N, y.H, y.W, K)), wp_col, y, mode=CONV_1x1, **epi)


WGRAD_GROUP_MAX = 12
WGRAD_PAIR = os.environ.get("TNR_WGRAD_PAIR", "1") != "0"
WGRAD_X3 = os.environ.get("TNR_WGRAD_X3", "1") == "1"


def _wgrad_desc(d, x, g, dw, db, mode, cin_begin, alpha, beta, reflect=False, pair=None):
    d.x = x.c()
    d.N, d.H, d.W, d.Cin = x.N, x.H, x.W, x.C
    d.g = g.c()
    d.Ho, d.Wo, d.Cout = g.H, g.W, g.C
    d.mode = mode
    d.dw, d.cin_total, d.cin_begin = dw.data_ptr(), dw.shape[1], cin_begin
    d.db = hip.ptr(db)
    d.alpha, d.beta = alpha, beta
    d.mma = hip.MMA_F32 if (MMA == hip.MMA_BF16X3 and not WGRAD_X3) else MMA
    d.pad_mode = 1 if reflect else 0
    if pair is not None:
        dw2, db2, split = pair
        d.dw2, d.cin_total2, d.cout_split, d.db2 = dw2.data_ptr(), dw2.shape[1], split, hip.ptr(db2)


def wgrad(x, g, dw, db=None, mode=CONV_3x3, cin_begin=0, alpha=1.0, beta=1.0, reflect=False):
    wgrad_group([dict(x=x, g=g, dw=dw, db=db, cin_begin=cin_begin, alpha=alpha, beta=beta, reflect=reflect)], mode=mode)


def wgrad_group(items, mode=CONV_3x3, family=None):
    lib = hip.load()
    n = len(items)
    assert 1 <= n <= WGRAD_GROUP_MAX
    descs = (WgradDesc * n)()
    for d, it in zip(descs, items):
        _wgrad_desc(d, it["x"], it["g"], it["dw"], it.get("db"), mode, it.get("cin_begin", 0),
                    it.get("alpha", 1.0), it.get("beta", 1.0), it.get("reflect", False), it.get("pair"))
    dev = items[0]["x"].buf.device
    for i, d in enumerate(descs):
        need = lib.tnr_wgrad_workspace_bytes(C.byref(d))
        ws = WS.get("wgrad%d" % i, need, dev)
        d.ws, d.ws_bytes = ws.data_ptr(), ws.numel() * 8
    if PROFILE is None:
        hip.check(lib.tnr_conv_wgrad_group(descs, n, hip.stream()), "conv_wgrad_group")
        return
    t0 = PROFILE.begin()
    hip.check(lib.tnr_conv_wgrad_group(descs, n, hip.stream()), "conv_wgrad_group")
    taps = 16 if mode == CONV_4x4_S2 else 9
    x0, g0 = items[0]["x"], items[0]["g"]
    flops = sum(2.0 * it["g"].pixels * taps * it["x"].C * it["g"].C for it in items)
    PROFILE.end(family or "wgrad_tile", flops, t0, (sum(it["x"].C for it in items) if n > 1 else x0.C, g0.C, g0.H, mode + 100 * (n - 1)))


def wgrad_tile_class(desc, group_jobs=0, x3_occ=-1):
    out = (C.c_int32 * 12)()
    hip.check(hip.load().tnr_wgrad_tile_class(C.byref(desc), group_jobs, x3_occ, C.byref(out)), "wgrad_tile_class")
    return dict(zip(("mode", "a_t", "b_t", "thg", "bf", "wps", "db", "ks", "splits", "tiles_per_split", "lds", "row"), out))


def wgrad_thin(big, small4, dw, db, flip, alpha=1.0, beta=1.0):
    lib = hip.load()
    cs = dw.shape[0] if flip else dw.shape[1]
    need = lib.tnr_wgrad_thin_workspace_bytes(big.N, big.H, big.C)
    ws = WS.get("wgrad_thin@%x" % hip.stream(), need, big.buf.device)
    t0 = PROFILE.begin() if PROFILE is not None else None
    hip.check(lib.tnr_wgrad_thin(big.c(), small4.c(), big.N, big.H, big.W, big.C, cs, int(flip), dw.data_ptr(), hip.ptr(db),
                                 alpha, beta, ws.data_ptr(), ws.numel() * 8, hip.stream()), "wgrad_thin")
    if PROFILE is not None:
        PROFILE.end("wgrad_thin", 2.0 * big.pixels * 9 * big.C * cs, t0, (big.C, cs, big.H, int(flip)))


def nchw_to_nhwc(src, dst, Cpad=None, scale=None, shift=None):
    N, Cc, H, W = src.shape
    assert src.is_contiguous() and src.dtype == torch.float32
    hip.check(hip.load().tnr_nchw_to_nhwc(src.data_ptr(), N, Cc, H, W, dst.c(), dst.C if Cpad is None else Cpad,
                                          hip.ptr(scale), hip.ptr(shift), hip.stream()), "nchw_to_nhwc")


def nhwc_to_nchw(src, dst, scale=None, accumulate=False):
    N, Cc, H, W = dst.shape
    assert dst.is_contiguous() and dst.dtype == torch.float32
    hip.check(hip.load().tnr_nhwc_to_nchw(src.c(), N, Cc, H, W, dst.data_ptr(), hip.ptr(scale), int(accumulate),
                                          hip.stream()), "nhwc_to_nchw")


def upsample2x_bwd(gup, gx, mask=None, mslope=0.2):
    hip.check(hip.load().tnr_upsample2x_bwd(gup.c(), gx.c(), gx.N, gx.H, gx.W, gx.C, cv(mask), mslope, hip.stream()),
              "upsample2x_bwd")


def depth_to_space(x, y):
    hip.check(hip.load().tnr_depth_to_space(x.c(), y.c(), x.N, x.H, x.W, y.C, hip.stream()), "depth_to_space")


def space_to_depth_bwd(gy, gx, mask=None, mslope=0.2):
    hip.check(hip.load().tnr_space_to_depth_bwd(gy.c(), gx.c(), gx.N, gx.H, gx.W, gy.C, cv(mask), mslope, hip.stream()),
              "space_to_depth_bwd")


def maxpool2_fwd(x, y):
    hip.check(hip.load().tnr_maxpool2_fwd(x.c(), y.c(), x.N, x.H, x.W, x.C, hip.stream()), "maxpool2_fwd")


def maxpool2_bwd(gy, x, gx):
    hip.check(hip.load().tnr_maxpool2_bwd(gy.c(), x.c(), gx.c(), x.N, x.H, x.W, x.C, hip.stream()), "maxpool2_bwd")


def bilinear2x_fwd(x, y):
    hip.check(hip.load().tnr_bilinear2x_fwd(x.c(), y.c(), x.N, x.H, x.W, x.C, hip.stream()), "bilinear2x_fwd")


def bilinear2x_bwd(gy, gx=None, gz=None, mask=None, mslope=0.2):
    ref = gx if gx is not None else gz
    hip.check(hip.load().tnr_bilinear2x_bwd(gy.c(), cv(gx), cv(gz), cv(mask), mslope, ref.N, ref.H, ref.W, ref.C, hip.stream()),
              "bilinear2x_bwd")


def add2(dst, a, b):
    hip.check(hip.load().tnr_add2(dst.c(), a.c(), b.c(), dst.pixels, dst.C, hip.stream()), "add2")


def mask_copy(dst, src, y, mslope=0.2):
    hip.check(hip.load().tnr_mask_copy(dst.c(), src.c(), y.c(), dst.pixels, dst.C, mslope, hip.stream()), "mask_copy")


def gconv_fwd(x, w, y, bias=None, stride=1, pad=0, reflect=False, act=ACT_NONE, slope=0.2):
    Cout, Cin, k, _ = w.shape
    t0 = PROFILE.begin() if PROFILE is not None else None
    hip.check(hip.load().tnr_gconv_fwd(x.c(), x.N, x.H, x.W, Cin, w.data_ptr(), hip.ptr(bias), y.c(), y.H, y.W, Cout, k, stride, pad,
                                       int(reflect), act, slope, hip.stream()), "gconv_fwd")
    if PROFILE is not None:
        PROFILE.end("gconv", 2.0 * y.pixels * k * k * Cin * Cout, t0, (Cin, Cout, y.H, k))


def gconv_dgrad(g, w, gx, stride=1, pad=0, reflect=False):
    Cout, Cin, k, _ = w.shape
    t0 = PROFILE.begin() if PROFILE is not None else None
    hip.check(hip.load().tnr_gconv_dgrad(g.c(), gx.N, gx.H, gx.W, Cin, w.data_ptr(), gx.c(), g.H, g.W, Cout, k, stride, pad, int(reflect),
                                         hip.stream()), "gconv_dgrad")
    if PROFILE is not None:
        PROFILE.end("gconv", 2.0 * g.pixels * k * k * Cin * Cout, t0, (Cin, Cout, g.H, k + 100))


def gconv_wgrad(x, g, dw, db=None, stride=1, pad=0, reflect=False, alpha=1.0, beta=1.0):
    Cout, Cin, k, _ = dw.shape
    lib = hip.load()
    ws = WS.get("gconv_wgrad@%x" % hip.stream(), lib.tnr_gconv_wgrad_workspace_bytes(Cout, Cin, k), x.buf.device)
    t0 = PROFILE.begin() if PROFILE is not None else None
    hip.check(lib.tnr_gconv_wgrad(x.c(), x.N, x.H, x.W, Cin, g.c(), g.H, g.W, Cout, k, stride, pad, int(reflect), dw.data_ptr(), hip.ptr(db),
                                  alpha, beta, ws.data_ptr(), ws.numel() * 8, hip.stream()), "gconv_wgrad")
    if PROFILE is not None:
        PROFILE.end("gconv", 2.0 * g.pixels * k * k * Cin * Cout, t0, (Cin, Cout, g.H, k + 200))


def bias_grad(g, db, alpha=1.0, beta=1.0):
    ws = WS.get("bias_grad@%x" % hip.stream(), 512 * g.C * 8, g.buf.device)
    hip.check(hip.load().tnr_bias_grad(g.c(), g.pixels, g.C, db.data_ptr(), alpha, beta, ws.data_ptr(), ws.numel() * 8, hip.stream()), "bias_grad")


def pad2d(x, y, pad, reflect):
    hip.check(hip.load().tnr_pad2d(x.c(), y.c(), x.N, x.H, x.W, x.C, pad, int(reflect), hip.stream()), "pad2d")


def unpad2d(xp, y, pad, fold):
    hip.check(hip.load().tnr_unpad2d(xp.c(), y.c(), y.N, y.H, y.W, y.C, pad, int(fold), hip.stream()), "unpad2d")


def window2d(src, dst, oy, ox, acc=False):
    hip.check(hip.load().tnr_window2d(src.c(), src.H, src.W, dst.c(), dst.N, dst.H, dst.W, dst.C, oy, ox, int(acc), hip.stream()), "window2d")


def tanh_fwd(x, y):
    hip.check(hip.load().tnr_tanh_fwd(x.data_ptr(), y.data_ptr(), x.numel(), hip.stream()), "tanh_fwd")


def tanh_bwd(g, y, gx):
    hip.check(hip.load().tnr_tanh_bwd(g.data_ptr(), y.data_ptr(), gx.data_ptr(), g.numel(), hip.stream()), "tanh_bwd")


def gan_loss(pred, kind, target, out, grad=None):
    hip.check(hip.load().tnr_gan_loss(pred.data_ptr(), pred.numel(), kind, float(target), out.data_ptr(), hip.ptr(grad), hip.stream()), "gan_loss")


def axpby(dst, src, a=1.0, b=1.0):
    hip.check(hip.load().tnr_axpby(dst.c(), src.c(), dst.pixels, dst.C, a, b, hip.stream()), "axpby")


def mask_mul(g, y, mslope=0.2):
    hip.check(hip.load().tnr_mask_mul(g.c(), y.c(), g.pixels, g.C, mslope, hip.stream()), "mask_mul")


def fill(t, value=0.0):
    hip.check(hip.load().tnr_fill(t.data_ptr(), t.numel(), value, hip.stream()), "fill")


def bn_train_fwd(z, y, gamma, beta, running_mean, running_var, num_batches, save_mean, save_invstd,
                 momentum=0.1, eps=1e-5, act=ACT_LRELU, slope=0.2, stat64=None):
    lib = hip.load()
    ws = WS.get("bn", lib.tnr_bn_workspace_bytes(z.C), z.buf.device)
    hip.check(lib.tnr_bn_train_fwd_stats(z.c(), y.c(), z.pixels, z.C, gamma.data_ptr(), beta.data_ptr(),
                                         hip.ptr(running_mean), hip.ptr(running_var), hip.ptr(num_batches), momentum, eps,
                                         save_mean.data_ptr(), save_invstd.data_ptr(), hip.ptr(stat64), act, slope, ws.data_ptr(),
                                         hip.stream()), "bn_train_fwd")


def bn_replay_running(running_mean, running_var, num_batches, stat64, momentum=0.1):
    hip.check(hip.load().tnr_bn_replay_running(running_mean.data_ptr(), running_var.data_ptr(), hip.ptr(num_batches), stat64.data_ptr(),
                                               running_mean.numel(), momentum, hip.stream()), "bn_replay_running")


BN_MASK_FROM_Z = os.environ.get("TNR_BN_MASK_FROM_Z", "1") != "0"


def bn_train_bwd(gy, y, z, gz, gamma, save_mean, save_invstd, dgamma=None, dbeta=None, acc_beta=1.0, mslope=0.2, beta=None):
    lib = hip.load()
    ws = WS.get("bn", lib.tnr_bn_workspace_bytes(z.C), z.buf.device)
    if beta is not None and BN_MASK_FROM_Z:
        hip.check(lib.tnr_bn_train_bwd_z(gy.c(), z.c(), gz.c(), z.pixels, z.C, gamma.data_ptr(), beta.data_ptr(), save_mean.data_ptr(),
                                         save_invstd.data_ptr(), mslope, hip.ptr(dgamma), hip.ptr(dbeta), acc_beta, ws.data_ptr(),
                                         hip.stream()), "bn_train_bwd_z")
        return
    hip.check(lib.tnr_bn_train_bwd(gy.c(), y.c(), z.c(), gz.c(), z.pixels, z.C, gamma.data_ptr(),
                                   save_mean.data_ptr(), save_invstd.data_ptr(), mslope, hip.ptr(dgamma),
                                   hip.ptr(dbeta), acc_beta, ws.data_ptr(), hip.stream()), "bn_train_bwd")


def instnorm_fwd(z, y, save_mean, save_invstd, eps=1e-5, act=ACT_NONE, slope=0.0):
    lib = hip.load()
    ws = WS.get("instnorm", lib.tnr_instnorm_workspace_bytes(z.N, z.C), z.buf.device)
    hip.check(lib.tnr_instnorm_fwd(z.c(), y.c(), z.N, z.H * z.W, z.C, eps, save_mean.data_ptr(), save_invstd.data_ptr(), act, slope,
                                   ws.data_ptr(), hip.stream()), "instnorm_fwd")


def instnorm_bwd(gy, y, z, gz, save_mean, save_invstd, mslope=1.0):
    lib = hip.load()
    ws = WS.get("instnorm", lib.tnr_instnorm_workspace_bytes(z.N, z.C), z.buf.device)
    hip.check(lib.tnr_instnorm_bwd(gy.c(), y.c(), z.c(), gz.c(), z.N, z.H * z.W, z.C, save_mean.data_ptr(), save_invstd.data_ptr(),
                                   mslope, ws.data_ptr(), hip.stream()), "instnorm_bwd")


def linear_fwd(x, w, b, y, act=ACT_NONE, slope=0.2):
    N, In = x.shape
    Out = w.shape[0]
    hip.check(hip.load().tnr_linear_fwd(x.data_ptr(), w.data_ptr(), hip.ptr(b), y.data_ptr(), N, In, Out, act, slope,
                                        hip.stream()), "linear_fwd")


def linear_bwd(x, w, gy, yact=None, gx=None, dw=None, db=None, acc_beta=1.0, mslope=0.2):
    N, In = x.shape
    Out = w.shape[0]
    gpre = WS.get("lin", N * Out * 4, x.device)
    hip.check(hip.load().tnr_linear_bwd(x.data_ptr(), w.data_ptr(), gy.data_ptr(), hip.ptr(yact), mslope, hip.ptr(gx),
                                        hip.ptr(dw), hip.ptr(db), N, In, Out, acc_beta, gpre.data_ptr(), hip.stream()),
              "linear_bwd")


def _reduce_ws(dev):
    return WS.get("reduce@%x" % hip.stream(), hip.load().tnr_reduce_workspace_bytes(), dev)


# ... 408 lines not shown
```

Before: 73.01.

## Fuse 2x2 max-pool into Winograd conv epilogue for VGG feature extractor

Adds a pooled epilogue to the Winograd 3x3 kernel. For a VGG conv whose ReLU is followed by a maxpool, the kernel now writes only the pooled output plus a compact uint8 route map holding the argmax and ReLU sign. The backward pass uses a new unpool kernel driven by the route map instead of re-reading the full-resolution activation. This removes writing and re-reading the full-res pre-pool tensor and one kernel launch per pool stage. In exchange the conv epilogue gets more complex, and the path is restricted to the Winograd route with no residual, noise or shuffle.

```diff
diff --git a/include/trainner_hip.h b/include/trainner_hip.h
--- a/include/trainner_hip.h
+++ b/include/trainner_hip.h
@@ -123,6 +123,8 @@
 int tnr_conv_wq_pack(const tnr_conv_desc *d, void *image, int64_t image_bytes, void *stream);
 int64_t tnr_conv_wino_bytes(const tnr_conv_desc *d);
 int tnr_conv_wino_pack(const tnr_conv_desc *d, void *image, int64_t image_bytes, void *stream);
+int tnr_conv_pool_ok(const tnr_conv_desc *d);
+int tnr_conv_forward_pool2(const tnr_conv_desc *d, uint8_t *route, void *stream);
 int tnr_im2col(tnr_view x, int32_t N, int32_t H, int32_t W, int32_t C, int32_t k, int32_t stride, int32_t pad,
                int32_t Ho, int32_t Wo, float *out, void *stream);
 #define TNR_CHAIN_MAX 6
@@ -221,6 +223,7 @@
 int tnr_maxpool2_fwd(tnr_view x, tnr_view y, int32_t N, int32_t H, int32_t W, int32_t C, void *stream);
 int tnr_maxpool2_bwd(tnr_view gy, tnr_view x, tnr_view gx, int32_t N, int32_t H, int32_t W, int32_t C,
                      void *stream);
+int tnr_unpool2_bwd(tnr_view gy, const uint8_t *map, tnr_view gx, int32_t N, int32_t H, int32_t W, int32_t C, void *stream);
 int tnr_axpby(tnr_view dst, tnr_view src, int64_t pixels, int32_t C, float a, float b, void *stream);
 int tnr_mask_mul(tnr_view g, tnr_view y, int64_t pixels, int32_t C, float mslope, void *stream);
 int tnr_fill(float *p, int64_t n, float v, void *stream);
diff --git a/trainner_amd/csrc/conv_epilogue.h b/trainner_amd/csrc/conv_epilogue.h
--- a/trainner_amd/csrc/conv_epilogue.h
+++ b/trainner_amd/csrc/conv_epilogue.h
@@ -2,6 +2,28 @@
 #include "conv_body.h"
 
 namespace {
+
+__device__ __forceinline__ void tnr_quad_transpose(float &v0, float &v1, float &v2, float &v3, const bool b0, const bool b1) {
+    auto xchg = [&](float &x, float &y, bool sel, int which) {
+        const float send = sel ? x : y;
+        const int r_ = which == 1 ? __builtin_amdgcn_mov_dpp(__builtin_bit_cast(int, send), 0xB1, 0xF, 0xF, true)
+                                  : __builtin_amdgcn_mov_dpp(__builtin_bit_cast(int, send), 0x4E, 0xF, 0xF, true);
+        const float recv = __builtin_bit_cast(float, r_);
+        x = sel ? recv : x;
+        y = sel ? y : recv;
+    };
+    xchg(v0, v1, b0, 1);
+    xchg(v2, v3, b0, 1);
+    xchg(v0, v2, b1, 2);
+    xchg(v1, v3, b1, 2);
+}
+
+__device__ __forceinline__ f32x4 tnr_bias_act4(const f32x4 acc, const f32x4 bv, const float ns, const float alpha) {
+    f32x4 v = acc + bv;
+#pragma unroll
+    for (int e = 0; e < 4; ++e) v[e] = __builtin_fmaf(ns, __builtin_fminf(v[e], 0.f), __builtin_fmaxf(v[e], 0.f)) * alpha;
+    return v;
+}
 
 template <int MODE, int TW, int NT, int MT, bool COH, int DEPTH = 1, bool NOISE = true, int BIAS_STEP = 1, class PixFn>
 __device__ __forceinline__ void conv_epilogue_dpp_map(const ConvK a, f32x16 (&acc)[MT][NT], const int cb, const int n, const int ty0,
@@ -16,20 +38,7 @@
 #endif
     const int qa = li >> 2, qb = li & 3;
     const bool b0 = (qb & 1) != 0, b1 = (qb & 2) != 0;
-    auto quad_transpose = [&](float &v0, float &v1, float &v2, float &v3) {
-        auto xchg = [&](float &x, float &y, bool sel, int which) {
-            const float send = sel ? x : y;
-            const int r_ = which == 1 ? __builtin_amdgcn_mov_dpp(__builtin_bit_cast(int, send), 0xB1, 0xF, 0xF, true)
-                                      : __builtin_amdgcn_mov_dpp(__builtin_bit_cast(int, send), 0x4E, 0xF, 0xF, true);
-            const float recv = __builtin_bit_cast(float, r_);
-            x = sel ? recv : x;
-            y = sel ? y : recv;
-        };
-        xchg(v0, v1, b0, 1);
-        xchg(v2, v3, b0, 1);
-        xchg(v0, v2, b1, 2);
-        xchg(v1, v3, b1, 2);
-    };
+    auto quad_transpose = [&](float &v0, float &v1, float &v2, float &v3) { tnr_quad_transpose(v0, v1, v2, v3, b0, b1); };
     TNR_STAMP(5);
     TNR_STAMP(6);
     TNR_STAMP(7);
@@ -109,9 +118,7 @@
         for (int nn = 0; nn < NT; ++nn) {
             float v0 = acc[mi][nn][4 * q + 0], v1 = acc[mi][nn][4 * q + 1], v2 = acc[mi][nn][4 * q + 2], v3 = acc[mi][nn][4 * q + 3];
             quad_transpose(v0, v1, v2, v3);
-            f32x4 v = f32x4{v0, v1, v2, v3} + bv[nn];
-#pragma unroll
-            for (int e = 0; e < 4; ++e) v[e] = __builtin_fmaf(ns, __builtin_fminf(v[e], 0.f), __builtin_fmaxf(v[e], 0.f)) * a.alpha;
+            f32x4 v = tnr_bias_act4(f32x4{v0, v1, v2, v3}, bv[nn], ns, a.alpha);
             if (has_r1) v += b1f[nn] * q1[set][nn];
             if (has_noise) {
                 const f32x4 nm = tnr_gauss_mult4(((unsigned)pixi[set] + a.noise_pix0) * (unsigned)(a.Cout >> 2) + (unsigned)(co_n[nn] >> 2),
@@ -156,6 +163,52 @@
     }
 }
 
+template <int QN, class PatchFn>
+__device__ __forceinline__ void conv_epilogue_pool2(const ConvK a, unsigned char *route, const float (&win)[4][QN * 4], const int q0,
+                                                    const int cb, const int n, const int ty0, const int tx0, const int li, const int half,
+                                                    PatchFn &&patchfn) {
+    const int qa = li >> 2, qb = li & 3;
+    const bool b0 = (qb & 1) != 0, b1 = (qb & 2) != 0;
+    const float ns = a.act == TNR_ACT_LRELU ? a.slope : (a.act == TNR_ACT_RELU ? 0.f : 1.f);
+    const int co = cb * 32 + qa * 4;
+    f32x4 bv = {0.f, 0.f, 0.f, 0.f};
+    if (a.bias != nullptr) bv = *reinterpret_cast<const f32x4 *>(a.bias + co);
+    const int Hp = a.Ho >> 1, Wp = a.Wo >> 1;
+#pragma unroll
+    for (int qq = 0; qq < QN; ++qq) {
+        int pr, pc;
+        patchfn(8 * (q0 + qq) + 4 * half + qb, pr, pc);
+        const int py = (ty0 >> 1) + pr, px = (tx0 >> 1) + pc;
+        f32x4 best;
+        unsigned arg[4] = {0u, 0u, 0u, 0u};
+#pragma unroll
+        for (int k = 0; k < 4; ++k) {
+            float v0 = win[k][4 * qq + 0], v1 = win[k][4 * qq + 1], v2 = win[k][4 * qq + 2], v3 = win[k][4 * qq + 3];
+            tnr_quad_transpose(v0, v1, v2, v3, b0, b1);
+            const f32x4 v = tnr_bias_act4(f32x4{v0, v1, v2, v3}, bv, ns, a.alpha);
+            if (k == 0) {
+                best = v;
+            } else {
+#pragma unroll
+                for (int e = 0; e < 4; ++e) {
+                    const bool gt = v[e] > best[e];
+                    best[e] = gt ? v[e] : best[e];
+                    arg[e] = gt ? (unsigned)k : arg[e];
+                }
+            }
+        }
+        if (!(py < Hp && px < Wp)) continue;
+        const size_t pix = ((size_t)n * Hp + py) * Wp + px;
+        *reinterpret_cast<f32x4 *>(a.y + pix * a.y_ct + a.y_co + co) = best;
+        if (route != nullptr) {
+            unsigned w = 0u;
+#pragma unroll
+            for (int e = 0; e < 4; ++e) w |= (arg[e] | (best[e] > 0.f ? 4u : 0u)) << (8 * e);
+            *reinterpret_cast<unsigned *>(route + pix * a.Cout + co) = w;
+        }
+    }
+}
+
 template <int MODE, int TW, int NT, int MT, bool COH, int DEPTH = 1, bool NOISE = true, int BIAS_STEP = 1>
 __device__ __forceinline__ void conv_epilogue_dpp(const ConvK a, f32x16 (&acc)[MT][NT], const int cb, const int n, const int ty0,
                                                   const int tx0, const int par, const int wave, const int li, const int half,
diff --git a/trainner_amd/csrc/conv_wino.hip b/trainner_amd/csrc/conv_wino.hip
--- a/trainner_amd/csrc/conv_wino.hip
+++ b/trainner_amd/csrc/conv_wino.hip
@@ -43,6 +43,8 @@
     int wq_bytes;
     int nck;
     int tiles_x, tiles_y, ncb, tiles;
+    int pool;
+    unsigned char *route;
 };
 
 struct WinoPackK {
@@ -380,6 +382,29 @@
                 }
         }
         __syncthreads();
+        if (c.pool != 0) {
+            float win[4][8];
+            auto slot = [&](int ip, int l) __attribute__((always_inline)) {
+                return smem + (((ip >> 1) * 4 + wn * 2 + (ip & 1)) * 4 + l * 2 + wh) * (16 * 64) + wil * (8 * 64) + lane;
+            };
+#pragma unroll
+            for (int l = 0; l < 2; ++l) {
+                const float *p0 = slot(0, l), *p1 = slot(1, l), *p2 = slot(2, l), *p3 = slot(3, l);
+#pragma unroll
+                for (int r = 0; r < 8; ++r) {
+                    const float x0 = p0[r * 64], x1 = p1[r * 64], x2 = p2[r * 64], x3 = p3[r * 64];
+                    win[l][r] = (x0 + x1) + x2;
+                    win[2 + l][r] = (x1 - x2) - x3;
+                }
+            }
+            conv_epilogue_pool2<2>(a, c.route, win, 2 * wil, cb * 2 + wn, n, ty0, tx0, li, half,
+                                   [&](int row, int &pr, int &pc) __attribute__((always_inline)) {
+                                       const int p = 32 * wh + row;
+                                       pr = p >> 3;
+                                       pc = p & 7;
+                                   });
+            continue;
+        }
         f32x16 keep[2][1];
         {
             const int k = wil, m = wh;
@@ -665,14 +690,24 @@
     return tnr_check_launch("conv_wino_pack");
 }
 
-int tnr_launch_conv3x3_wino(const tnr_conv_desc *d, void *stream) {
+namespace {
+
+bool wino16_requested() {
+    static const bool w16 = [] { const char *e = getenv("TNR_WINO_WAVES"); return e != nullptr && atoi(e) == 16; }();
+    return w16;
+}
+
+int launch_wino(const tnr_conv_desc *d, int pool, unsigned char *route, void *stream) {
     if (!wino_ok(d) || d->wq == nullptr || d->wq_bytes < tnr_conv_wino_bytes(d) || d->noise_pos < 0 || d->noise_pos > 2) return 1;
     static int cus = 0;
     if (const int rc = tnr_kernel_setup(&cus, "conv3x3_wino", {{conv3x3_wino_kernel, WN_LDS_BYTES}, {conv3x3_wino16_kernel, WN_LDS_BYTES}})) return rc;
     WinoK c;
     if (!stream_k_from_desc(c, *d, tnr_conv_wino_bytes(d), WN_T, WN_T, 1)) return 1;
+    c.pool = pool;
+    c.route = route;
     const int grid = c.tiles < cus ? c.tiles : cus;
-    static const bool w16 = [] { const char *e = getenv("TNR_WINO_WAVES"); return e != nullptr && atoi(e) == 16; }();
+    const bool w16 = wino16_requested();
+    if (w16 && pool != 0) return 1;
     if (w16) {
         hipLaunchKernelGGL(conv3x3_wino16_kernel, dim3((unsigned)grid), dim3(1024), WN_LDS_BYTES, (hipStream_t)stream, c);
         return tnr_check_launch("conv3x3_wino16");
@@ -680,3 +715,24 @@
     hipLaunchKernelGGL(conv3x3_wino_kernel, dim3((unsigned)grid), dim3(512), WN_LDS_BYTES, (hipStream_t)stream, c);
     return tnr_check_launch("conv3x3_wino");
 }
+
+}
+
+int tnr_launch_conv3x3_wino(const tnr_conv_desc *d, void *stream) { return launch_wino(d, 0, nullptr, stream); }
+
+extern "C" int tnr_conv_pool_ok(const tnr_conv_desc *d) {
+    return d != nullptr && wino_ok(d) && !wino16_requested() && (d->H % 2) == 0 && (d->W % 2) == 0 &&
+           (d->act == TNR_ACT_RELU || d->act == TNR_ACT_NONE) && d->r1.ptr == nullptr && d->r2.ptr == nullptr && d->m.ptr == nullptr &&
+           d->noise_pos == 0 && d->shuffle == 0 && d->ws == nullptr && views_aligned(*d);
+}
+
+extern "C" int tnr_conv_forward_pool2(const tnr_conv_desc *d, uint8_t *route, void *stream) {
+    TNR_REQUIRE(d != nullptr && d->x.ptr && d->y.ptr && d->wp, "conv_forward_pool2: null pointer");
+    TNR_REQUIRE(tnr_conv_pool_ok(d), "conv_forward_pool2: the launch cannot store its pooled output (tnr_conv_pool_ok() == 0)");
+    TNR_REQUIRE(d->wq != nullptr && d->wq_form == 1 && d->wq_bytes >= tnr_conv_wino_bytes(d),
+                "conv_forward_pool2: needs the transform-domain weight stream (tnr_conv_wino_pack, wq_form = 1)");
+    TNR_REQUIRE((reinterpret_cast<uintptr_t>(route) & 3) == 0, "conv_forward_pool2: the route map must be 4-byte aligned");
+    const int rc = launch_wino(d, 2, route, stream);
+    TNR_REQUIRE(rc != 1, "conv_forward_pool2: the launch does not qualify for the Winograd kernel");
+    return rc;
+}
diff --git a/trainner_amd/csrc/elementwise.hip b/trainner_amd/csrc/elementwise.hip
--- a/trainner_amd/csrc/elementwise.hip
+++ b/trainner_amd/csrc/elementwise.hip
@@ -199,6 +199,36 @@
         }
 #pragma unroll
         for (int k = 0; k < 4; ++k) *reinterpret_cast<f32x4 *>(gx + ip[k] * gx_ct + gx_co + c4 * 4) = o[k];
+    }
+}
+
+__global__ void unpool2_bwd_kernel(const float *gy, int g_ct, int g_co, const unsigned char *map, float *gx, int gx_ct, int gx_co, int N,
+                                   int H, int W, int C) {
+    const int Ho = H / 2, Wo = W / 2, c4n = C / 4;
+    const int64_t total = (int64_t)N * Ho * Wo * c4n;
+    for (int64_t e = (int64_t)blockIdx.x * blockDim.x + threadIdx.x; e < total; e += (int64_t)gridDim.x * blockDim.x) {
+        const int c4 = (int)(e % c4n);
+        const int64_t pix = e / c4n;
+        const int ox = (int)(pix % Wo);
+        const int64_t q = pix / Wo;
+        const int oy = (int)(q % Ho);
+        const int64_t n = q / Ho;
+        const f32x4 g = *reinterpret_cast<const f32x4 *>(gy + pix * g_ct + g_co + c4 * 4);
+        const unsigned mw = *reinterpret_cast<const unsigned *>(map + pix * C + c4 * 4);
+        f32x4 o[4];
+#pragma unroll
+        for (int j = 0; j < 4; ++j) {
+            const unsigned b = (mw >> (8 * j)) & 0xffu;
+            const int arg = (int)(b & 3u);
+            const bool on = (b & 4u) != 0u;
+#pragma unroll
+            for (int k = 0; k < 4; ++k) o[k][j] = (k == arg && on) ? g[j] : 0.f;
+        }
+#pragma unroll
+        for (int k = 0; k < 4; ++k) {
+            const int64_t ip = (n * H + 2 * oy + (k >> 1)) * W + 2 * ox + (k & 1);
+            *reinterpret_cast<f32x4 *>(gx + ip * gx_ct + gx_co + c4 * 4) = o[k];
+        }
     }
 }
 
@@ -457,6 +487,15 @@
     return tnr_check_launch("maxpool2_bwd");
 }
 
+extern "C" int tnr_unpool2_bwd(tnr_view gy, const uint8_t *map, tnr_view gx, int32_t N, int32_t H, int32_t W, int32_t C, void *stream) {
+    TNR_REQUIRE(view_ok(gy) && view_ok(gx) && map != nullptr && (reinterpret_cast<uintptr_t>(map) & 3) == 0 && N > 0 && H > 0 && W > 0 && C > 0 &&
+                (C % 4) == 0 && (H % 2) == 0 && (W % 2) == 0, "unpool2_bwd: bad arguments");
+    const int64_t total = (int64_t)N * (H / 2) * (W / 2) * (C / 4);
+    hipLaunchKernelGGL(unpool2_bwd_kernel, dim3(ew_grid(total)), dim3(EW_BLOCK), 0, (hipStream_t)stream, gy.ptr, gy.ctot, gy.coff, map,
+                       gx.ptr, gx.ctot, gx.coff, N, H, W, C);
+    return tnr_check_launch("unpool2_bwd");
+}
+
 extern "C" int tnr_im2col(tnr_view x, int32_t N, int32_t H, int32_t W, int32_t C, int32_t k, int32_t stride, int32_t pad,
                           int32_t Ho, int32_t Wo, float *out, void *stream) {
     TNR_REQUIRE(view_ok(x) && out != nullptr && (C % 4) == 0 && k >= 1 && stride >= 1 && pad >= 0, "im2col: bad arguments");
diff --git a/trainner_amd/engine.py b/trainner_amd/engine.py
--- a/trainner_amd/engine.py
+++ b/trainner_amd/engine.py
@@ -59,6 +59,11 @@
     def fwd_shuffle2(self, x, y, **epi):
         return ops.conv_shuffle2(x, self.packer.get(self.i_f), y, layer=self.dirs[False][1], bias=self.mod.bias, **epi)
 
+    def fwd_pool2(self, x, y, route=None, **epi):
+        if self.mode_f != ops.CONV_3x3:
+            return False
+        return ops.conv_pool2(x, self.packer.get(self.i_f), y, route=route, layer=self.dirs[False][1], bias=self.mod.bias, **epi)
+
     def dgrad(self, g, gx, **epi):
         self._run(True, g, gx, epi)
 
diff --git a/trainner_amd/hip.py b/trainner_amd/hip.py
--- a/trainner_amd/hip.py
+++ b/trainner_amd/hip.py
@@ -79,6 +79,8 @@
     "tnr_conv_wq_pack": (c_i, [C.POINTER(ConvDesc), c_p, c_l, c_p]),
     "tnr_conv_wino_bytes": (c_l, [C.POINTER(ConvDesc)]),
     "tnr_conv_wino_pack": (c_i, [C.POINTER(ConvDesc), c_p, c_l, c_p]),
+    "tnr_conv_pool_ok": (c_i, [C.POINTER(ConvDesc)]),
+    "tnr_conv_forward_pool2": (c_i, [C.POINTER(ConvDesc), c_p, c_p]),
     "tnr_gauss_mult": (c_i, [CView, CView, c_l, c_i, c_f, C.c_uint32, C.c_uint32, C.c_uint32, c_p]),
     "tnr_im2col": (c_i, [CView, c_i, c_i, c_i, c_i, c_i, c_i, c_i, c_i, c_i, c_p, c_p]),
     "tnr_conv_chain_workspace_bytes": (c_l, [C.POINTER(ConvDesc)]),
@@ -109,6 +111,7 @@
     "tnr_space_to_depth_bwd": (c_i, [CView, CView, c_i, c_i, c_i, c_i, CView, c_f, c_p]),
     "tnr_maxpool2_fwd": (c_i, [CView, CView, c_i, c_i, c_i, c_i, c_p]),
     "tnr_maxpool2_bwd": (c_i, [CView, CView, CView, c_i, c_i, c_i, c_i, c_p]),
+    "tnr_unpool2_bwd": (c_i, [CView, c_p, CView, c_i, c_i, c_i, c_i, c_p]),
     "tnr_gconv_fwd": (c_i, [CView, c_i, c_i, c_i, c_i, c_p, c_p, CView, c_i, c_i, c_i, c_i, c_i, c_i, c_i, c_i, c_f, c_p]),
     "tnr_gconv_dgrad": (c_i, [CView, c_i, c_i, c_i, c_i, c_p, CView, c_i, c_i, c_i, c_i, c_i, c_i, c_i, c_p]),
     "tnr_gconv_wgrad_workspace_bytes": (c_l, [c_i, c_i, c_i]),
diff --git a/trainner_amd/models/modules/architectures/perceptual.py b/trainner_amd/models/modules/architectures/perceptual.py
--- a/trainner_amd/models/modules/architectures/perceptual.py
+++ b/trainner_amd/models/modules/architectures/perceptual.py
@@ -30,6 +30,22 @@
 
 
 TORCHVISION_FILES = {"vgg11": "vgg11-8a719046.pth", "vgg13": "vgg13-19584684.pth", "vgg16": "vgg16-397923af.pth", "vgg19": "vgg19-dcbb9e9d.pth"}
+
+
+class PooledAway:
+    __slots__ = ("route", "pooled")
+
+    def __init__(self, route, pooled):
+        self.route, self.pooled = route, pooled
+
+    def dense(self):
+        p = self.pooled.dense()
+        N, Hp, Wp, Cc = p.shape
+        arg = self.route & 3
+        out = torch.full((N, Hp, 2, Wp, 2, Cc), float("-inf"), dtype=p.dtype, device=p.device)
+        for k in range(4):
+            out[:, :, k >> 1, :, k & 1] = torch.where(arg == k, p, out[:, :, k >> 1, :, k & 1])
+        return out.reshape(N, 2 * Hp, 2 * Wp, Cc)
 
 
 class FeatureExtractor(HipNet):
@@ -122,6 +138,30 @@
             self._norm = (scale, shift)
         return self._norm
 
+    def _fwd_pooled(self, i, cur, save):
+        names = self.names
+        n = names[i]
+        if (i + 2 >= len(names) or not names[i + 2].startswith("pool") or n in self.listen_list or names[i + 1] in self.listen_list
+                or not ops.pool_fold_on() or cur.H % 2 or cur.W % 2):
+            return None
+        shape = (cur.N, cur.H // 2, cur.W // 2, self.feature_net[n].out_channels)
+        dev = cur.buf.device
+        y = View(new_act(*shape, dev))
+        route = torch.empty(shape, dtype=torch.uint8, device=dev) if save else None
+        if not self._ops[n].fwd_pool2(cur, y, route=route, act=ops.ACT_RELU):
+            return None
+        away = PooledAway(route, y) if save else None
+        return [(n, cur, away), (names[i + 2], away, y)]
+
+    @staticmethod
+    def _pool_bwd(g, xin, y):
+        gx = View(new_act(y.N, 2 * y.H, 2 * y.W, y.C, y.buf.device))
+        if isinstance(xin, View):
+            ops.maxpool2_bwd(g, xin, gx)
+        else:
+            ops.unpool2_bwd(g, xin.route, gx)
+        return gx
+
     def engine_forward(self, x, save):
         N, Cc, H, W = x.shape
         if Cc != 3:
@@ -130,9 +170,14 @@
         scale, shift = self._norm_consts(dev)
         x4 = View(new_act(N, H, W, 4, dev))
         ops.nchw_to_nhwc(x, x4, Cpad=4, scale=scale, shift=shift)
-        cur, tape = x4, []
-        for n in self.names:
+        cur, tape, folded = x4, [], None
+        for i, n in enumerate(self.names):
             if n.startswith("conv"):
+                entries = self._fwd_pooled(i, cur, save)
+                if entries is not None:
+                    tape += entries
+                    cur, folded = entries[1][2], entries[1][0]
+                    continue
                 y = View(new_act(N, cur.H, cur.W, self.feature_net[n].out_channels, dev))
                 if n == self.listen:
                     self._ops[n].fwd(cur, y)
@@ -140,7 +185,7 @@
                     self._ops[n].fwd(cur, y, act=ops.ACT_RELU)
                 tape.append((n, cur, y))
                 cur = y
-            elif n.startswith("pool"):
+            elif n.startswith("pool") and n != folded:
                 y = View(new_act(N, cur.H // 2, cur.W // 2, cur.C, dev))
                 ops.maxpool2_fwd(cur, y)
                 tape.append((n, cur, y))
@@ -160,10 +205,10 @@
         g = View(g_nhwc)
         for i in range(len(tape) - 1, -1, -1):
             n, xin, y = tape[i]
-            gx = View(new_act(N, xin.H, xin.W, xin.C, dev))
             if n.startswith("pool"):
-                ops.maxpool2_bwd(g, xin, gx)
+                gx = self._pool_bwd(g, xin, y)
             else:
+                gx = View(new_act(N, xin.H, xin.W, xin.C, dev))
                 prev = tape[i - 1][0] if i > 0 else None
                 if prev is not None and prev.startswith("conv"):
                     self._ops[n].dgrad(g, gx, mask=xin, m_slope=0.0)
@@ -183,9 +228,14 @@
         scale, shift = self._norm_consts(dev)
         x4 = View(new_act(N, H, W, 4, dev))
         ops.nchw_to_nhwc(x, x4, Cpad=4, scale=scale, shift=shift)
-        cur, tape, feats = x4, [], {}
+        cur, tape, feats, folded = x4, [], {}, None
         for i, n in enumerate(self.names):
             if n.startswith("conv"):
+                entries = self._fwd_pooled(i, cur, save)
+                if entries is not None:
+                    tape += entries
+                    cur, folded = entries[1][2], entries[1][0]
+                    continue
                 y = View(new_act(N, cur.H, cur.W, self.feature_net[n].out_channels, dev))
                 if n not in self.listen_list:
                     self._ops[n].fwd(cur, y, act=ops.ACT_RELU)
@@ -199,12 +249,13 @@
                 tape.append((n, cur, y))
                 cur = y
             elif n.startswith("pool"):
-                y = View(new_act(N, cur.H // 2, cur.W // 2, cur.C, dev))
-                ops.maxpool2_fwd(cur, y)
-                tape.append((n, cur, y))
-                cur = y
+                if n != folded:
+                    y = View(new_act(N, cur.H // 2, cur.W // 2, cur.C, dev))
+                    ops.maxpool2_fwd(cur, y)
+                    tape.append((n, cur, y))
+                    cur = y
                 if n in self.listen_list:
-                    feats[n] = y
+                    feats[n] = cur
             elif n in self.listen_list:
                 feats[n] = cur
         outs = tuple(feats[n].buf.permute(0, 3, 1, 2) for n in self.taps)
@@ -216,7 +267,9 @@
         return View(g_nhwc if g_nhwc.is_contiguous() else g_nhwc.contiguous())
 
     def _inject(self, entry, tg, g):
-        n, _, y = entry
+        n, xin, y = entry
+        if not isinstance(y, View):
+            return g
         dev = y.buf.device
 
         def add(g, t):
@@ -249,10 +302,10 @@
         for i in range(len(tape) - 1, -1, -1):
             n, xin, y = tape[i]
             if g is not None:
-                gx = View(new_act(N, xin.H, xin.W, xin.C, dev))
                 if n.startswith("pool"):
-                    ops.maxpool2_bwd(g, xin, gx)
+                    gx = self._pool_bwd(g, xin, y)
                 else:
+                    gx = View(new_act(N, xin.H, xin.W, xin.C, dev))
                     prev = tape[i - 1][0] if i > 0 else None
                     if prev is not None and prev.startswith("conv"):
                         self._ops[n].dgrad(g, gx, mask=xin, m_slope=0.0)
diff --git a/trainner_amd/ops.py b/trainner_amd/ops.py
--- a/trainner_amd/ops.py
+++ b/trainner_amd/ops.py
@@ -441,6 +441,38 @@
     _conv_launch(x, wp, y, mode, wino, 0, epi, family=family)
 
 
+_NATIVE_CONV = conv
+_FullRes = collections.namedtuple("_FullRes", "N H W C pixels")
+
+
+def pool_fold_on():
+    return os.environ.get("TNR_POOL_FOLD", "1") != "0"
+
+
+def conv_pool2(x, wp, y, route=None, layer=None, wino=None, **epi):
+    if conv is not _NATIVE_CONV or not x.buf.is_cuda or not pool_fold_on() or x.H % 2 or x.W % 2 or (y.N, y.H, y.W) != (x.N, x.H // 2, x.W // 2):
+        return False
+    full = _FullRes(x.N, x.H, x.W, y.C, x.N * x.H * x.W)
+    if conv_plan(x, wp, full, CONV_3x3, epi, 0, layer, wino)[0] != "wino":
+        return False
+    lib, d = hip.load(), ConvDesc()
+    _conv_desc(d, x, wp, y, CONV_3x3, **epi)
+    d.Ho, d.Wo = x.H, x.W
+    if not lib.tnr_conv_pool_ok(C.byref(d)):
+        return False
+    img = _wino_image(lib, d, wp, x.buf.device)
+    if img is None:
+        return False
+    d.wq, d.wq_bytes, d.wq_form = img.data_ptr(), img.numel() * 4, 1
+    if route is not None:
+        assert route.dtype == torch.uint8 and route.is_contiguous() and tuple(route.shape) == (y.N, y.H, y.W, y.C)
+    t0 = PROFILE.begin() if PROFILE is not None else None
+    hip.check(lib.tnr_conv_forward_pool2(C.byref(d), hip.ptr(route), hip.stream()), "conv_forward_pool2")
+    if PROFILE is not None:
+        PROFILE.end("conv_wino_3x3", 2.0 * d.N * d.Ho * d.Wo * 9 * min(x.C, wp.KinP) * d.Cout, t0, (x.C, d.Cout, d.Ho, wp.kind))
+    return True
+
+
 UPFOLD_FAMILY = "conv_upfold"
 UPFOLD_PASSES = ("fwd", "dgrad", "wgrad")
 UPFOLD_TAPS = ((2,), (1, 2), (0, 1), (0,))
@@ -918,6 +950,12 @@
     hip.check(hip.load().tnr_maxpool2_bwd(gy.c(), x.c(), gx.c(), x.N, x.H, x.W, x.C, hip.stream()), "maxpool2_bwd")
 
 
+def unpool2_bwd(gy, route, gx):
+    assert route.dtype == torch.uint8 and route.is_contiguous() and tuple(route.shape) == (gy.N, gy.H, gy.W, gy.C)
+    assert (gx.N, gx.H, gx.W, gx.C) == (gy.N, 2 * gy.H, 2 * gy.W, gy.C)
+    hip.check(hip.load().tnr_unpool2_bwd(gy.c(), route.data_ptr(), gx.c(), gx.N, gx.H, gx.W, gx.C, hip.stream()), "unpool2_bwd")
+
+
 def bilinear2x_fwd(x, y):
     hip.check(hip.load().tnr_bilinear2x_fwd(x.c(), y.c(), x.N, x.H, x.W, x.C, hip.stream()), "bilinear2x_fwd")
 
```

New measurement: 73.75, median of 6. +1.0%, better.
